# cavelandiah/BBMap

Hardware: AMD Instinct MI355X
Metric: aligned_reads_per_sec (higher is better)
Workload: dtype int32

## Files before the change

### bbmap_amd/csrc/mapper_ctx.h

```cpp
#pragma once
#include <hip/hip_runtime.h>

#include <cstdio>
#include <thread>
#include <vector>

#include "bbmap_amd.h"
#include "host_common.h"
#include "index_ctx.h"
#include "mapper_dev.h"
#include "msa_ctx.h"

enum { HIO_READS, HIO_BASES, HIO_SCORES, HIO_KEYINFO, HIO_COUNTS, HIO_OFFSETS, HIO_PACKED, BUF_PACK_TMP, BUF_SAM_TMP, BUF_SAM_TEXT, BUF_COUNT };

enum { ACC_STATS, ACC_COV, ACC_HIST, ACC_SPLIT, ACC_COUNT };
struct Accum { bool counted = false; hipStream_t stream = nullptr; };

struct bbmap_ctx {
    bbmap_config cfg;
    bbidx_ctx *index;
    hipStream_t hostStream = nullptr;
    bbidx_launch probeLs;
    bbmsa_ctx *msa, *msaGapped;
    bbmapper::Settings S;
    std::vector<void *> allocs;
    bbidx_site *d_psites; int *d_pnsites;
    bbmap_msite *d_ms; int *d_mcount, *d_near;
    bbmapper::SlowState *d_slow;
    int *d_active[2];
    int *d_classList;
    unsigned *d_counters;
    bbmsa_job *d_jobs; bbmap_jobinfo *d_jinfo; bbmsa_result *d_results; uint8_t *d_match;
    bbmsa_job *d_gjobs; bbmsa_gaps *d_ggaps; bbmap_jobinfo *d_ginfo; bbmsa_result *d_gresults; uint8_t *d_gmatch;
    bbresc_job *d_rjobs; bbmapper::RescInfo *d_rinfo; bbresc_result *d_rres; bbmapper::PairResc *d_pres; bbmap_msite *d_rsite;
    const uint8_t *const *d_chromArr; const int *d_chromArrLen; const uint8_t *refsBase;
    int *d_chromMin;
    long long *d_chromOff;
    long long jobCap, gjobCap, rescCap;
    bbmapper::FinalRead *d_fin; bbmap_final *d_final; uint8_t *d_pool; long long poolUnits, poolUsed, finalFills;
    int matchStride, gmatchStride, maxRows, plainColumns;
    unsigned *h_counters;
    hipEvent_t ev[bbmapper::EV_COUNT];
    bbmap_stats stats;
    long long nJobs, nGapped;
    bool ran;
    bbmap_ctx *tier;
    bool ownsMsa;
    long long narrowMinJobs;
    bool sortWide;
    bool sortPlain;
    bool classSwap;
    bool classOrder;
    bool kernargDev;
    int *d_tierUnits; bbidx_read *d_tierReads; int *d_tierReadIds;
    long long tierReads;
    hipStream_t tierStream;
    hipStream_t dpStream; hipEvent_t evFork, evJoin;
    std::thread tierThread;
    bool tierStarted;
    int tierRc; char tierErr[320];
    long long overAfterBegin;
    struct BatchArgs { int64_t n_reads; const bbidx_read *reads; uint8_t *bases; int64_t minus_delta; const int8_t *baseScores; const int32_t *keyinfo; } batch;
    DevBuf buf[BUF_COUNT];
    bbmap_scafrec *d_scafRec = nullptr;
    int *d_scafTier = nullptr;
    bbmap_samrec *d_samRec = nullptr;
    bbmap_samtags *d_samTags = nullptr;
    int *d_samCounts = nullptr;
    long long *d_samOffsets = nullptr;
    float *d_mapqMax = nullptr;
    long long samTextBytes = 0;
    unsigned long long *d_runStats = nullptr, *d_insertHist = nullptr;
    int adaptive = 0;
    long long numMatedSeen = 0;
    const bbmap_truth *truthNext = nullptr;
    struct CovState *cov = nullptr;
    unsigned long long *d_readHist = nullptr;
    int rhFlags = 0;
    uint8_t *d_pool2 = nullptr; long long pool2Units = 0;
    int *d_untrimCounts = nullptr;
    long long *d_untrimOffsets = nullptr;
    DevBuf untrimTmp;
    bool untrimmed = false;
    struct SplitState *split = nullptr;
    Accum accum[ACC_COUNT];
    void new_batch() { for (Accum &a : accum) a.counted = false; untrimmed = false; }
};

struct SplitState {
    bbmap_split_config cfg = {};
    int nscaf = 0;
    long long gen = 0, added = -1, total = 0;
    DevBuf sets, keys, state, recs, ws, setoff, units;
    SplitState() = default;
    SplitState(const SplitState &) = delete;
    ~SplitState() { for (DevBuf *b : {&sets, &keys, &state, &recs, &ws, &setoff, &units}) b->release(); }
};

struct CovState {
    int flags = 0, nscaf = 0, binsize = -1;
    long long slots = 0, nbins = 0, gen = 0;
    DevBuf covoff, len, diff[2], depth[2], recs, hist[2], totals, ws, refgc, binoff, bins[2];
// ... 19 lines not shown
```

### bbmap_amd/csrc/mapper_host.hip

```cpp
#include <hip/hip_runtime.h>

#include <algorithm>
#include <cstdlib>
#include <cstring>
#include <new>
#include <thread>
#include <vector>

#include "mapper_ctx.h"

using namespace bbmapper;

extern "C" int bbmap_default_config_profile(int32_t profile, bbmap_config *c) {
    if (!c || (profile != BBIDX_PROFILE_BBMAP && profile != BBIDX_PROFILE_PACBIO)) return bbfail(BBMAP_E_ARG, "bbmap_default_config: bad argument");
    memset(c, 0, sizeof *c);
    c->paired = 0; c->max_reads = 0; c->max_sites = 32;
    c->extraPadding = 10; c->maxPairDist = 32000; c->averagePairDist = 100; c->maxRescueDist = 1200; c->maxRescueMismatches = 32;
    c->maxTrimSitesToRetain = 800; c->trimList = 1; c->doRescue = 1; c->clearzone3 = 800; c->fastCols = 0; c->jobsPerRead = 0;
    c->finalStage = profile == BBIDX_PROFILE_BBMAP ? 1 : 0;
    if (profile == BBIDX_PROFILE_PACBIO) {
        c->max_read_len = 6016; c->minRatio = 0.46f; c->slowAlignPadding = 8; c->slowRescuePadding = 16; c->tipSearchDist = 15;
        c->alignColumns = 7600; c->msaMaxColumns = 7600;
    } else {
        c->max_read_len = 150; c->minRatio = 0.56f; c->slowAlignPadding = 4; c->slowRescuePadding = 8; c->tipSearchDist = 100;
// ... 62 lines not shown
    S.clearzone1e = 2 * S.ptsMatch2 - S.ptsMatch - S.ptsSub + 1;
    S.msaMaxColumns = cfg->msaMaxColumns;
    if (pacbio) { S.ptsSubR = -157; S.ptsIns = -205; S.ptsIns2 = -42; S.ptsIns3 = -23; S.ptsIns4 = -8; S.ptsDel = -292; S.ptsDel2 = -37; S.ptsDel3 = -17; S.ptsDel4 = -2; }
    else { S.ptsSubR = -147; S.ptsIns = -395; S.ptsIns2 = -39; S.ptsIns3 = -23; S.ptsIns4 = -8; S.ptsDel = -472; S.ptsDel2 = -33; S.ptsDel3 = -9; S.ptsDel4 = -1; }
    S.ptsDel5 = -1; S.ptsGap = -2;
    if (pacbio && (cfg->finalStage < 0 || cfg->finalStage > 2)) return bail(bbfail(BBMAP_E_ARG, "bbmap_create: finalStage must be 0, 1 or 2"));
    S.finalStage = cfg->finalStage ? 1 : 0;
    S.finalPolicy = (pacbio && cfg->finalStage == 1) ? 1 : 0;
    {
        const float rP = S.finalPolicy ? 1.5f : 1.6f, r1 = S.finalPolicy ? 2.2f : 2.0f, r1b = S.finalPolicy ? 2.8f : 2.6f, r1c = S.finalPolicy ? 4.8f : 4.6f;
        const float m2 = (float)S.ptsMatch2;
        S.czP = (int)(rP * m2); S.cz1 = (int)(r1 * m2); S.cz1b = (int)(r1b * m2); S.cz1c = (int)(r1c * m2);
        S.czLimit1e = 40;
    }
    index->dev.p.quitAfterTwoPerfects = cfg->paired ? 0 : 1;
    S.expLimit = (cfg->alignColumns * 17) / 20 - (2 * (cfg->slowAlignPadding + 10));
    const int maxRows = ((cfg->max_read_len + 31) / 32) * 32;
    c->maxRows = maxRows;
    bbmsa_config mc; memset(&mc, 0, sizeof mc);
    mc.device = cfg->device; mc.maxRows = maxRows;
    bbmsa_config gc;
    if (pacbio) {
        mc.maxRows = cfg->max_read_len + 4 > 6100 ? 6100 : cfg->max_read_len + 4;
        c->maxRows = mc.maxRows;
        mc.maxColumns = cfg->msaMaxColumns;
        mc.reserved[2] = BBMSA_SCHEME_9PACBIO;
        gc = mc;
        c->plainColumns = mc.maxColumns;
        if (parent) { c->msa = parent->msa; c->msaGapped = parent->msaGapped; c->ownsMsa = false; }
        else {
            c->ownsMsa = true;
            if ((rc = bbmsa_create(&mc, &c->msa)) != BBMAP_OK) return bail(rc);
            c->msaGapped = c->msa;
        }
    } else {
        mc.maxColumns = cfg->fastCols > 0 ? cfg->fastCols : 256;
        if (mc.maxColumns > cfg->msaMaxColumns) mc.maxColumns = cfg->msaMaxColumns;
        c->plainColumns = mc.maxColumns;
        gc = mc;
        gc.maxColumns = cfg->msaMaxColumns;
        gc.reserved[0] = 32; gc.reserved[1] = 640 < gc.maxColumns ? 640 : gc.maxColumns;
        if (const char *e = getenv("BBMAP_G2_LANES")) { if (*e) gc.reserved[0] = atoi(e); }
        if (const char *e = getenv("BBMAP_G2_COLS")) { if (*e) gc.reserved[1] = atoi(e) < gc.maxColumns ? atoi(e) : gc.maxColumns; }
        (void)parent;
        c->ownsMsa = true;
        if ((rc = bbmsa_create(&mc, &c->msa)) != BBMAP_OK) return bail(rc);
        if ((rc = bbmsa_create(&gc, &c->msaGapped)) != BBMAP_OK) return bail(rc);
    }
    const long long n = cfg->max_reads;
    const int cap = cfg->max_sites;
    c->narrowMinJobs = getenv("BBMAP_NARROW_MIN_JOBS") ? atoll(getenv("BBMAP_NARROW_MIN_JOBS")) : 32768;
    c->sortWide = !(getenv("BBMAP_SORT_WIDE") && atoi(getenv("BBMAP_SORT_WIDE")) == 0);
    c->sortPlain = !(getenv("BBMAP_SORT_PLAIN") && atoi(getenv("BBMAP_SORT_PLAIN")) == 0);
    c->classOrder = !(getenv("BBMAP_CLASS_ORDER") && atoi(getenv("BBMAP_CLASS_ORDER")) == 0);
    c->classSwap = getenv("BBMAP_CLASS_ORDER") && atoi(getenv("BBMAP_CLASS_ORDER")) == 2;
    c->kernargDev = !(getenv("BBMAP_KERNARG_DEV") && atoi(getenv("BBMAP_KERNARG_DEV")) == 0);
    S.chunkLoads = !(getenv("BBMAP_CHUNK_LOADS") && atoi(getenv("BBMAP_CHUNK_LOADS")) == 0);
    if (!pacbio) {
        const bool wideUnl = !(getenv("BBMAP_WIDE_UNLIMITED") && atoi(getenv("BBMAP_WIDE_UNLIMITED")) == 0);
        bbmsa_set_wide_unlimited(c->msa, wideUnl);
        if (c->msaGapped != c->msa) bbmsa_set_wide_unlimited(c->msaGapped, wideUnl);
    }
    if (!pacbio) {
        const long long lat = getenv("BBMAP_LATENCY_JOBS") ? atoll(getenv("BBMAP_LATENCY_JOBS")) : 4096;
        if ((rc = bbmsa_set_latency_jobs(c->msa, lat)) != BBMAP_OK) return bail(rc);
        if (c->msaGapped != c->msa && (rc = bbmsa_set_latency_jobs(c->msaGapped, lat)) != BBMAP_OK) return bail(rc);
    }
    const int jpr = cfg->jobsPerRead > 0 ? cfg->jobsPerRead : 3;
    c->jobCap = n * jpr + 1024;
    c->gjobCap = parent ? n * 16 + 4096 : (n * jpr) / 24 + 4096;
    if (cfg->jobsPerRead < 0) c->jobCap = c->gjobCap = -(long long)cfg->jobsPerRead;
    c->rescCap = parent ? n * 64 + 1024 : n * 2 + 1024;
    c->matchStride = ((maxRows + c->plainColumns + 15) / 16) * 16;
    c->gmatchStride = ((maxRows + gc.maxColumns + 2 + 128 * 8 + 15) / 16) * 16;
#define DA(ptr, count) if ((rc = dalloc(c, &(ptr), (size_t)(count))) != BBMAP_OK) return bail(rc)
    DA(c->d_psites, n * cap); DA(c->d_pnsites, n);
    DA(c->d_ms, n * cap); DA(c->d_mcount, n); DA(c->d_near, n);
    DA(c->d_slow, n);
    DA(c->d_active[0], n); DA(c->d_active[1], n);
    c->d_classList = nullptr;
    if (c->classOrder) DA(c->d_classList, 2 * n);
    DA(c->d_counters, CNT_WORDS);
    DA(c->d_jobs, c->jobCap); DA(c->d_jinfo, c->jobCap); DA(c->d_results, c->jobCap); DA(c->d_match, c->jobCap * c->matchStride);
    DA(c->d_gjobs, c->gjobCap); DA(c->d_ggaps, c->gjobCap); DA(c->d_ginfo, c->gjobCap); DA(c->d_gresults, c->gjobCap); DA(c->d_gmatch, c->gjobCap * c->gmatchStride);
    DA(c->d_rjobs, c->rescCap); DA(c->d_rinfo, c->rescCap); DA(c->d_rres, c->rescCap); DA(c->d_rsite, c->rescCap);
    DA(c->d_pres, n / 2 + 1);
    if (S.finalStage) {
        c->poolUnits = (n * (long long)(3 * (cfg->max_read_len + 16)) + 65536) / 4;
        if (const char *e = getenv("BBMAP_FINAL_POOL_UNITS")) { if (*e && atoll(e) >= 64) c->poolUnits = atoll(e); }
        DA(c->d_fin, n); DA(c->d_final, n); DA(c->d_pool, c->poolUnits * 4);
    }
    const int nch = index->dev.nchroms;
    DA(c->d_chromMin, nch + 1); DA(c->d_chromOff, nch + 1);
#undef DA
    c->d_chromArr = index->dev.chromArr; c->d_chromArrLen = index->dev.chromArrLen;
    {
        std::vector<const uint8_t *> hc((size_t)nch + 1);
        if (hipMemcpy(hc.data(), index->dev.chromArr, sizeof(void *) * hc.size(), hipMemcpyDeviceToHost) != hipSuccess) return bail(bbfail(BBMAP_E_HIP, "bbmap_create: reading the chromosome table failed"));
        c->refsBase = hc[1];
        std::vector<long long> off((size_t)nch + 1, 0);
        for (int i = 1; i <= nch; i++) off[(size_t)i] = (long long)(hc[(size_t)i] - hc[1]);
        if (hipMemcpy(c->d_chromOff, off.data(), 8 * off.size(), hipMemcpyHostToDevice) != hipSuccess) return bail(bbfail(BBMAP_E_HIP, "bbmap_create: upload failed"));
        if (hipMemset(c->d_chromMin, 0, 4 * ((size_t)nch + 1)) != hipSuccess) return bail(bbfail(BBMAP_E_HIP, "bbmap_create: memset failed"));
    }
    if (hipHostMalloc((void **)&c->h_counters, CNT_WORDS * 4) != hipSuccess) return bail(bbfail(BBMAP_E_NOMEM, "bbmap_create: pinned allocation failed"));
    for (hipEvent_t &e : c->ev) if (hipEventCreate(&e) != hipSuccess) return bail(bbfail(BBMAP_E_HIP, "bbmap_create: hipEventCreate failed"));
// ... 30 lines not shown
    return BBMAP_OK;
}

static int read_counters(bbmap_ctx *c, hipStream_t stream) {
    BBHIP(hipMemcpyAsync(c->h_counters, c->d_counters, CNT_WORDS * 4, hipMemcpyDeviceToHost, stream));
    BBHIP(hipStreamSynchronize(stream));
    return BBMAP_OK;
}

template <class T> static int regrow(bbmap_ctx *c, hipStream_t stream, T **p, size_t oldCount, size_t newCount, std::vector<void *> &dead) {
    void *d = nullptr;
    if (hipMalloc(&d, (newCount ? newCount : 1) * sizeof(T)) != hipSuccess) return bbfail(BBMAP_E_NOMEM, "bbmap_map_batch_device: growing a fill log failed (device memory)");
    if (oldCount) BBHIP(hipMemcpyAsync(d, *p, oldCount * sizeof(T), hipMemcpyDeviceToDevice, stream));
    for (void *&q : c->allocs) if (q == (void *)*p) q = d;
    dead.push_back((void *)*p);
    *p = (T *)d;
    return BBMAP_OK;
}
struct DeadArrays {
    hipStream_t stream; std::vector<void *> v;
    explicit DeadArrays(hipStream_t s) : stream(s) {}
    ~DeadArrays() { if (!v.empty()) { (void)hipStreamSynchronize(stream); for (void *q : v) (void)hipFree(q); } }
};
static int grow_logs(bbmap_ctx *c, hipStream_t stream, Dev &D, long long needJobs, long long needGapped, long long usedJobs, long long usedGapped) {
    DeadArrays guard(stream);
    std::vector<void *> &dead = guard.v;
    if (needJobs > c->jobCap) {
        long long nc = c->jobCap * 2; if (nc < needJobs) nc = needJobs + needJobs / 4 + 1024;
        BBTRY(regrow(c, stream, &c->d_jobs, (size_t)usedJobs, (size_t)nc, dead));
        BBTRY(regrow(c, stream, &c->d_jinfo, (size_t)usedJobs, (size_t)nc, dead));
        BBTRY(regrow(c, stream, &c->d_results, (size_t)usedJobs, (size_t)nc, dead));
        BBTRY(regrow(c, stream, &c->d_match, (size_t)usedJobs * c->matchStride, (size_t)nc * c->matchStride, dead));
        c->jobCap = nc;
    }
    if (needGapped > c->gjobCap) {
        long long nc = c->gjobCap * 2; if (nc < needGapped) nc = needGapped + needGapped / 4 + 1024;
        BBTRY(regrow(c, stream, &c->d_gjobs, (size_t)usedGapped, (size_t)nc, dead));
        BBTRY(regrow(c, stream, &c->d_ggaps, (size_t)usedGapped, (size_t)nc, dead));
        BBTRY(regrow(c, stream, &c->d_ginfo, (size_t)usedGapped, (size_t)nc, dead));
        BBTRY(regrow(c, stream, &c->d_gresults, (size_t)usedGapped, (size_t)nc, dead));
        BBTRY(regrow(c, stream, &c->d_gmatch, (size_t)usedGapped * c->gmatchStride, (size_t)nc * c->gmatchStride, dead));
        c->gjobCap = nc;
    }
    c->h_counters[CNT_STAGE_FILLS] = (unsigned)usedJobs; c->h_counters[CNT_STAGE_GAPPED] = (unsigned)usedGapped;
    BBHIP(hipMemcpyAsync(c->d_counters + CNT_FILLS, c->h_counters + CNT_STAGE_FILLS, 8, hipMemcpyHostToDevice, stream));
    BBHIP(hipStreamSynchronize(stream));
    D.jobs = c->d_jobs; D.jinfo = c->d_jinfo; D.results = c->d_results; D.match = c->d_match; D.jobCap = c->jobCap;
    D.gjobs = c->d_gjobs; D.ggaps = c->d_ggaps; D.ginfo = c->d_ginfo; D.gresults = c->d_gresults; D.gmatch = c->d_gmatch; D.gjobCap = c->gjobCap;
    c->stats.log_growths += 1.0f;
    return BBMAP_OK;
}

static int run_fills(bbmap_ctx *c, hipStream_t stream, const uint8_t *bases, long long jobBase, long long nNew, long long gBase, long long gNew,
                     bool finalStage = false) {
    bbmsa_use_narrow(c->msa, nNew >= c->narrowMinJobs);
    bbmsa_sort_by_width(c->msa, c->sortPlain && nNew >= c->narrowMinJobs);
    bbmsa_sort_with_band(c->msa, c->sortPlain);
    if (c->msaGapped != c->msa) { bbmsa_use_narrow(c->msaGapped, false); bbmsa_sort_by_width(c->msaGapped, c->sortWide); }
    hipStream_t gs = (c->dpStream && nNew > 0) ? c->dpStream : stream;
    if (gNew > 0) {
        if (gs != stream) { BBHIP(hipEventRecord(c->evFork, stream)); BBHIP(hipStreamWaitEvent(gs, c->evFork, 0)); }
        BBTRY(bbmsa_align_gapped_batch_device(c->msaGapped, gs, gNew, c->d_gjobs + gBase, c->d_ggaps + gBase, bases, c->refsBase,
                                             c->d_gresults + gBase, c->d_gmatch + gBase * c->gmatchStride, c->gmatchStride));
        if (gs != stream) { BBHIP(hipEventRecord(c->evJoin, gs)); if (nNew > 0) BBTRY(bbmsa_wait_first_pass(c->msaGapped, stream)); }
    }
    if (nNew > 0)
        BBTRY(bbmsa_align_batch_device(c->msa, stream, nNew, c->d_jobs + jobBase, bases, c->refsBase, c->d_results + jobBase,
                                      c->d_match + jobBase * c->matchStride, c->matchStride));
    const int r1 = nNew > 0 ? bbmsa_last_route_flags(c->msa) : 0;
    const int r2 = gNew > 0 ? bbmsa_last_route_flags(c->msaGapped) : 0;
    c->stats.dp_narrow_launches += (r1 & 1) + (r2 & 1);
    c->stats.dp_sorted_launches += ((r1 >> 1) & 1) + ((r2 >> 1) & 1);
    if (gNew > 0 && gs != stream) BBHIP(hipStreamWaitEvent(stream, c->evJoin, 0));
    return BBMAP_OK;
}

static void add_dp_ms(bbmap_ctx *c, bool plain, bool gapped) {
    float k3[3];
    if (plain && bbmsa_last_kernel_ms3(c->msa, k3) == BBMAP_OK) { c->stats.ms_dp_narrow += k3[0]; c->stats.ms_dp_wave += k3[1]; c->stats.ms_dp_generic += k3[2];
                                                                 if (k3[1] > c->stats.ms_dp_wave_max) c->stats.ms_dp_wave_max = k3[1]; }
    if (gapped && c->msaGapped != c->msa && bbmsa_last_kernel_ms3(c->msaGapped, k3) == BBMAP_OK) c->stats.ms_dp_gapped += k3[0] + k3[1] + k3[2];
    static const bool show = getenv("BBMAP_DP_COUNTS") != nullptr;
    if (show) {
        int64_t n4[4], u4[4];
        if (plain && bbmsa_last_counts(c->msa, n4) == BBMAP_OK && bbmsa_last_unlimited(c->msa, u4) == BBMAP_OK)
            fprintf(stderr, "dp counts plain : narrow finished %lld, narrow handed on %lld, wavefront list %lld, to the wide/generic pass %lld, "
                    "unlimited in their own build %lld, in the general build %lld, wavefront steps unlimited %lld of %lld\n",
                    (long long)n4[0], (long long)n4[1], (long long)n4[2], (long long)n4[3], (long long)u4[0], (long long)u4[1], (long long)u4[2], (long long)u4[3]);
        if (gapped && bbmsa_last_counts(c->msaGapped, n4) == BBMAP_OK && bbmsa_last_unlimited(c->msaGapped, u4) == BBMAP_OK)
            fprintf(stderr, "dp counts second: narrow finished %lld, narrow handed on %lld, wavefront list %lld, to the wide/generic pass %lld, "
                    "unlimited in their own build %lld, in the general build %lld, wavefront steps unlimited %lld of %lld\n",
                    (long long)n4[0], (long long)n4[1], (long long)n4[2], (long long)n4[3], (long long)u4[0], (long long)u4[1], (long long)u4[2], (long long)u4[3]);
    }
}

static void tier_start_async(bbmap_ctx *c, long long found);

struct Rounds {
    bool finalStage;
    long long jobBase, gBase;
    long long nActive;
    int cur = 0;
    bool first = true, ranPlain = false, ranGapped = false;
};
template <class K> static int round_begin(bbmap_ctx *c, hipStream_t stream, Dev &D, Rounds &R, K kernel) {
    BBHIP(hipMemsetAsync(c->d_counters + CNT_NEXT_ACTIVE, 0, 4, stream));
    if (R.finalStage) {
        BBHIP(hipMemsetAsync(c->d_counters + CNT_POOL_AT_FAILURE, 0xff, 4, stream));
        BBHIP(hipMemsetAsync(c->d_counters + CNT_POOL_FAILED, 0, 4, stream));
    }
    D.activeIn = R.first ? nullptr : c->d_active[R.cur]; D.nActiveIn = (int)R.nActive; D.activeOut = c->d_active[1 - R.cur];
    BBTRY(launch<128>(kernel, R.nActive, stream, D));
    return read_counters(c, stream);
}
static int round_end(bbmap_ctx *c, hipStream_t stream, Dev &D, Rounds &R, const uint8_t *bases) {
    add_dp_ms(c, R.ranPlain, R.ranGapped);
    const long long asked = c->h_counters[CNT_FILLS], gasked = c->h_counters[CNT_GAPPED_FILLS];
    const long long total = asked < c->jobCap ? asked : c->jobCap, gtotal = gasked < c->gjobCap ? gasked : c->gjobCap;
    BBTRY(run_fills(c, stream, bases, R.jobBase, total - R.jobBase, R.gBase, gtotal - R.gBase, R.finalStage));
    R.ranPlain = total > R.jobBase; R.ranGapped = gtotal > R.gBase;
    R.jobBase = total; R.gBase = gtotal;
    if (asked > c->jobCap || gasked > c->gjobCap) BBTRY(grow_logs(c, stream, D, asked, gasked, total, gtotal));
    R.nActive = c->h_counters[CNT_NEXT_ACTIVE];
    R.cur = 1 - R.cur; R.first = false;
    return BBMAP_OK;
}

static int grow_pool(bbmap_ctx *c, hipStream_t stream, Dev &D, long long used, long long units, bool setCounter) {
    if (units > 0x7ffffff0LL) return bbfail(BBMAP_E_NOMEM, "bbmap_map_batch_device: the final stage's match strings exceed 8 GB; map smaller batches");
    DeadArrays guard(stream);
    BBTRY(regrow(c, stream, &c->d_pool, (size_t)used * 4, (size_t)units * 4, guard.v));
    if (setCounter) {
        c->h_counters[CNT_STAGE_POOL] = (unsigned)used;
        BBHIP(hipMemcpyAsync(c->d_counters + CNT_POOL_UNITS, c->h_counters + CNT_STAGE_POOL, 4, hipMemcpyHostToDevice, stream));
    }
    BBHIP(hipStreamSynchronize(stream));
    c->poolUnits = units; D.pool = c->d_pool; D.poolUnits = units;
    return BBMAP_OK;
}

static int run_final_stage(bbmap_ctx *c, hipStream_t stream, Dev &D, int64_t n_reads, const uint8_t *bases, long long jobBase, long long gBase,
                           long long &finalRounds, long long &finalLocal) {
    const long long units = c->cfg.paired ? n_reads / 2 : n_reads;
    const unsigned *h = c->h_counters;
    D.fin = c->d_fin; D.finalOut = c->d_final; D.pool = c->d_pool; D.poolUnits = c->poolUnits;
    D.match = c->d_match; D.gmatch = c->d_gmatch; D.matchStride = c->matchStride; D.gmatchStride = c->gmatchStride;
    if (D.classList) BBHIP(hipMemsetAsync(c->d_counters + CNT_CLASS_LONG, 0, 8, stream));
    BBTRY(launch<128>(final_begin_kernel, units, stream, D));
    Rounds R; R.finalStage = true; R.jobBase = jobBase; R.gBase = gBase; R.nActive = n_reads;
    for (int round = 0; R.nActive > 0; round++) {
        if (round > 64 * c->cfg.max_sites + 64) return bbfail(BBMAP_E_HIP, "bbmap_map_batch_device: the final stage does not come to an end (internal error)");
        BBTRY(round_begin(c, stream, D, R, DEV_KERNEL(c, final_round_kernel)));
        BBTRY(round_end(c, stream, D, R, bases));
        if (h[CNT_POOL_FAILED] > 0) {
            const long long used = h[CNT_POOL_AT_FAILURE];
            long long nu = c->poolUnits * 2, need = used + ((long long)h[CNT_POOL_UNITS] - used) * 2 + 65536;
            if (nu < need) nu = need;
            BBTRY(grow_pool(c, stream, D, used, nu, true));
        }
        finalRounds++;
    }
    BBHIP(hipStreamSynchronize(stream));
    add_dp_ms(c, R.ranPlain, R.ranGapped);
    BBHIP(hipMemsetAsync(c->d_counters + CNT_LOCAL_READS, 0, 8, stream));
    BBTRY(launch<128>(final_end_kernel, units, stream, D));
    BBTRY(read_counters(c, stream));
    finalLocal = h[CNT_LOCAL_READS];
    const long long used = h[CNT_POOL_UNITS], local = h[CNT_LOCAL_UNITS];
    if (used + local + 64 > c->poolUnits) BBTRY(grow_pool(c, stream, D, used, used + local + 65536, false));
    BBTRY(launch<128>(final_local_kernel, units, stream, D));
    return BBMAP_OK;
}
// ... 51 lines not shown
    if (writeRc) BBTRY(launch<128>(revcomp_unprobed_kernel, n_reads, stream, reads, (long long)n_reads, (int)c->index->dev.p.k, (const uint8_t *)bases, bases + minus_delta));
    BBHIP(hipEventRecord(c->ev[EV_PROBE_END], stream));
    Dev D;
    fill_dev(c, D, n_reads, reads, bases, minus_delta);
    const long long units = c->cfg.paired ? n_reads / 2 : n_reads;
    BBTRY(launch<128>(begin_kernel, units, stream, D));
    if (c->tier) {
        BBTRY(launch<128>(collect_overflow_kernel, units, stream, c->d_mcount, units, c->cfg.paired, c->d_tierUnits, c->d_counters + CNT_TIER_FOUND));
    }
    BBHIP(hipEventRecord(c->ev[EV_BEGIN_END], stream));
    BBTRY(launch<128>(DEV_KERNEL(c, score_kernel), n_reads, stream, D));
    BBHIP(hipEventRecord(c->ev[EV_SCORE_END], stream));
    Rounds R; R.finalStage = false; R.jobBase = R.gBase = 0; R.nActive = n_reads;
    for (int round = 0; R.nActive > 0 && round < 4 * c->cfg.max_sites + 4; round++) {
        BBTRY(round_begin(c, stream, D, R, slow_round_kernel));
        if (round == 0) {
            float pms = 0; long long ps[5];
            if (writeRc && bbidx_last_stats_with(c->index, &c->probeLs, (int64_t *)ps, &pms) == BBMAP_OK) for (int i = 0; i < 5; i++) c->stats.probe_stats[i] = ps[i];
            c->overAfterBegin = c->h_counters[CNT_OVERFLOWED];
            if (c->tier && c->h_counters[CNT_TIER_FOUND] > 0 && c->tier->msa != c->msa) tier_start_async(c, c->h_counters[CNT_TIER_FOUND]);
        }
        BBTRY(round_end(c, stream, D, R, bases));
        c->stats.rounds++;
    }
    long long jobBase = R.jobBase, gBase = R.gBase;
    BBHIP(hipEventRecord(c->ev[EV_SLOW_END], stream));
    BBTRY(launch<128>(finish_kernel, n_reads, stream, D));
    BBHIP(hipEventRecord(c->ev[EV_FINISH_END], stream));
    if (c->cfg.paired && c->cfg.doRescue) {
        const long long pairs = n_reads / 2;
        for (int pass = 0; pass < 2; pass++) {
            D.pass = pass;
            BBHIP(hipMemsetAsync(c->d_counters + CNT_RESCUE_SEARCHES, 0, 4, stream));
            BBTRY(launch<128>(rescue_plan_kernel, pairs, stream, D));
            BBTRY(read_counters(c, stream));
            const long long nsearch = c->h_counters[CNT_RESCUE_SEARCHES];
            if (nsearch > c->rescCap) return bbfail(BBMAP_E_NOMEM, "bbmap_map_batch_device: rescue list full");
            c->stats.rescue_scans += nsearch;
            if (nsearch == 0) {
                BBTRY(launch<128>(rescue_finish_kernel, pairs, stream, D));
                continue;
            }
            hipEvent_t q0 = c->ev[EV_QUICK_BEGIN], q1 = c->ev[EV_QUICK_END];
            BBHIP(hipEventRecord(q0, stream));
            BBTRY(bbpipe_quick_rescue_device(stream, nsearch, c->d_rjobs, bases, (const int64_t *)c->d_chromOff, c->d_chromArrLen, c->d_chromMin, c->refsBase,
                                            c->d_rres, c->S.ptsMatch, c->S.ptsMatch2, 1, 100));
            BBHIP(hipEventRecord(q1, stream));
            if (jobBase + nsearch > c->jobCap || gBase + nsearch > c->gjobCap) BBTRY(grow_logs(c, stream, D, jobBase + nsearch, gBase + nsearch, jobBase, gBase));
            BBTRY(launch<128>(DEV_KERNEL(c, rescue_prep_kernel), pairs, stream, D));
            BBTRY(read_counters(c, stream));
            { float ms = 0; if (hipEventElapsedTime(&ms, q0, q1) == hipSuccess) c->stats.ms_quick_rescue += ms; }
            const long long total = c->h_counters[CNT_FILLS], gtotal = c->h_counters[CNT_GAPPED_FILLS];
            if (total > c->jobCap || gtotal > c->gjobCap) return bbfail(BBMAP_E_HIP, "bbmap_map_batch_device: rescue fills beyond the reserved log entries (internal error)");
            BBTRY(run_fills(c, stream, bases, jobBase, total - jobBase, gBase, gtotal - gBase));
            const bool ranPlain = total > jobBase, ranGapped = gtotal > gBase;
            jobBase = total; gBase = gtotal;
            BBTRY(launch<128>(rescue_finish_kernel, pairs, stream, D));
            BBHIP(hipStreamSynchronize(stream));
            add_dp_ms(c, ranPlain, ranGapped);
        }
    }
    BBHIP(hipEventRecord(c->ev[EV_RESCUE_END], stream));
    c->finalFills = 0; c->poolUsed = 0;
    long long finalRounds = 0, finalLocal = 0;
    if (c->S.finalStage) BBTRY(run_final_stage(c, stream, D, n_reads, bases, jobBase, gBase, finalRounds, finalLocal));
    BBTRY(finish_stats(c, stream, true, jobBase + gBase, finalRounds, finalLocal));
    c->ran = true;
    return BBMAP_OK;
}

static int tier_pass(bbmap_ctx *c, hipStream_t s, long long found) {
    bbmap_ctx *t = c->tier;
    const bbmap_ctx::BatchArgs &B = c->batch;
    const int paired = c->cfg.paired;
    c->tierReads = 0; t->ran = false;
    std::vector<int> ids((size_t)found);
    BBHIP(hipMemcpyAsync(ids.data(), c->d_tierUnits, 4 * (size_t)found, hipMemcpyDeviceToHost, s));
    BBHIP(hipStreamSynchronize(s));
    std::sort(ids.begin(), ids.end());
    const long long room = paired ? t->cfg.max_reads / 2 : t->cfg.max_reads;
    const long long take = found < room ? found : room;
    BBHIP(hipMemcpyAsync(c->d_tierUnits, ids.data(), 4 * (size_t)take, hipMemcpyHostToDevice, s));
    BBTRY(launch<128>(gather_reads_kernel, take, s, B.reads, c->d_tierUnits, (int)take, paired, c->d_tierReads, c->d_tierReadIds));
    BBHIP(hipStreamSynchronize(s));
    const long long tn = paired ? 2 * take : take;
    BBTRY(map_records(t, s, tn, c->d_tierReads, B.bases, B.minus_delta, B.baseScores, B.keyinfo, false));
    c->tierReads = tn;
    return BBMAP_OK;
}

static void tier_start_async(bbmap_ctx *c, long long found) {
    c->tierStarted = true; c->tierRc = BBMAP_OK; c->tierErr[0] = 0;
    c->tierThread = std::thread([c, found]() {
        int rc = hipSetDevice(c->cfg.device) == hipSuccess ? BBMAP_OK : BBMAP_E_HIP;
        if (rc == BBMAP_OK) rc = tier_pass(c, c->tierStream, found);
        if (rc != BBMAP_OK) { snprintf(c->tierErr, sizeof c->tierErr, "overflow tier: %s", bbmap_last_error()); }
        c->tierRc = rc;
    });
}

static int tier_finish(bbmap_ctx *c, hipStream_t stream) {
    bbmap_ctx *t = c->tier;
    const long long tn = c->tierReads;
    if (tn == 0) return BBMAP_OK;
    BBHIP(hipMemsetAsync(c->d_counters + CNT_TIER_RESOLVED, 0, 4, stream));
    BBTRY(launch<128>(mark_tier_kernel, tn, stream, c->d_mcount, t->d_mcount, c->d_tierReadIds, (int)tn, c->d_counters + CNT_TIER_RESOLVED));
    BBTRY(read_counters(c, stream));
    bbmap_stats &st = c->stats; const bbmap_stats &ts = t->stats;
    st.reads_reprobed = tn;
    st.reads_overflowed -= (long long)c->h_counters[CNT_TIER_RESOLVED];
    st.reads_without_site += ts.reads_without_site;
    st.fills += ts.fills; st.gapped_fills += ts.gapped_fills; st.refills += ts.refills; st.rescue_scans += ts.rescue_scans;
    st.rescue_fills += ts.rescue_fills; st.fills_dropped += ts.fills_dropped;
    st.final_fills += ts.final_fills; st.final_local += ts.final_local;
    st.dp_narrow_launches += ts.dp_narrow_launches; st.dp_sorted_launches += ts.dp_sorted_launches;
    st.sites_cross_scaffold += ts.sites_cross_scaffold;
    if (getenv("BBMAP_TIER_DEBUG"))
        fprintf(stderr, "[bbmap tier] reads %lld: probe %.2f begin %.2f score %.2f slow %.2f (rounds %lld) finish %.2f rescue %.2f total %.2f\n",
                tn, ts.ms_probe, ts.ms_begin, ts.ms_score, ts.ms_slow, (long long)ts.rounds, ts.ms_finish, ts.ms_rescue, ts.ms_total);
    return BBMAP_OK;
}

static int rescue_skip_rule(bbmap_ctx *c, bool *skip) {
    *skip = false;
    if (!c->d_runStats) return BBMAP_OK;
    bbmap_runstats rs;
    BBHIP(hipStreamSynchronize(c->accum[ACC_STATS].stream));
    BBHIP(hipMemcpy(&rs, c->d_runStats, sizeof rs, hipMemcpyDeviceToHost));
    *skip = rs.mappedRetained2 > 1000 && rs.numMated * 20LL < rs.mappedRetained2;
    return BBMAP_OK;
}

static int adapt_after_batch(bbmap_ctx *c, hipStream_t stream) {
    if (!(c->adaptive & BBMAP_ADAPT_INSERT_LENGTH)) return BBMAP_OK;
    bbmap_runstats rs;
    BBHIP(hipMemcpyAsync(&rs, c->d_runStats, sizeof rs, hipMemcpyDeviceToHost, stream));
    BBHIP(hipStreamSynchronize(stream));
    const bool heldPaired = rs.numMated > c->numMatedSeen;
    c->numMatedSeen = rs.numMated;
    if (rs.numMated > 1000 && heldPaired) {
        volatile float sum = (float)rs.innerLengthSum, cnt = (float)rs.numMated;
        const float q = sum * 1.0f / cnt;
        const int v = (int)q;
        if (v >= 0) BBTRY(bbmap_set_average_pair_dist(c, v));
    }
    return BBMAP_OK;
}

extern "C" int bbmap_get_adaptive_state(bbmap_ctx *c, int32_t *averagePairDist, int32_t *rescueSkipped) {
    if (!c) return bbfail(BBMAP_E_ARG, "bbmap_get_adaptive_state: null context");
    if (averagePairDist) *averagePairDist = c->cfg.averagePairDist;
    if (rescueSkipped) {
        bool skip = false;
        if (c->adaptive & BBMAP_ADAPT_RESCUE_SKIP) { BBHIP(hipSetDevice(c->cfg.device)); BBTRY(rescue_skip_rule(c, &skip)); }
        *rescueSkipped = skip ? 1 : 0;
    }
    return BBMAP_OK;
}

static int map_batch_device(bbmap_ctx *c, hipStream_t stream, int64_t n_reads, const bbidx_read *reads, uint8_t *bases,
                            int64_t minus_delta, const int8_t *baseScores, const int32_t *keyinfo) {
    c->batch = {n_reads, reads, bases, minus_delta, baseScores, keyinfo};
    c->tierStarted = false; c->tierReads = 0;
    if (c->tier) c->tier->ran = false;
    const int rc = map_records(c, stream, n_reads, reads, bases, minus_delta, baseScores, keyinfo, true);
    hipEvent_t e0 = c->ev[EV_TIER_BEGIN], e1 = c->ev[EV_TIER_END];
    if (c->tierStarted) {
        c->tierThread.join();
        if (rc == BBMAP_OK && c->tierRc != BBMAP_OK) return bbfail(c->tierRc, "%s", c->tierErr);
// ... 71 lines not shown
```

### bbmap_amd/csrc/msa_common.h

```cpp
#pragma once
#include <hip/hip_runtime.h>
#include <stdint.h>
#include "bbmap_amd.h"

namespace bbmsa {

constexpr int kScoreOffset = 11;
constexpr int kTimeMask = 0x7FF;
constexpr int kScoreMask = (int)0xFFFFF800;
constexpr int kMaxTime = 2047;

#define BBMSA_PT(x) ((x) * 2048)
constexpr int P_MATCH = BBMSA_PT(70), P_MATCH2 = BBMSA_PT(100);
constexpr int P_SUB = BBMSA_PT(-127), P_SUBR = BBMSA_PT(-147), P_SUB2 = BBMSA_PT(-51), P_SUB3 = BBMSA_PT(-25);
constexpr int P_INS = BBMSA_PT(-395), P_INS2 = BBMSA_PT(-39), P_INS3 = BBMSA_PT(-23), P_INS4 = BBMSA_PT(-8);
constexpr int P_DEL = BBMSA_PT(-472), P_DEL2 = BBMSA_PT(-33), P_DEL3 = BBMSA_PT(-9), P_DEL4 = BBMSA_PT(-1),
              P_DEL5 = BBMSA_PT(-1);
constexpr int P_DEL_REF_N = BBMSA_PT(-10), P_GAP = BBMSA_PT(-2);
constexpr int kBadOff = (-(((1 << 20) - 1) - 2000) - 1) * 2048;
constexpr int kMinOffScore = (-(((1 << 20) - 1) - 2000)) * 2048;
constexpr int kNegInf = -(1 << 30);
constexpr int kGapLen = 128;

constexpr int kTableLen = 3072;
// ... 48 lines not shown
    static constexpr int BAR_I1 = 1, BAR_D1 = 1;
    static constexpr int BADOFF = (-(((1 << 22) - 1) - 2000) - 1) * 512;
#undef BBMSA_PB
    __host__ __device__ static inline int del_off(int len) {
        if (len <= 0) return 0;
        int s = DEL;
        if (len > 80) { s += ((len - 80 + 3) / 4) * DEL5; len = 80; }
        if (len > 20) { s += (len - 20) * DEL4; len = 20; }
        if (len > 5) { s += (len - 5) * DEL3; len = 5; }
        if (len > 1) s += (len - 1) * DEL2;
        return s;
    }
    __host__ __device__ static inline int ins_cum_off(int len) {
        if (len <= 0) return 0;
        int s = INS;
        if (len > 20) { s += (len - 20) * INS4; len = 20; }
        if (len > 5) { s += (len - 5) * INS3; len = 5; }
        if (len > 1) s += (len - 1) * INS2;
        return s;
    }
    __host__ __device__ static inline int col0(int row) {
        if (row <= 0) return 0;
        int s = INS;
        if (row >= 20) { s += (row - 19) * INS4; row = 19; }
        if (row >= 5) { s += (row - 4) * INS3; row = 4; }
        if (row >= 2) s += (row - 1) * INS2;
        return s;
    }
};

__host__ __device__ inline int fill_halfband(int rows, int columns, int bandwidth, float bandwidthRatio) {
    if (bandwidth < 1 && bandwidthRatio <= 0.0f) return 0;
    const int bwA = bandwidth < 1 ? 9999999 : bandwidth;
    const int bwB = bandwidthRatio <= 0.0f ? 9999999 : 8 + (int)((float)rows * bandwidthRatio);
    return max(min(bwA, bwB), columns - rows + 8) / 2;
}
__host__ __device__ inline bool fill_is_limited(int flags, int minScore, int rows, int columns, int halfband) {
    const int mode = flags & BBMSA_MODE_MASK;
    if (mode == BBMSA_FILL_UNLIMITED_RAW) return false;
    if (mode == BBMSA_FILL_LIMITED_RAW) return true;
    return !(minScore < 1 || (columns + rows < 90) ||
             ((halfband < 1 || halfband * 3 > columns) && (columns > rows + min(170, rows + 20))));
}

__host__ __device__ inline bool band_is_candidate(int flags, int minScore, int rows, int columns, int maxRows, int maxColumns, int bandRows, int maxSlack) {
    const int mode = flags & BBMSA_MODE_MASK;
    if (!(rows >= 16 && columns >= rows && rows <= maxRows && rows <= bandRows && columns <= maxColumns && mode != BBMSA_FILL_UNLIMITED_RAW)) return false;
    int tmin = minScore;
    if (mode == BBMSA_FILL_LIMITED) {
        if (tmin < 1 || (columns + rows < 90) || (columns > rows + min(170, rows + 20))) return false;
        tmin -= 120;
    }
    return (70 + 100 * (rows - 1)) - tmin <= maxSlack;
}

__device__ inline long long job_count(long long njobs, const unsigned int *njobs_dev) {
    if (!njobs_dev) return njobs;
    const long long n = (long long)__hip_atomic_load(njobs_dev, __ATOMIC_RELAXED, __HIP_MEMORY_SCOPE_AGENT);
    return n < njobs ? n : njobs;
}

constexpr int kCounterWords = 32, kCounterBytes = kCounterWords * 4;
enum CounterSlot {
    CNT_FAST_QUEUE = 0,
    CNT_SLOW_COUNT = 1,
    CNT_GENERIC_QUEUE = 2,
    CNT_BAND_QUEUE = 3,
    CNT_LIST_COUNT = 4,
    CNT_BAND_DONE = 5,
    CNT_BAND_HANDED = 6,
    CNT_WIDE_SLOW_COUNT = 7,
    CNT_WIDE_QUEUE = 8,
    CNT_UNL_RAN_UNL = 9,
    CNT_UNL_RAN_GENERAL = 10,
    CNT_UNL_LIST_COUNT = 11,
    CNT_UNL_QUEUE = 12,
    CNT_UNL_STEPS = 13,
    CNT_ALL_STEPS = 14,
    CNT_CAND_COUNT = 15,
    CNT_SORTED_COUNT = 16,
    CNT_WAVE_STEPS = 17,
};
constexpr int CNT_BAND_STATS = 5, CNT_UNL_STATS = 9;
enum BandStat { BAND_STAT_DONE = 0, BAND_STAT_HANDED = 1 };
enum UnlStat { UNL_STAT_RAN_UNL = 0, UNL_STAT_RAN_GENERAL = 1, UNL_STAT_STEPS = 4, UNL_STAT_ALL_STEPS = 5, UNL_STAT_WAVE_STEPS = 8 };
static_assert(CNT_BAND_DONE == CNT_BAND_STATS + BAND_STAT_DONE && CNT_BAND_HANDED == CNT_BAND_STATS + BAND_STAT_HANDED, "band kernel's counters");
static_assert(CNT_UNL_RAN_UNL == CNT_UNL_STATS + UNL_STAT_RAN_UNL && CNT_UNL_RAN_GENERAL == CNT_UNL_STATS + UNL_STAT_RAN_GENERAL &&
              CNT_UNL_STEPS == CNT_UNL_STATS + UNL_STAT_STEPS && CNT_ALL_STEPS == CNT_UNL_STATS + UNL_STAT_ALL_STEPS &&
              CNT_WAVE_STEPS == CNT_UNL_STATS + UNL_STAT_WAVE_STEPS, "wavefront kernel's counters");
constexpr bool counter_slots_distinct() {
    constexpr int all[] = {CNT_FAST_QUEUE, CNT_SLOW_COUNT, CNT_GENERIC_QUEUE, CNT_BAND_QUEUE, CNT_LIST_COUNT, CNT_BAND_DONE, CNT_BAND_HANDED,
                           CNT_WIDE_SLOW_COUNT, CNT_WIDE_QUEUE, CNT_UNL_RAN_UNL, CNT_UNL_RAN_GENERAL, CNT_UNL_LIST_COUNT, CNT_UNL_QUEUE,
                           CNT_UNL_STEPS, CNT_ALL_STEPS, CNT_CAND_COUNT, CNT_SORTED_COUNT, CNT_WAVE_STEPS};
    unsigned seen = 0;
    for (int s : all) { if (s < 0 || s >= kCounterWords || ((seen >> s) & 1u)) return false; seen |= 1u << s; }
    return true;
}
static_assert(counter_slots_distinct(), "two counter names share a word, or one lies outside d_counters");

struct FillParams {
    const bbmsa_job *jobs;
    const uint8_t *reads;
    const uint8_t *refs;
    bbmsa_result *results;
    uint8_t *match;
    long long njobs;
    const unsigned int *njobs_dev;
    unsigned int *queue;
    unsigned int *dirbuf;
    long long dir_slot_dwords;
    const int *list;
    const unsigned int *list_count;
    int priority;
    int *slow_list;
    unsigned int *slow_count;
    int match_stride;
    int lanesPerJob;
    int fastCols;
    int tmpBytes;
    int tableLen;
    int maxRows, maxColumns;
    int bandwidth;
    float bandwidthRatio;
    unsigned int *unl_stats;
    int *planes;
    const long long *plane_off;
    int *limits;
    const long long *limits_off;
};

struct NarrowParams {
    const bbmsa_job *jobs;
    const uint8_t *reads;
    const uint8_t *refs;
    bbmsa_result *results;
    uint8_t *match;
    long long njobs;
    const unsigned int *njobs_dev;
    unsigned int *queue;
    int *fast_list;
    unsigned int *fast_count;
    unsigned int *stats;
    int match_stride;
    int maxRows, maxColumns;
    int bandwidth;
    float bandwidthRatio;
    int maxSlack;
    unsigned int *dirbuf32;
    int tableLen;
    int bandRows;
    const int *list;
    const unsigned int *list_count;
};

struct GenericParams {
    const bbmsa_job *jobs;
    const uint8_t *reads;
    const uint8_t *refs;
    bbmsa_result *results;
    uint8_t *match;
    const int *list;
    const unsigned int *list_count;
    long long njobs;
    const unsigned int *njobs_dev;
    int *matrix;
    int *limits;
    unsigned int *queue;
    int match_stride;
    int maxRows, maxColumns;
    int bandwidth;
    float bandwidthRatio;
};

}
```

### bbmap_amd/csrc/msa_ctx.h

```cpp
#pragma once
#include <hip/hip_runtime.h>

#include "bbmap_amd.h"
#include "host_common.h"
#include "msa_route.h"

struct bbmsa_ctx {
    bbmsa_config cfg = {};
    int device = 0;
    int numCUs = 0;
    RouteSwitches sw;
    Route last;
    int G = 0, R = 0, fastCols = 0, tmpBytes = 0, blocks = 0, ldsBytes = 0, tableLen = 0, wideTableLen = 0;
    long long dirSlotDwords = 0;
    unsigned int *d_dir = nullptr;
    unsigned int *d_counters = nullptr;
    DevBuf slowList;
    int genThreads = 0;
    int *d_matrix = nullptr;
    int *d_limits = nullptr;
    int wideR = 0, wideCols = 0, wideTmpBytes = 0, wideBlocks = 0, wideLdsBytes = 0;
    long long wideDirSlotDwords = 0;
    unsigned int *d_wideDir = nullptr;
    DevBuf slowList2;
    int narrowBlocks = 0, narrowSlack = 0;
    bool unlimitedStats = false;
    unsigned int *d_widthHist = nullptr;
    int bandRows = 0, bandLds = 0;
    unsigned int *d_bandDir = nullptr;
    DevBuf fastList;
    DevBuf gref, gaux, gjobs;
    hipEvent_t ev[4] = {};
    bool timed = false;
    bool legacyOnly = false;
    struct bbmsa_legacy *legacy = nullptr;
    int stripBlocks = 0, stripLds = 0;
    long long stripDwords = 0, stripSlotDwords = 0;
    int *d_stripBoundary = nullptr;
    uint8_t *d_stripTmp = nullptr;
    int pipeK = 0, pipeSlots = 0;
    int *d_pipeBoundary = nullptr, *d_pipeSync = nullptr;
};

struct JobBatch {
    int64_t n_jobs; const uint32_t *n_jobs_dev; const bbmsa_job *jobs; const uint8_t *reads, *refs; bbmsa_result *results; uint8_t *match;
    int32_t match_stride;
};
template <class P> void set_batch(P &p, const bbmsa_ctx *c, const JobBatch &B) {
    p.jobs = B.jobs; p.reads = B.reads; p.refs = B.refs; p.results = B.results; p.match = B.match;
    p.njobs = B.n_jobs; p.njobs_dev = B.n_jobs_dev; p.match_stride = B.match_stride;
    p.maxRows = c->cfg.maxRows; p.maxColumns = c->cfg.maxColumns; p.bandwidth = c->cfg.bandwidth; p.bandwidthRatio = c->cfg.bandwidthRatio;
}

int bbmsa_width_sort(bbmsa_ctx *c, hipStream_t stream, const bbmsa_job *jobs, int64_t n_jobs, bool band);

int bbmsa_align_impl(bbmsa_ctx *c, void *stream_, int64_t n_jobs, const uint32_t *n_jobs_dev, const bbmsa_job *jobs,
                     const uint8_t *reads, const uint8_t *refs, bbmsa_result *results, uint8_t *match, int32_t match_stride);

void bbmsa_use_narrow(bbmsa_ctx *c, bool on);
int bbmsa_wait_first_pass(bbmsa_ctx *c, void *waiter);
void bbmsa_sort_by_width(bbmsa_ctx *c, bool on);
void bbmsa_sort_with_band(bbmsa_ctx *c, bool on);
void bbmsa_set_wide_unlimited(bbmsa_ctx *c, bool on);
int bbmsa_set_latency_jobs(bbmsa_ctx *c, int64_t n);
enum { BBMSA_ROUTE_NARROW = 1, BBMSA_ROUTE_SORTED = 2, BBMSA_ROUTE_LATENCY = 4 };
int bbmsa_last_route_flags(const bbmsa_ctx *c);

int bbmsa_legacy_create(bbmsa_ctx *c);
void bbmsa_legacy_destroy(bbmsa_ctx *c);
void bbmsa_legacy_rows_per_lane(bbmsa_ctx *c, int *last, int *mask);
```

### bbmap_amd/csrc/msa_fill_band.hip

```cpp
#include "msa_common.h"
#include "msa_cell.h"

namespace bbmsa {

namespace {

__device__ __forceinline__ int from_left(int x, int fill) { return __builtin_amdgcn_update_dpp(fill, x, 0x138, 0xf, 0xf, false); }
__device__ __forceinline__ int from_right(int x, int fill) { return __builtin_amdgcn_update_dpp(fill, x, 0x130, 0xf, 0xf, false); }

__device__ __forceinline__ unsigned ld_coherent(const unsigned *p) { return __hip_atomic_load(p, __ATOMIC_RELAXED, __HIP_MEMORY_SCOPE_AGENT); }
__device__ __forceinline__ unsigned ld_coherent(const uint8_t *p) { return __hip_atomic_load(p, __ATOMIC_RELAXED, __HIP_MEMORY_SCOPE_AGENT); }

struct BandSet {
    int M[4], D[4], I[4];
    int rows, columns;
    int c0off;
    int minScoreOff, vs;
    unsigned w;
    int gprev;
    int gmask, mprev;
    int gpass;
    int bail;
    int rdOff, rfOff;
    int slot;
};

}

#ifndef BBMSA_BAND_OCC
#define BBMSA_BAND_OCC 4
#endif

template <int Q>
__global__ __launch_bounds__(256, BBMSA_BAND_OCC) void msa_fill_band_kernel(const NarrowParams p) {
    constexpr int B = 4 * Q;
    constexpr int GROUPS = 64 / Q;
    constexpr int JOBS = 2 * GROUPS;
    static_assert(Q == 4 || Q == 8 || Q == 16, "a group is a power of two of lanes, its good bits fit 64");
    extern __shared__ int lds[];
    const int TL = p.tableLen;
    int *delC = lds, *insC = lds + TL, *delExt = lds + 2 * TL, *insExt = delExt + 128;
    int4 *mTab = reinterpret_cast<int4 *>(delExt + 192);
    LdsPen pen; pen.delC = delC; pen.insC = insC; pen.delExt = delExt; pen.insExt = insExt; pen.mTab = mTab;
    for (int i = threadIdx.x; i < TL; i += blockDim.x) { delC[i] = calc_del_off(i); insC[i] = calc_ins_cum_off(i); }
    for (int i = threadIdx.x; i < 128; i += blockDim.x) delExt[i] = SpelledPen<Scheme11ts>().del_ext(i);
    if (threadIdx.x < 32) insExt[threadIdx.x] = SpelledPen<Scheme11ts>().ins_ext(threadIdx.x);
    if (threadIdx.x < 32) {
        const int st = threadIdx.x & 7, mt = (threadIdx.x >> 3) & 1, pv = threadIdx.x >> 4;
        const MEntry e = SpelledPen<Scheme11ts>().m_entry(min(st, 5), 0, 0, pv != 0, mt != 0);
        int4 v; v.x = e.addA; v.y = e.bonus; v.z = e.t3sub; v.w = 0;
        mTab[threadIdx.x] = v;
    }
    __syncthreads();

    const int lane = threadIdx.x & 63, wave = threadIdx.x >> 6;
    const int q = lane & (Q - 1), grp = lane / Q, groupBase = grp * Q;
    const int RB = (p.bandRows + 4 + 3) & ~3, FB = (p.bandRows + B + 4 + 3) & ~3;
    uint8_t *jobLds = reinterpret_cast<uint8_t *>(lds + lds_table_ints(TL)) + (long long)wave * JOBS * (RB + FB);
    unsigned *dir = p.dirbuf32 + ((long long)blockIdx.x * 4 + wave) * (long long)(p.bandRows + 1) * 128;
    const long long NJ = p.list ? (long long)ld_coherent(p.list_count) : job_count(p.njobs, p.njobs_dev);
    unsigned nDone = 0, nLeft = 0;

    for (;;) {
        long long myJ = -1;
        if (lane < JOBS) {
            for (;;) {
                const long long e_ = (long long)atomicAdd(p.queue, 1u);
                if (e_ >= NJ || e_ >= p.njobs) break;
                const long long t_ = p.list ? (long long)p.list[e_] : e_;
                const bbmsa_job t = p.jobs[t_];
                int ta = t.refStartLoc, tb = t.refEndLoc;
                if (t.flags & BBMSA_CLAMP_WINDOW) {
                    ta = max(0, ta); tb = min(t.ref_len - 1, tb);
                    if (tb - ta >= p.maxColumns) tb = min(t.ref_len - 1, ta + p.maxColumns - 1);
                }
                if (band_is_candidate(t.flags, t.minScore, t.read_len, tb - ta + 1, p.maxRows, p.maxColumns, p.bandRows, p.maxSlack)) { myJ = t_; break; }
                const unsigned k = atomicAdd(p.fast_count, 1u);
                p.fast_list[k] = (int)t_;
            }
        }
        if (!__any(myJ >= 0)) break;

        BandSet S[2];
        long long jobJ[2]; bool jobOk[2];
#pragma unroll
        for (int s = 0; s < 2; s++) {
            const long long j = __shfl(myJ, grp * 2 + s, 64);
            jobJ[s] = j;
            bbmsa_job jb;
            jb.read_off = 0; jb.ref_off = 0; jb.read_len = 0; jb.ref_len = 0; jb.refStartLoc = 0; jb.refEndLoc = -1; jb.minScore = 0; jb.flags = 0;
            if (j >= 0) jb = p.jobs[j];
            int a = jb.refStartLoc, b = jb.refEndLoc;
            if (jb.flags & BBMSA_CLAMP_WINDOW) {
                a = max(0, a); b = min(jb.ref_len - 1, b);
                if (b - a >= p.maxColumns) b = min(jb.ref_len - 1, a + p.maxColumns - 1);
            }
            const int rows = jb.read_len, columns = b - a + 1;
            int minScore = jb.minScore;
            if ((jb.flags & BBMSA_MODE_MASK) == BBMSA_FILL_LIMITED) minScore -= 120;
            const int D0 = (columns - rows) / 2 - B / 2;
            const uint8_t *rd = p.reads + jb.read_off, *rf = p.refs + jb.ref_off + a;
            const int rdOff = (grp * 2 + s) * (RB + FB), rfOff = rdOff + RB;
            int cost = 0; bool allDef = true;
#pragma unroll 4
            for (int i = q; i < rows; i += Q) {
                const int cb = rd[i];
                jobLds[rdOff + i] = (uint8_t)cb;
                if (fully_defined(cb)) cost += (i + 1 < rows && fully_defined(rd[i + 1])) ? P_MATCH2 : P_MATCH;
            }
            if (j >= 0)
#pragma unroll 4
            for (int k = q; k < rows + B + 1; k += Q) {
                const int col = k + D0;
                int v = 0;
                if (col == 0) v = '!';
                else if (col >= 1 && col <= columns) { v = rf[col - 1]; allDef = allDef && fully_defined(v); }
                jobLds[rfOff + k] = (uint8_t)v;
            }
            for (int c = 1 + q; c <= columns; c += Q) if (c < 1 + D0 || c > D0 + B) allDef = allDef && fully_defined(rf[c - 1]);
            int nd = allDef ? 0 : 1;
            for (int d = 1; d < Q; d <<= 1) { cost += __shfl_xor(cost, d, 64); nd |= __shfl_xor(nd, d, 64); }
            bool ok = j >= 0 && nd == 0;

            const int minScoreOff = minScore * 2048;
            const int floorv = minScoreOff - ((rows - 1) * P_MATCH2 + P_MATCH);
            const int subfloor = floorv - 5 * P_MATCH2;
            if (ok) {
                const int cl1 = rd[0];
                const int c0cost = fully_defined(cl1) ? ((rows > 1 && fully_defined(rd[1])) ? P_MATCH2 : P_MATCH) : 0;
                const int vlimP = max(minScoreOff - (cost - c0cost), floorv) + 2048;
                int outGood = 0;
                for (int c = 1 + q; c <= columns; c += Q) {
                    if (c >= 1 + D0 && c <= D0 + B) continue;
                    const int ref1 = rf[c - 1];
                    const int hs = c <= columns - 1 ? P_MATCH + (columns - 1 - c) * P_MATCH2 : 0;
                    CellIn ci;
                    ci.row = 1; ci.c = c; ci.rows = rows; ci.insNeededBase = (columns - c) + 1;
                    ci.cl1 = cl1; ci.ref1 = ref1; ci.refN = false; ci.gap = false; ci.match = cl1 == ref1; ci.act = true;
                    ci.refPen = 0; ci.limitP = max(vlimP, max(minScoreOff - hs, floorv) + 2048); ci.floorP = floorv + 2048; ci.subfloor = subfloor;
                    ci.dgM = 0; ci.dgD = 0; ci.dgI = 0;
                    ci.lM = c == 1 ? insC[1] : subfloor; ci.lD = ci.lM; ci.upM = 0; ci.upI = 0;
                    ci.delForce = INT_MAX;
                    ci.insForce = (c > 1 || (1 > rows - 2 && c < columns - 1)) ? INT_MAX : INT_MIN;
                    ci.pm8 = 0;
                    const CellOut co = cell_update<Scheme11ts, false>(pen, ci);
                    outGood |= (co.goodM | co.goodD | co.goodI) ? 1 : 0;
                }
                for (int d = 1; d < Q; d <<= 1) outGood |= __shfl_xor(outGood, d, 64);
                if (outGood) ok = false;
            }
            if (j >= 0 && !ok && q == 0) { const unsigned k = atomicAdd(p.fast_count, 1u); p.fast_list[k] = (int)j; nLeft++; }
            jobOk[s] = ok;

            const int set = (q & 1) ^ s;
#pragma unroll
            for (int x = 0; x < 2; x++) if (x == set) {
                BandSet &T = S[x];
                for (int i = 0; i < 4; i++) { T.M[i] = 0; T.D[i] = 0; T.I[i] = 0; }
                T.rows = ok ? rows : 0; T.columns = columns; T.c0off = D0 + 4 * q;
                T.minScoreOff = minScoreOff; T.vs = cost;
                T.w = 0; T.gprev = 1; T.gmask = 0; T.mprev = 0; T.gpass = 0; T.bail = 0;
                T.rdOff = rdOff; T.rfOff = rfOff; T.slot = s;
            }
        }
        __builtin_amdgcn_fence(__ATOMIC_ACQ_REL, "wavefront");
        __builtin_amdgcn_wave_barrier();
#pragma unroll
        for (int x = 0; x < 2; x++) {
            BandSet &T = S[x];
            if (T.rows > 0) for (int i = 0; i < 3; i++) T.w |= (unsigned)jobLds[T.rfOff + 1 + 4 * q + i] << (8 * (i + 1));
        }
        int maxRowsWave = max(S[0].rows, S[1].rows);
        for (int d = 32; d >= 1; d >>= 1) maxRowsWave = max(maxRowsWave, __shfl_xor(maxRowsWave, d, 64));

        const int rowLagX = (q + 1) >> 1, rowLagY = q >> 1;
        for (int k = 1; k <= maxRowsWave + Q / 2; k++) {
#pragma unroll
            for (int x = 0; x < 2; x++) {
                BandSet &T = S[x];
                const BandSet &O = S[1 - x];
                const int row = k - (x == 0 ? rowLagX : rowLagY);
                int lM = from_left(O.M[3], 0), lD = from_left(O.D[3], 0), gIn = from_left(O.gpass, 0);
                int uM = from_right(O.M[0], 0), uI = from_right(O.I[0], 0), uG = from_right(O.gmask, 0);
                const bool rowAct = row >= 1 && row <= T.rows;
                if (rowAct) {
                    const int rows = T.rows, columns = T.columns;
                    const int floorv = T.minScoreOff - ((rows - 1) * P_MATCH2 + P_MATCH);
                    const int subfloor = floorv - 5 * P_MATCH2, floorP = floorv + 2048;
                    if (q == 0) { lM = subfloor; lD = subfloor; gIn = 0; }
                    if (q == Q - 1) { uM = row == 1 ? 0 : subfloor; uI = uM; uG = 0; }
                    const int cl1 = jobLds[T.rdOff + row - 1];
                    const int clN = row < rows ? jobLds[T.rdOff + row] : 0;
                    T.vs -= fully_defined(cl1) ? (fully_defined(clN) ? P_MATCH2 : P_MATCH) : 0;
                    const int vlimP = max(T.minScoreOff - T.vs, floorv) + 2048;
                    T.w = (T.w >> 8) | ((unsigned)jobLds[T.rfOff + row + 4 * q + 3] << 24);
                    const int c0 = row + T.c0off;
                    const int insRow = insC[row], insPrev = insC[row - 1];
                    const int delForce = (row < 3 || row > rows - 3) ? INT_MAX : INT_MIN;
                    const unsigned g5 = (unsigned)T.gmask | (((unsigned)uG & 1u) << 4);
                    const bool rowOne = row == 1;
                    unsigned goods = 0, mbits = 0, word = 0;
                    int leftM = lM, leftD = lD;
#pragma unroll
                    for (int i = 0; i < 4; i++) {
                        const int c = c0 + i;
                        const int ref1 = (int)((T.w >> (8 * i)) & 255u);
                        const bool inRange = (c >= 1) & (c <= columns);
                        const bool started = (T.gprev != 0) | ((g5 & ((4u << i) - 1u)) != 0u);
                        const bool first = c == 1;
                        const int hs = c <= columns - 1 ? P_MATCH + (columns - 1 - c) * P_MATCH2 : 0;
                        CellIn ci;
                        ci.row = row; ci.c = c; ci.rows = rows; ci.insNeededBase = (columns - c) + 1;
                        ci.cl1 = cl1; ci.ref1 = ref1; ci.refN = false; ci.gap = false; ci.match = cl1 == ref1; ci.act = inRange & started;
                        ci.refPen = 0; ci.limitP = max(vlimP, max(T.minScoreOff - hs, floorv) + 2048); ci.floorP = floorP; ci.subfloor = subfloor;
                        ci.dgM = first ? insPrev : T.M[i]; ci.dgD = first ? insPrev : T.D[i]; ci.dgI = first ? insPrev : T.I[i];
                        ci.lM = first ? insRow : leftM; ci.lD = first ? insRow : leftD;
                        ci.upM = i < 3 ? T.M[i + 1] : uM; ci.upI = i < 3 ? T.I[i + 1] : uI;
                        ci.delForce = delForce;
                        ci.insForce = ((rowOne & (c > 1)) | ((row > rows - 2) & (c < columns - 1))) ? INT_MAX : INT_MIN;
                        ci.pm8 = ((T.mprev >> i) & 1) ? 8 : 0;
                        const CellOut co = cell_update<Scheme11ts, false>(pen, ci);
                        const bool good = co.goodM | co.goodD | co.goodI;
                        goods |= good ? (1u << i) : 0u;
                        mbits |= ci.match ? (1u << i) : 0u;
                        word |= co.nib << (4 * i);
                        T.M[i] = co.nM; T.D[i] = co.nD; T.I[i] = co.nI;
                        leftM = co.nM; leftD = co.nD;
                    }
                    if (q == 0 && (goods & 1u) && c0 >= 1) T.bail = 1;
                    if (q == Q - 1 && (goods & 8u) && c0 + 3 < columns) T.bail = 1;
                    T.gprev = gIn; T.gmask = (int)goods; T.mprev = (int)mbits; T.gpass = (gIn | (goods ? 1 : 0));
                    dir[((long long)row * 2 + T.slot) * 64 + lane] = word | (goods << 16);
                }
            }
        }
        asm volatile("s_waitcnt vmcnt(0)" ::: "memory");
        __builtin_amdgcn_wave_barrier();

#pragma unroll
        for (int s = 0; s < 2; s++) {
            const long long j = jobJ[s];
            const int set = (q & 1) ^ s;
            int lastM[4], lastD[4], lastI[4];
#pragma unroll
            for (int i = 0; i < 4; i++) { lastM[i] = set ? S[1].M[i] : S[0].M[i]; lastD[i] = set ? S[1].D[i] : S[0].D[i]; lastI[i] = set ? S[1].I[i] : S[0].I[i]; }
            int bail = set ? S[1].bail : S[0].bail;
            for (int d = 1; d < Q; d <<= 1) bail |= __shfl_xor(bail, d, 64);
            const bool live = jobOk[s];
            if (live && bail) { if (q == 0) { const unsigned k = atomicAdd(p.fast_count, 1u); p.fast_list[k] = (int)j; nLeft++; } }
            if (!(live && !bail)) continue;

            const bbmsa_job jb = p.jobs[j];
            int a = jb.refStartLoc, b = jb.refEndLoc;
            if (jb.flags & BBMSA_CLAMP_WINDOW) {
                a = max(0, a); b = min(jb.ref_len - 1, b);
                if (b - a >= p.maxColumns) b = min(jb.ref_len - 1, a + p.maxColumns - 1);
            }
            const int rows = jb.read_len, columns = b - a + 1, mode = jb.flags & BBMSA_MODE_MASK;
            const int minScoreOff = (mode == BBMSA_FILL_LIMITED ? jb.minScore - 120 : jb.minScore) * 2048;
            const int subfloor = minScoreOff - ((rows - 1) * P_MATCH2 + P_MATCH) - 5 * P_MATCH2;
            const int D0 = (columns - rows) / 2 - B / 2;
            const uint8_t *rdL = jobLds + (grp * 2 + s) * (RB + FB), *rfL = rdL + RB;
            const unsigned *jdir = dir + s * 64 + groupBase;

            const int per = (rows + Q - 1) / Q;
            const int rFirst = q * per + 1, rLast = min(rows, (q + 1) * per);
            int iters = 0, lastColStart = 1, lastHasGood = 0, lastEntered = 0;
            {
                unsigned long long pg = 0;
                if (rFirst > 1 && rFirst <= rLast) for (int l = 0; l < Q; l++) pg |= (unsigned long long)((ld_coherent(jdir + (long long)(rFirst - 1) * 128 + l) >> 16) & 15u) << (4 * l);
                for (int r = rFirst; r <= rLast; r++) {
                    unsigned long long g = 0;
                    for (int l = 0; l < Q; l++) g |= (unsigned long long)((ld_coherent(jdir + (long long)r * 128 + l) >> 16) & 15u) << (4 * l);
                    const bool entered = r == 1 || pg != 0;
                    const int colStart = r == 1 ? 1 : (r - 1) + D0 + __builtin_ctzll(pg | (1ull << 63));
                    const int colStop = r == 1 ? columns : (r - 1) + D0 + (63 - __builtin_clzll(pg | 1ull));
                    const int maxG = g ? r + D0 + (63 - __builtin_clzll(g)) : -2;
                    const int endc = min(columns, max(colStop, maxG) + 1);
                    if (entered) iters += endc - colStart + 1;
                    if (r == rows) { lastColStart = colStart; lastHasGood = g != 0; lastEntered = entered; }
                    pg = g;
                }
            }
            for (int d = 1; d < Q; d <<= 1) iters += __shfl_xor(iters, d, 64);
            {
                const int owner = groupBase + (rows - 1) / per;
                lastColStart = __shfl(lastColStart, owner, 64); lastHasGood = __shfl(lastHasGood, owner, 64); lastEntered = __shfl(lastEntered, owner, 64);
            }
            int bScore = INT_MIN, bKey = INT_MAX, bPacked = 0;
#pragma unroll
            for (int i = 0; i < 4; i++) {
                const int c = rows + D0 + 4 * q + i;
                if (c >= 1 && c <= columns) {
                    const int v[3] = {lastM[i], lastD[i], lastI[i]};
#pragma unroll
                    for (int st = 0; st < 3; st++) {
                        const int sc = v[st] & kScoreMask, key = st * 65536 + c;
                        if (sc > bScore || (sc == bScore && key < bKey)) { bScore = sc; bKey = key; bPacked = v[st]; }
                    }
                }
            }
            for (int d = 1; d < Q; d <<= 1) {
                const int os = __shfl_xor(bScore, d, 64), ok_ = __shfl_xor(bKey, d, 64), op = __shfl_xor(bPacked, d, 64);
                if (os > bScore || (os == bScore && ok_ < bKey)) { bScore = os; bKey = ok_; bPacked = op; }
            }
            const int bCol = bKey & 65535, bState = bKey >> 16;

            int res1, res2, res3, res4 = 0;
            bool fillNull = false;
            if (!lastEntered) { res1 = 1; res2 = 0; res3 = kBadOff; res4 = 1; fillNull = true; }
            else if (!lastHasGood) { res1 = max(1, lastColStart - 1); res2 = 0; res3 = subfloor; res4 = 1; fillNull = true; }
            else if (bScore < minScoreOff) { res1 = bCol; res2 = bState; res3 = bScore; res4 = 1; fillNull = true; }
            else { res1 = bCol; res2 = bState; res3 = bScore >> kScoreOffset; }

            const bool wantScore = !fillNull && (jb.flags & BBMSA_DO_SCORE);
            const bool wantTrace = !fillNull && (jb.flags & BBMSA_DO_TRACEBACK) && p.match != nullptr;
            int sc[8] = {0, 0, 0, 0, 0, 0, 0, 0};
            int scoreLen = 0, matchLen = 0;
            if (wantScore || wantTrace) {
                uint8_t *out = p.match ? p.match + j * (long long)p.match_stride : nullptr;
                auto nib_at = [&](int r, int c) -> unsigned {
                    const int pos = c - r - D0;
                    if (pos < 0 || pos >= B) return 0u;
                    return (ld_coherent(jdir + (long long)r * 128 + (pos >> 2)) >> (4 * (pos & 3))) & 15u;
                };
                int row = rows, col = res1, state = res2, n = 0, stateTime = 0;
                while (row > 0 && col > 0) {
                    if (state == 0) {
                        const int rr = row - q, cq = col - q;
                        const bool inside = rr >= 1 && cq >= 1;
                        const unsigned nibv = inside ? nib_at(rr, cq) : 0u;
                        const bool brk = !inside || (nibv & 3u) != 0u;
                        const unsigned long long mine = (__ballot(brk) >> groupBase) & ((1ull << Q) - 1ull);
                        const int fb = mine ? __builtin_ctzll(mine) : Q;
                        const int fbInside = __shfl((int)inside, groupBase + min(fb, Q - 1), 64);
                        const int fbPrev = __shfl((int)(nibv & 3u), groupBase + min(fb, Q - 1), 64);
                        const int consumed = (fb < Q && fbInside) ? fb + 1 : fb;
                        if (wantTrace && q < consumed && n + q < p.match_stride) {
                            const int cb = rdL[rr - 1], rb = rfL[min(max(cq - D0, 0), rows + B)];
                            out[n + q] = (cb == rb) ? 'm' : ((!fully_defined(cb) || !fully_defined(rb)) ? 'N' : 'S');
                        }
                        stateTime += fb;
                        if (fb < Q && fbInside) { stateTime = 0; state = fbPrev; }
                        row -= consumed; col -= consumed; n += consumed;
                    } else {
                        const unsigned nibv = nib_at(row, col);
                        int prev;
                        uint8_t sym;
                        if (state == 1) { prev = (nibv & 4u) ? 1 : 0; sym = 'D'; col--; }
                        else { prev = (nibv & 8u) ? 2 : 0; sym = (col >= columns) ? 'Y' : 'I'; row--; }
                        if (wantTrace && q == 0 && n < p.match_stride) out[n] = sym;
                        n++;
                        if (prev == state) stateTime++; else stateTime = 0;
                        state = prev;
                    }
                }
                int colS = col;
                if (row > colS) colS -= row;
                const int bestRefStart = a + colS, bestRefStop = a + res1 - 1;
                int padLeft = 0, padRight = 0;
                if (bestRefStart < a) padLeft = max(0, a - bestRefStart);
                else if (bestRefStart == a && state == 2) padLeft = stateTime;
                const int bW = (jb.flags & BBMSA_INTERNAL_GAPPED) ? jb.ref_len : b;
                if (bestRefStop > bW) padRight = max(0, bestRefStop - bW);
                else if (bestRefStop == bW && res2 == 2) padRight = bPacked & kTimeMask;
                if (wantScore) {
                    sc[0] = bScore >> kScoreOffset; sc[1] = bestRefStart; sc[2] = bestRefStop; sc[3] = rows; sc[4] = res1; sc[5] = res2;
                    scoreLen = (padLeft > 0 || padRight > 0) ? 8 : 6;
                    if (scoreLen == 8) { sc[6] = padLeft; sc[7] = padRight; }
                }
                if (wantTrace) {
                    const int xs = (col != row) ? row : 0;
                    for (int i = q; i < xs; i += Q) if (n + i < p.match_stride) out[n + i] = 'X';
                    n += xs;
                    if (n > p.match_stride) matchLen = -1;
                    else {
                        asm volatile("s_waitcnt vmcnt(0)" ::: "memory");
                        __builtin_amdgcn_wave_barrier();
                        for (int i = q; i < n / 2; i += Q) {
                            const uint8_t lo = (uint8_t)ld_coherent(out + i), hi = (uint8_t)ld_coherent(out + n - 1 - i);
                            out[i] = hi; out[n - 1 - i] = lo;
                        }
                        matchLen = n;
                    }
                }
            }
            if (q == 0) {
                bbmsa_result r;
                r.result[0] = rows; r.result[1] = res1; r.result[2] = res2; r.result[3] = res3; r.result[4] = res4;
                r.status = (fillNull && mode == BBMSA_FILL_LIMITED) ? BBMSA_ST_NULL : BBMSA_ST_OK;
                r.iterations = iters;
#pragma unroll
                for (int i = 0; i < 8; i++) r.score[i] = sc[i];
                r.score_len = scoreLen; r.match_len = matchLen; r.fill_kind = 0; r.columns = columns;
                p.results[j] = r;
                nDone++;
            }
        }
        __builtin_amdgcn_fence(__ATOMIC_ACQ_REL, "wavefront");
        __builtin_amdgcn_wave_barrier();
    }
    if (p.stats) {
        for (int d = 32; d >= 1; d >>= 1) { nDone += __shfl_xor(nDone, d, 64); nLeft += __shfl_xor(nLeft, d, 64); }
        if (lane == 0) { if (nDone) atomicAdd(&p.stats[BAND_STAT_DONE], nDone); if (nLeft) atomicAdd(&p.stats[BAND_STAT_HANDED], nLeft); }
    }
}

template __global__ void msa_fill_band_kernel<8>(const NarrowParams);

const void *band_kernel() { return (const void *)msa_fill_band_kernel<8>; }
int band_lds_bytes(int tableLen, int bandRows) {
    constexpr int Q = 8, B = 4 * Q, JOBS = 2 * (64 / Q);
    const int RB = (bandRows + 4 + 3) & ~3, FB = (bandRows + B + 4 + 3) & ~3;
    return lds_table_ints(tableLen) * 4 + 4 * JOBS * (RB + FB);
}

}
```

### bbmap_amd/csrc/msa_host.hip

```cpp
#include <hip/hip_runtime.h>

#include <cstdio>
#include <cstdlib>
#include <new>

#include "host_common.h"
#include "msa_common.h"
#include "msa_ctx.h"

namespace bbmsa {
struct StripParams {
    const bbmsa_job *jobs; const uint8_t *reads; const uint8_t *refs; bbmsa_result *results; uint8_t *match;
    long long njobs; const unsigned int *njobs_dev; unsigned int *queue; unsigned int *dirbuf;
    long long dir_slot_dwords, dir_strip_dwords; int *boundary; uint8_t *tmpbuf; int *slow_list; unsigned int *slow_count;
    int match_stride; int maxRows, maxColumns; int bandwidth; float bandwidthRatio;
    int pipeK, pipeSlots; int *pipeBoundary; int *pipeSync; int pipeSpinLimit;
};
int strip_rows_per_lane();
const void *strip_kernel_pacbio();
const void *strip_kernel_pacbio_pipelined();
int strip_pipe_sync_ints(int K);
const void *fast_kernel_for(int R, bool banded);
const void *fast_kernel_unl_for(int R);
const void *fast_kernel_both_for(int R);
template <class S> __global__ void msa_fill_generic_kernel(const GenericParams p);
const void *band_kernel();
int band_lds_bytes(int tableLen, int bandRows);
}

static int clamp_occupancy(int per, int most) { return per < 1 ? 1 : (per > most ? most : per); }

static int setup_wide_pass(bbmsa_ctx *c) {
    if (c->wideBlocks > 0) return BBMAP_OK;
    c->wideR = (c->cfg.maxRows + 63) / 64;
    c->wideCols = c->cfg.maxColumns;
    c->wideTmpBytes = ((64 * c->wideR + c->wideCols + 8) + 3) & ~3;
    const int perJob = bbmsa::lds_job_ints(c->wideCols, c->wideTmpBytes);
    c->wideLdsBytes = (bbmsa::lds_table_ints(c->wideTableLen) + perJob) * 4;
    const void *wfn = bbmsa::fast_kernel_for(c->wideR, c->sw.banded);
    if (wfn && c->wideLdsBytes <= 160 * 1024) {
        if (c->wideLdsBytes > 64 * 1024) BBHIP(hipFuncSetAttribute(wfn, hipFuncAttributeMaxDynamicSharedMemorySize, c->wideLdsBytes));
        const void *bfn = c->sw.banded ? nullptr : bbmsa::fast_kernel_both_for(c->wideR);
        if (bfn && c->wideLdsBytes > 64 * 1024) BBHIP(hipFuncSetAttribute(bfn, hipFuncAttributeMaxDynamicSharedMemorySize, c->wideLdsBytes));
        int per = 0;
        BBHIP(hipOccupancyMaxActiveBlocksPerMultiprocessor(&per, wfn, 64, c->wideLdsBytes));
        per = clamp_occupancy(per, 8);
        const long long slotDwords = (long long)(((c->wideCols + 64 - 1) >> 3) + 1) * c->wideR * 64;
        BBHIP(hipMalloc(&c->d_wideDir, (size_t)((long long)c->numCUs * per * slotDwords * 4)));
        c->wideDirSlotDwords = slotDwords;
        c->wideBlocks = c->numCUs * per;
        c->sw.widePresent = true;
    }
    return BBMAP_OK;
}

static int generic_threads(const bbmsa_config &cfg, int defaultMB, long long mostThreads, int *out) {
    const long long perThread = 3LL * (cfg.maxRows + 1) * (cfg.maxColumns + 2) * 4;
    long long threads = ((long long)env_int("BBMSA_GENERIC_SCRATCH_MB", defaultMB) << 20) / perThread;
    if (threads > mostThreads) threads = mostThreads;
    threads = (threads / 64) * 64;
    if (threads < 64) return bbfail(BBMAP_E_NOMEM, "bbmsa_create: BBMSA_GENERIC_SCRATCH_MB cannot hold one wavefront of scratch matrices for this maxRows x maxColumns");
    *out = (int)threads;
    return BBMAP_OK;
}
static int alloc_generic_scratch(bbmsa_ctx *c, int threads) {
    c->genThreads = threads;
    BBHIP(hipMalloc(&c->d_matrix, (size_t)threads * 3 * (size_t)(c->cfg.maxRows + 1) * (size_t)(c->cfg.maxColumns + 2) * 4));
    BBHIP(hipMalloc(&c->d_limits, (size_t)threads * (size_t)(c->cfg.maxRows + c->cfg.maxColumns + 4) * 4));
    return BBMAP_OK;
}

static int create_legacy_only(bbmsa_ctx *c) {
    BBTRY(alloc_generic_scratch(c, 1));
    return bbmsa_legacy_create(c);
}

static int create_pacbio(bbmsa_ctx *c) {
    const bbmsa_config *cfg = &c->cfg;
    int threads = 0;
    BBTRY(generic_threads(*cfg, 40960, 4096, &threads));
// ... 36 lines not shown
    if (G != 16 && G != 32 && G != 64) {
        G = env_int("BBMSA_LANES_PER_JOB", 0);
        if (G != 16 && G != 32 && G != 64) G = (cfg->maxRows <= 320) ? 32 : 64;
    }
    while (G < 64 && (cfg->maxRows + G - 1) / G > 10) G *= 2;
    c->G = G;
    c->R = (cfg->maxRows + G - 1) / G;
    int fastCols = cfg->reserved[1] > 0 ? cfg->reserved[1] : env_int("BBMSA_FAST_COLS", 0);
    if (fastCols <= 0) fastCols = cfg->maxColumns < 640 ? cfg->maxColumns : 640;
    if (fastCols > cfg->maxColumns) fastCols = cfg->maxColumns;
    c->fastCols = fastCols;
    c->tmpBytes = ((G * c->R + fastCols + 8) + 3) & ~3;
    const int jobsPerWave = 64 / G;
    const int perJobInts = bbmsa::lds_job_ints(fastCols, c->tmpBytes);
    {
        const int side = (cfg->maxColumns > cfg->maxRows ? cfg->maxColumns : cfg->maxRows) + 2;
        c->wideTableLen = (side < 2048 ? side : 2048) + cfg->maxRows + 8;
        const int sideF = (fastCols > cfg->maxRows ? fastCols : cfg->maxRows) + 2;
        c->tableLen = (sideF < 2048 ? sideF : 2048) + cfg->maxRows + 8;
    }
    if (c->tableLen > bbmsa::kTableLen) c->tableLen = bbmsa::kTableLen;
    if (c->wideTableLen > bbmsa::kTableLen) c->wideTableLen = bbmsa::kTableLen;
    c->tableLen = (c->tableLen + 3) & ~3; c->wideTableLen = (c->wideTableLen + 3) & ~3;
    c->ldsBytes = (bbmsa::lds_table_ints(c->tableLen) + 4 * jobsPerWave * perJobInts) * 4;
    if (c->ldsBytes > 160 * 1024) return bbfail(BBMAP_E_ARG, "bbmsa_create: fast-path LDS budget exceeded; lower reserved[1] (fastCols)");

    c->sw.banded = !(cfg->bandwidth < 1 && cfg->bandwidthRatio <= 0.0f);
    const void *kfn = bbmsa::fast_kernel_for(c->R, c->sw.banded);
    if (!kfn) return bbfail(BBMAP_E_ARG, "bbmsa_create: no kernel for this rows-per-lane");
    if (c->ldsBytes > 64 * 1024) {
        BBHIP(hipFuncSetAttribute(kfn, hipFuncAttributeMaxDynamicSharedMemorySize, c->ldsBytes));
        BBHIP(hipFuncSetAttribute(bbmsa::fast_kernel_unl_for(c->R), hipFuncAttributeMaxDynamicSharedMemorySize, c->ldsBytes));
    }
    int blocksPerCU = 0;
    BBHIP(hipOccupancyMaxActiveBlocksPerMultiprocessor(&blocksPerCU, kfn, 256, c->ldsBytes));
    if (blocksPerCU < 1) blocksPerCU = 1;
    const int capBlocks = env_int("BBMSA_BLOCKS_PER_CU", 0);
    if (capBlocks > 0 && capBlocks < blocksPerCU) blocksPerCU = capBlocks;
    c->blocks = c->numCUs * blocksPerCU;

    const int maxSteps = fastCols + G - 1;
    c->dirSlotDwords = (long long)((maxSteps >> 3) + 1) * c->R * G;
    const long long slots = (long long)c->blocks * 4 * jobsPerWave;
    BBHIP(hipMalloc(&c->d_dir, (size_t)(slots * c->dirSlotDwords * 4)));

    int threads = 0;
    BBTRY(generic_threads(*cfg, 2048, 16384, &threads));
    BBTRY(alloc_generic_scratch(c, threads));
    if (cfg->maxColumns > fastCols) BBTRY(setup_wide_pass(c));
    c->narrowSlack = env_int("BBMSA_NARROW_SLACK", 2000);
    if (!c->sw.banded && env_int("BBMSA_NARROW", 1) != 0) {
        int perCU = 0;
        c->bandRows = cfg->maxRows < 256 ? cfg->maxRows : 256;
        c->bandLds = bbmsa::band_lds_bytes(c->tableLen, c->bandRows);
        if (c->bandLds > 64 * 1024) BBHIP(hipFuncSetAttribute(bbmsa::band_kernel(), hipFuncAttributeMaxDynamicSharedMemorySize, c->bandLds));
        BBHIP(hipOccupancyMaxActiveBlocksPerMultiprocessor(&perCU, bbmsa::band_kernel(), 256, c->bandLds));
        c->narrowBlocks = c->numCUs * clamp_occupancy(perCU, 4);
        c->sw.bandPresent = true;
        BBHIP(hipMalloc(&c->d_bandDir, (size_t)c->narrowBlocks * 4 * (size_t)(c->bandRows + 1) * 128 * 4));
    }
    c->sw.sortByWidth = env_int("BBMSA_SORT_BY_WIDTH", 0) != 0;
    c->sw.sortWithBand = env_int("BBMSA_SORT_WITH_BAND", 0) != 0;
    c->sw.wideUnlimited = env_int("BBMSA_WIDE_UNLIMITED", 0) != 0;
    c->sw.unlimitedLoop = env_int("BBMSA_UNLIMITED_LOOP", 1) != 0;
    c->unlimitedStats = env_int("BBMSA_UNLIMITED_STATS", 0) != 0 || getenv("BBMAP_DP_COUNTS") != nullptr;
    { const int lat = env_int("BBMSA_LATENCY_JOBS", 0); if (lat > 0) BBTRY(bbmsa_set_latency_jobs(c, lat)); }
    return BBMAP_OK;
}

extern "C" int bbmsa_create(const bbmsa_config *cfg, bbmsa_ctx **out) {
    if (!cfg || !out) return bbfail(BBMAP_E_ARG, "bbmsa_create: null argument");
    *out = nullptr;
    const int scheme = cfg->reserved[2] & 0xFF;
    const bool legacyOnly = (cfg->reserved[2] & BBMSA_LEGACY_ONLY) != 0;
    if (scheme != BBMSA_SCHEME_11TS && scheme != BBMSA_SCHEME_9PACBIO) return bbfail(BBMAP_E_ARG, "bbmsa_create: unknown scoring scheme");
    if (scheme == BBMSA_SCHEME_11TS && (cfg->maxRows < 1 || cfg->maxRows > 640 || cfg->maxColumns < 1 || cfg->maxColumns > 4096))
        return bbfail(BBMAP_E_ARG, "bbmsa_create: maxRows must be 1..640 and maxColumns 1..4096");
    if (scheme == BBMSA_SCHEME_9PACBIO && (cfg->maxRows < 1 || cfg->maxRows > 6100 || cfg->maxColumns < 1 || cfg->maxColumns > 8192))
        return bbfail(BBMAP_E_ARG, "bbmsa_create: the PacBio scheme takes maxRows 1..6100 and maxColumns 1..8192");
    hipDeviceProp_t prop;
    BBTRY(bb_use_gfx950("bbmsa_create", cfg->device, &prop));

    bbmsa_ctx *c = new (std::nothrow) bbmsa_ctx();
    if (!c) return bbfail(BBMAP_E_NOMEM, "bbmsa_create: out of host memory");
    c->cfg = *cfg;
    c->device = cfg->device;
    c->numCUs = prop.multiProcessorCount;
    c->sw.scheme = scheme;
    c->legacyOnly = legacyOnly;
    struct Guard { bbmsa_ctx *c; ~Guard() { if (c) bbmsa_destroy(c); } } guard{c};
    BBTRY(legacyOnly ? create_legacy_only(c) : scheme != BBMSA_SCHEME_11TS ? create_pacbio(c) : create_11ts(c));
    BBHIP(hipMalloc(&c->d_counters, bbmsa::kCounterBytes));
    BBHIP(hipMemset(c->d_counters, 0, bbmsa::kCounterBytes));
    for (int i = 0; i < 4; i++) BBHIP(hipEventCreate(&c->ev[i]));
    guard.c = nullptr;
    *out = c;
    return BBMAP_OK;
}

extern "C" void bbmsa_destroy(bbmsa_ctx *c) {
    if (!c) return;
    (void)hipSetDevice(c->device);
    bbmsa_legacy_destroy(c);
    if (c->d_dir) (void)hipFree(c->d_dir);
    if (c->d_counters) (void)hipFree(c->d_counters);
    if (c->d_widthHist) (void)hipFree(c->d_widthHist);
    for (DevBuf *b : {&c->slowList, &c->slowList2, &c->fastList, &c->gref, &c->gaux, &c->gjobs}) b->release();
    if (c->d_matrix) (void)hipFree(c->d_matrix);
    if (c->d_limits) (void)hipFree(c->d_limits);
    if (c->d_wideDir) (void)hipFree(c->d_wideDir);
    if (c->d_bandDir) (void)hipFree(c->d_bandDir);
    if (c->d_stripBoundary) (void)hipFree(c->d_stripBoundary);
    if (c->d_stripTmp) (void)hipFree(c->d_stripTmp);
    if (c->d_pipeBoundary) (void)hipFree(c->d_pipeBoundary);
    if (c->d_pipeSync) (void)hipFree(c->d_pipeSync);
    for (int i = 0; i < 4; i++) if (c->ev[i]) (void)hipEventDestroy(c->ev[i]);
    delete c;
}

extern "C" int bbmsa_align_batch_device(bbmsa_ctx *c, void *stream_, int64_t n_jobs,
                                        const bbmsa_job *jobs, const uint8_t *reads, const uint8_t *refs,
                                        bbmsa_result *results, uint8_t *match, int32_t match_stride) {
    return bbmsa_align_impl(c, stream_, n_jobs, nullptr, jobs, reads, refs, results, match, match_stride);
}

extern "C" int bbmsa_align_batch_device_indirect(bbmsa_ctx *c, void *stream_, const uint32_t *n_jobs_dev, int64_t max_jobs,
                                                 const bbmsa_job *jobs, const uint8_t *reads, const uint8_t *refs,
                                                 bbmsa_result *results, uint8_t *match, int32_t match_stride) {
    if (!n_jobs_dev) return bbfail(BBMAP_E_ARG, "bbmsa_align_batch_device_indirect: null counter");
    return bbmsa_align_impl(c, stream_, max_jobs, n_jobs_dev, jobs, reads, refs, results, match, match_stride);
}

namespace {
using namespace bbmsa;

template <class S> int launch_generic(bbmsa_ctx *c, const JobBatch &B, hipStream_t stream, const int *list, const unsigned int *count) {
    bbmsa::GenericParams gp;
    set_batch(gp, c, B);
    gp.list = list; gp.list_count = count;
    gp.matrix = c->d_matrix; gp.limits = c->d_limits; gp.queue = c->d_counters + CNT_GENERIC_QUEUE;
    hipLaunchKernelGGL(bbmsa::msa_fill_generic_kernel<S>, dim3(c->genThreads / 64), dim3(64), 0, stream, gp);
    BBHIP(hipGetLastError());
    BBHIP(hipEventRecord(c->ev[2], stream));
    c->timed = true;
    return BBMAP_OK;
}

int launch_strip(bbmsa_ctx *c, const JobBatch &B, const Route &r, hipStream_t stream) {
    bbmsa::StripParams sp;
    set_batch(sp, c, B);
    sp.queue = c->d_counters + CNT_FAST_QUEUE; sp.dirbuf = c->d_dir; sp.dir_slot_dwords = c->stripSlotDwords; sp.dir_strip_dwords = c->stripDwords;
    sp.boundary = c->d_stripBoundary; sp.tmpbuf = c->d_stripTmp; sp.slow_list = c->slowList.as<int>(); sp.slow_count = c->d_counters + CNT_SLOW_COUNT;
    sp.pipeK = 0; sp.pipeSlots = 0; sp.pipeBoundary = nullptr; sp.pipeSync = nullptr;
    sp.pipeSpinLimit = env_int("BBMSA_PIPE_SPIN_LIMIT", 1 << 21);
    if (sp.pipeSpinLimit < 1) sp.pipeSpinLimit = 1;
    void *sargs[] = {&sp};
    if (r.pipelined) {
        const long long slots = r.jobs < c->pipeSlots ? r.jobs : c->pipeSlots;
        sp.pipeK = c->pipeK; sp.pipeSlots = (int)slots; sp.pipeBoundary = c->d_pipeBoundary; sp.pipeSync = c->d_pipeSync;
        BBHIP(hipMemsetAsync(c->d_pipeSync, 0, (size_t)(slots * bbmsa::strip_pipe_sync_ints(c->pipeK) * 4), stream));
        BBHIP(hipLaunchKernel(bbmsa::strip_kernel_pacbio_pipelined(), dim3((unsigned)(slots * c->pipeK)), dim3(64), sargs, (size_t)c->stripLds, stream));
        return BBMAP_OK;
    }
    const long long sblocks = r.jobs < c->stripBlocks ? r.jobs : c->stripBlocks;
    BBHIP(hipLaunchKernel(bbmsa::strip_kernel_pacbio(), dim3((unsigned)sblocks), dim3(64), sargs, (size_t)c->stripLds, stream));
    return BBMAP_OK;
}

int launch_band(bbmsa_ctx *c, const JobBatch &B, const Route &r, hipStream_t stream) {
    int *const fastList = c->fastList.as<int>();
    bbmsa::NarrowParams np;
    set_batch(np, c, B);
    np.queue = c->d_counters + CNT_BAND_QUEUE; np.fast_list = fastList; np.fast_count = c->d_counters + CNT_LIST_COUNT;
    np.stats = c->d_counters + CNT_BAND_STATS; np.maxSlack = c->narrowSlack;
    np.dirbuf32 = c->d_bandDir; np.tableLen = c->tableLen; np.bandRows = c->bandRows;
    np.list = r.sorted ? fastList + 2 * r.jobs : nullptr; np.list_count = r.sorted ? c->d_counters + CNT_CAND_COUNT : nullptr;
    long long nb = (r.jobs + 63) / 64;
    if (nb > c->narrowBlocks) nb = c->narrowBlocks;
    void *nargs[] = {&np};
    BBHIP(hipLaunchKernel(bbmsa::band_kernel(), dim3((unsigned)nb), dim3(256), nargs, (size_t)c->bandLds, stream));
    return BBMAP_OK;
}

bbmsa::FillParams first_pass_params(const bbmsa_ctx *c, const JobBatch &B, const Route &r) {
    bbmsa::FillParams fp = {};
    set_batch(fp, c, B);
    fp.queue = c->d_counters + CNT_FAST_QUEUE; fp.dirbuf = c->d_dir; fp.dir_slot_dwords = c->dirSlotDwords;
    fp.list = (r.band || r.sorted) ? c->fastList.as<int>() : nullptr; fp.list_count = c->d_counters + CNT_LIST_COUNT; fp.priority = 0;
    fp.slow_list = c->slowList.as<int>(); fp.slow_count = c->d_counters + CNT_SLOW_COUNT;
    fp.lanesPerJob = c->G; fp.fastCols = c->fastCols; fp.tmpBytes = c->tmpBytes; fp.tableLen = c->tableLen;
    fp.unl_stats = c->unlimitedStats ? c->d_counters + CNT_UNL_STATS : nullptr;
    return fp;
}

int launch_unlimited(bbmsa_ctx *c, const bbmsa::FillParams &fp, const Route &r, long long blocks, hipStream_t stream) {
    bbmsa::FillParams up = fp;
    up.queue = c->d_counters + CNT_UNL_QUEUE; up.list = c->fastList.as<int>() + r.jobs; up.list_count = c->d_counters + CNT_UNL_LIST_COUNT;
    void *uargs[] = {&up};
    BBHIP(hipLaunchKernel(bbmsa::fast_kernel_unl_for(c->R), dim3((unsigned)blocks), dim3(256), uargs, (size_t)c->ldsBytes, stream));
    return BBMAP_OK;
}

int launch_wide(bbmsa_ctx *c, const bbmsa::FillParams &fp, const Route &r, hipStream_t stream) {
    bbmsa::FillParams wp = fp;
    wp.queue = c->d_counters + CNT_WIDE_QUEUE; wp.dirbuf = c->d_wideDir; wp.dir_slot_dwords = c->wideDirSlotDwords;
    wp.list = r.latency ? nullptr : fp.slow_list; wp.list_count = r.latency ? nullptr : fp.slow_count;
    wp.slow_list = c->slowList2.as<int>(); wp.slow_count = c->d_counters + CNT_WIDE_SLOW_COUNT;
    wp.lanesPerJob = 64; wp.fastCols = c->wideCols; wp.tmpBytes = c->wideTmpBytes; wp.tableLen = c->wideTableLen;
    static const int widePrio = env_int("BBMSA_WIDE_PRIORITY", 2);
    wp.priority = widePrio;
    void *wargs[] = {&wp};
    const long long wblocks = r.latency && r.jobs < c->wideBlocks ? r.jobs : c->wideBlocks;
    const void *bothFn = r.wideBoth ? bbmsa::fast_kernel_both_for(c->wideR) : nullptr;
    BBHIP(hipLaunchKernel(bothFn ? bothFn : bbmsa::fast_kernel_for(c->wideR, c->sw.banded), dim3((unsigned)wblocks), dim3(64), wargs, (size_t)c->wideLdsBytes, stream));
    return BBMAP_OK;
}
}

int bbmsa_align_impl(bbmsa_ctx *c, void *stream_, int64_t n_jobs, const uint32_t *n_jobs_dev,
                     const bbmsa_job *jobs, const uint8_t *reads, const uint8_t *refs,
                     bbmsa_result *results, uint8_t *match, int32_t match_stride) {
    if (!c) return bbfail(BBMAP_E_ARG, "bbmsa_align_batch_device: null context");
    if (n_jobs < 0 || n_jobs > 0x7fffffffLL) return bbfail(BBMAP_E_ARG, "bbmsa_align_batch_device: n_jobs out of range");
    if (n_jobs == 0) return BBMAP_OK;
    if (!jobs || !reads || !refs || !results) return bbfail(BBMAP_E_ARG, "bbmsa_align_batch_device: null buffer");
    if (match && match_stride < 1) return bbfail(BBMAP_E_ARG, "bbmsa_align_batch_device: match_stride must be positive");
    hipStream_t stream = (hipStream_t)stream_;
    BBHIP(hipSetDevice(c->device));
    if (c->legacyOnly) return bbfail(BBMAP_E_ARG, "bbmsa_align_batch_device: this context was created for bbmsa_fill_packed only (BBMSA_LEGACY_ONLY)");
    const JobBatch B = {n_jobs, n_jobs_dev, jobs, reads, refs, results, match, match_stride};
    const Route r = plan_route(c->sw, n_jobs, n_jobs_dev != nullptr);
    const size_t listBytes = (size_t)n_jobs * 4;
    BBHIP(c->slowList.grow(listBytes, 0, &stream));
    if (r.wide) BBHIP(c->slowList2.grow(listBytes, 0, &stream));
    if (c->sw.bandPresent || r.sorted) BBHIP(c->fastList.grow(r.sorted ? 3 * listBytes : listBytes, 0, &stream));
    BBHIP(hipMemsetAsync(c->d_counters, 0, bbmsa::kCounterBytes, stream));
    c->last = r;
    BBHIP(hipEventRecord(c->ev[0], stream));
    if (c->sw.scheme != BBMSA_SCHEME_11TS) {
        BBHIP(hipEventRecord(c->ev[3], stream));
        BBTRY(launch_strip(c, B, r, stream));
        BBHIP(hipEventRecord(c->ev[1], stream));
        return launch_generic<bbmsa::Scheme9PacBio>(c, B, stream, c->slowList.as<int>(), c->d_counters + CNT_SLOW_COUNT);
    }
    if (r.sorted) BBTRY(bbmsa_width_sort(c, stream, jobs, n_jobs, r.band));
    if (r.band) BBTRY(launch_band(c, B, r, stream));
    BBHIP(hipEventRecord(c->ev[3], stream));
    bbmsa::FillParams fp = first_pass_params(c, B, r);
    const int jobsPerBlock = 4 * (64 / c->G);
    long long blocks = (n_jobs + jobsPerBlock - 1) / jobsPerBlock;
    if (blocks > c->blocks) blocks = c->blocks;
    if (r.unlList) BBTRY(launch_unlimited(c, fp, r, blocks, stream));
    void *args[] = {&fp};
    if (!r.latency)
        BBHIP(hipLaunchKernel(bbmsa::fast_kernel_for(c->R, c->sw.banded), dim3((unsigned)blocks), dim3(256), args, (size_t)c->ldsBytes, stream));
    if (r.wide) BBTRY(launch_wide(c, fp, r, stream));
    BBHIP(hipEventRecord(c->ev[1], stream));
    return launch_generic<bbmsa::Scheme11ts>(c, B, stream, r.wide ? c->slowList2.as<int>() : fp.slow_list,
                                             c->d_counters + (r.wide ? CNT_WIDE_SLOW_COUNT : CNT_SLOW_COUNT));
}

void bbmsa_use_narrow(bbmsa_ctx *c, bool on) { if (c) c->sw.bandOff = !on; }
void bbmsa_sort_by_width(bbmsa_ctx *c, bool on) { if (c) c->sw.sortByWidth = on; }
void bbmsa_sort_with_band(bbmsa_ctx *c, bool on) { if (c) c->sw.sortWithBand = on; }
void bbmsa_set_wide_unlimited(bbmsa_ctx *c, bool on) { if (c) c->sw.wideUnlimited = on; }
int bbmsa_set_latency_jobs(bbmsa_ctx *c, int64_t n) {
    if (!c || c->sw.scheme != BBMSA_SCHEME_11TS || c->legacyOnly) return BBMAP_OK;
    BBHIP(hipSetDevice(c->device));
    if (n > 0) BBTRY(setup_wide_pass(c));
    if (n > 0 && !c->slowList2.p) BBHIP(c->slowList2.grow(c->slowList.cap));
    c->sw.latencyJobs = c->sw.widePresent ? n : 0;
    return BBMAP_OK;
}
int bbmsa_wait_first_pass(bbmsa_ctx *c, void *waiter) {
    if (!c || !c->timed) return BBMAP_OK;
    BBHIP(hipStreamWaitEvent((hipStream_t)waiter, c->ev[3], 0));
    return BBMAP_OK;
}

extern "C" int bbmsa_last_kernel_ms(bbmsa_ctx *c, float *ms_fast, float *ms_slow) {
    if (!c || !c->timed) return bbfail(BBMAP_E_ARG, "bbmsa_last_kernel_ms: nothing launched yet");
    BBHIP(hipSetDevice(c->device));
    BBHIP(hipEventSynchronize(c->ev[2]));
    float a = 0, b = 0;
    BBHIP(hipEventElapsedTime(&a, c->ev[0], c->ev[1]));
    BBHIP(hipEventElapsedTime(&b, c->ev[1], c->ev[2]));
    if (ms_fast) *ms_fast = a;
    if (ms_slow) *ms_slow = b;
    return BBMAP_OK;
}

extern "C" int bbmsa_last_kernel_ms3(bbmsa_ctx *c, float *ms3) {
    if (!c || !c->timed || !ms3) return bbfail(BBMAP_E_ARG, "bbmsa_last_kernel_ms3: nothing launched yet");
    BBHIP(hipSetDevice(c->device));
    BBHIP(hipEventSynchronize(c->ev[2]));
    BBHIP(hipEventElapsedTime(&ms3[0], c->ev[0], c->ev[3]));
    BBHIP(hipEventElapsedTime(&ms3[1], c->ev[3], c->ev[1]));
    BBHIP(hipEventElapsedTime(&ms3[2], c->ev[1], c->ev[2]));
    return BBMAP_OK;
}

static int read_counters(bbmsa_ctx *c, unsigned (&h)[bbmsa::kCounterWords]) {
    BBHIP(hipSetDevice(c->device));
    BBHIP(hipEventSynchronize(c->ev[2]));
    BBHIP(hipMemcpy(h, c->d_counters, sizeof h, hipMemcpyDeviceToHost));
    return BBMAP_OK;
}

extern "C" int bbmsa_last_counts(bbmsa_ctx *c, int64_t *counts4) {
    if (!c || !c->timed || !counts4) return bbfail(BBMAP_E_ARG, "bbmsa_last_counts: nothing launched yet");
    unsigned h[bbmsa::kCounterWords];
    BBTRY(read_counters(c, h));
    const Route &r = c->last;
    counts4[0] = h[CNT_BAND_DONE]; counts4[1] = h[CNT_BAND_HANDED];
    counts4[2] = r.band ? (r.sorted ? h[CNT_SORTED_COUNT] + h[CNT_UNL_LIST_COUNT] : h[CNT_LIST_COUNT]) : 0;
    counts4[3] = r.wide ? h[CNT_WIDE_SLOW_COUNT] : h[CNT_SLOW_COUNT];
    if (getenv("BBMAP_DP_COUNTS")) {
        if (r.wide) fprintf(stderr, "   (first pass handed %u jobs to the wide pass)\n", h[CNT_SLOW_COUNT]);
        if (r.sorted) fprintf(stderr, "   (sorted: %u general, %u unlimited, %u band candidates)\n", h[CNT_SORTED_COUNT], h[CNT_UNL_LIST_COUNT], h[CNT_CAND_COUNT]);
        fprintf(stderr, "   (the wavefronts ran %u steps)\n", h[CNT_WAVE_STEPS]);
    }
    return BBMAP_OK;
}

extern "C" int bbmsa_debug_sorted_lists(bbmsa_ctx *c, int64_t n_jobs, int32_t *lists3, int64_t *lens3) {
    if (!c || !c->timed || !lists3 || !lens3) return bbfail(BBMAP_E_ARG, "bbmsa_debug_sorted_lists: nothing launched yet");
    if (!c->last.sorted || n_jobs != c->last.jobs) return bbfail(BBMAP_E_ARG, "bbmsa_debug_sorted_lists: the last launch was not a sorted launch of n_jobs jobs");
    unsigned h[bbmsa::kCounterWords];
    BBTRY(read_counters(c, h));
    const unsigned len[3] = {h[CNT_SORTED_COUNT], h[CNT_UNL_LIST_COUNT], h[CNT_CAND_COUNT]};
    for (int k = 0; k < 3; k++) {
        if ((int64_t)len[k] > n_jobs) return bbfail(BBMAP_E_HIP, "bbmsa_debug_sorted_lists: a list is longer than the launch");
        lens3[k] = len[k];
        if (len[k]) BBHIP(hipMemcpy(lists3 + (size_t)k * (size_t)n_jobs, c->fastList.as<int>() + (size_t)k * (size_t)n_jobs, (size_t)len[k] * 4, hipMemcpyDeviceToHost));
    }
    return BBMAP_OK;
}

extern "C" int bbmsa_last_unlimited(bbmsa_ctx *c, int64_t *counts4) {
    if (!c || !c->timed || !counts4) return bbfail(BBMAP_E_ARG, "bbmsa_last_unlimited: nothing launched yet");
    const bool wave = c->sw.scheme == BBMSA_SCHEME_11TS && !c->legacyOnly;
    if (wave && !c->unlimitedStats) return bbfail(BBMAP_E_ARG, "bbmsa_last_unlimited: the context does not count (create it with BBMSA_UNLIMITED_STATS=1 in the environment)");
    unsigned h[bbmsa::kCounterWords];
    BBTRY(read_counters(c, h));
    counts4[0] = wave ? h[CNT_UNL_RAN_UNL] : 0; counts4[1] = wave ? h[CNT_UNL_RAN_GENERAL] : 0;
    counts4[2] = wave ? h[CNT_UNL_STEPS] : 0; counts4[3] = wave ? h[CNT_ALL_STEPS] : 0;
    return BBMAP_OK;
}

int bbmsa_last_route_flags(const bbmsa_ctx *c) {
    if (!c || !c->timed) return 0;
    return (c->last.band ? BBMSA_ROUTE_NARROW : 0) | (c->last.sorted ? BBMSA_ROUTE_SORTED : 0) | (c->last.latency ? BBMSA_ROUTE_LATENCY : 0);
}

extern "C" int bbmsa_last_route(bbmsa_ctx *c, int64_t *route8) {
    if (!c || !c->timed || !route8) return bbfail(BBMAP_E_ARG, "bbmsa_last_route: nothing launched yet");
    unsigned h[bbmsa::kCounterWords];
    BBTRY(read_counters(c, h));
    const Route &r = c->last;
    route8[0] = r.band; route8[1] = r.sorted; route8[2] = r.latency; route8[3] = r.wide; route8[4] = r.indirect;
    route8[5] = h[CNT_SLOW_COUNT]; route8[6] = r.wide ? h[CNT_WIDE_SLOW_COUNT] : 0; route8[7] = r.band ? h[CNT_BAND_DONE] : 0;
    return BBMAP_OK;
}

extern "C" int bbmsa_geometry(bbmsa_ctx *c, int32_t *geo4) {
    if (!c || !geo4) return bbfail(BBMAP_E_ARG, "bbmsa_geometry: null argument");
    geo4[0] = geo4[1] = geo4[2] = geo4[3] = 0;
    if (c->legacy) {
        int last = 0, mask = 0;
        bbmsa_legacy_rows_per_lane(c, &last, &mask);
        geo4[0] = 64; geo4[1] = last; geo4[2] = c->cfg.maxColumns; geo4[3] = mask;
    } else if (c->sw.scheme == BBMSA_SCHEME_11TS) {
        geo4[0] = c->G; geo4[1] = c->R; geo4[2] = c->fastCols; geo4[3] = c->wideBlocks > 0 ? c->wideR : 0;
    }
    return BBMAP_OK;
}

extern "C" int bbmsa_align_batch(bbmsa_ctx *c, int64_t n_jobs, const bbmsa_job *jobs,
                                 const uint8_t *reads, int64_t reads_bytes,
                                 const uint8_t *refs, int64_t refs_bytes,
                                 bbmsa_result *results, uint8_t *match, int32_t match_stride) {
    if (!c) return bbfail(BBMAP_E_ARG, "bbmsa_align_batch: null context");
    if (n_jobs == 0) return BBMAP_OK;
    if (n_jobs < 0 || !jobs || !reads || !refs || !results || reads_bytes < 0 || refs_bytes < 0)
        return bbfail(BBMAP_E_ARG, "bbmsa_align_batch: bad argument");
    BBHIP(hipSetDevice(c->device));
    for (int64_t i = 0; i < n_jobs; i++) {
        const bbmsa_job &j = jobs[i];
        if (j.read_len < 0 || j.read_off < 0 || j.read_off + j.read_len > reads_bytes)
            return bbfail(BBMAP_E_ARG, "bbmsa_align_batch: a read lies outside the reads buffer");
        if (j.ref_len < 0 || j.ref_off < 0 || j.ref_off + j.ref_len > refs_bytes)
            return bbfail(BBMAP_E_ARG, "bbmsa_align_batch: a reference array lies outside the refs buffer");
        if (!(j.flags & BBMSA_CLAMP_WINDOW) && (j.refStartLoc < 0 || j.refEndLoc >= j.ref_len))
            return bbfail(BBMAP_E_ARG, "bbmsa_align_batch: window outside its reference array (set BBMSA_CLAMP_WINDOW to clamp)");
    }
    DevTmp<bbmsa_job> d_jobs; DevTmp<uint8_t> d_reads, d_refs, d_match; DevTmp<bbmsa_result> d_res;
    BBTRY(d_jobs.upload(jobs, (size_t)n_jobs));
    BBTRY(d_reads.upload(reads, (size_t)reads_bytes));
    BBTRY(d_refs.upload(refs, (size_t)refs_bytes));
    BBTRY(d_res.alloc((size_t)n_jobs));
    if (match) BBTRY(d_match.alloc((size_t)n_jobs * (size_t)match_stride));
    BBHIP(hipMemset(d_res, 0xff, (size_t)n_jobs * sizeof(bbmsa_result)));
    BBTRY(bbmsa_align_batch_device(c, nullptr, n_jobs, d_jobs, d_reads, d_refs, d_res, d_match, match_stride));
    BBHIP(hipStreamSynchronize(nullptr));
    BBHIP(hipMemcpy(results, d_res, (size_t)n_jobs * sizeof(bbmsa_result), hipMemcpyDeviceToHost));
// ... 4 lines not shown
```

### bbmap_amd/csrc/msa_route.h

```cpp
#pragma once
#include "bbmap_amd.h"

struct RouteSwitches {
    int scheme = 0;
    bool banded = false;
    bool bandPresent = false;
    bool bandOff = false;
    bool sortByWidth = false;
    bool sortWithBand = false;
    bool unlimitedLoop = true;
    bool wideUnlimited = false;
    bool widePresent = false;
    long long latencyJobs = 0;
    int pipeJobsMax = 0;
};

struct Route {
    bool band = false;
    bool sorted = false;
    bool latency = false;
    bool indirect = false;
    bool wide = false;
    bool unlList = false;
    bool wideBoth = false;
    bool pipelined = false;
    long long jobs = 0;
};

inline Route plan_route(const RouteSwitches &s, long long n_jobs, bool indirect) {
    Route r;
    r.indirect = indirect; r.jobs = n_jobs;
    if (s.scheme != BBMSA_SCHEME_11TS) {
        r.pipelined = !indirect && s.pipeJobsMax > 0 && n_jobs <= s.pipeJobsMax;
        return r;
    }
    r.band = s.bandPresent && !s.bandOff;
    r.wide = s.widePresent;
    r.sorted = s.sortByWidth && !indirect && n_jobs >= 256 && n_jobs > s.latencyJobs && (!r.band || s.sortWithBand);
    r.latency = r.wide && !indirect && !r.band && n_jobs <= s.latencyJobs;
    r.unlList = r.sorted && s.unlimitedLoop;
    r.wideBoth = s.wideUnlimited && !s.banded;
    return r;
}
```

### bbmap_amd/csrc/msa_sort.hip

```cpp
#include <hip/hip_runtime.h>

#include "host_common.h"
#include "msa_common.h"
#include "msa_ctx.h"

namespace bbmsa {
constexpr int WIDTH_PER_CLASS = 512;
constexpr int WIDTH_CLASSES = 3;
constexpr int WIDTH_BUCKETS = WIDTH_CLASSES * WIDTH_PER_CLASS;
enum { CLASS_UNLIMITED = 0, CLASS_CANDIDATE = 1, CLASS_GENERAL = 2 };
constexpr int SORT_THREADS = 256, SORT_JOBS_PER_THREAD = 4;
struct SortKey { int maxRows, maxColumns, bandwidth; float bandwidthRatio; int byKind, band, bandRows, maxSlack; };
__device__ inline int job_width_bucket(const bbmsa_job &t, const SortKey k) {
    int a = t.refStartLoc, b = t.refEndLoc;
    if (t.flags & BBMSA_CLAMP_WINDOW) { a = max(0, a); b = min(t.ref_len - 1, b); if (b - a >= k.maxColumns) b = min(t.ref_len - 1, a + k.maxColumns - 1); }
    const int cols = max(0, b - a + 1);
    int cls = CLASS_GENERAL;
    if (k.band && band_is_candidate(t.flags, t.minScore, t.read_len, b - a + 1, k.maxRows, k.maxColumns, k.bandRows, k.maxSlack)) cls = CLASS_CANDIDATE;
    else if (k.byKind && !fill_is_limited(t.flags, t.minScore, t.read_len, b - a + 1, fill_halfband(t.read_len, b - a + 1, k.bandwidth, k.bandwidthRatio))) cls = CLASS_UNLIMITED;
    constexpr int W = WIDTH_PER_CLASS;
    return cls * W + W - 1 - min(W - 1, cols >> 3);
}
__global__ __launch_bounds__(SORT_THREADS) void width_hist_kernel(const bbmsa_job *jobs, long long n, SortKey key, unsigned *hist) {
    __shared__ unsigned s[WIDTH_BUCKETS];
    for (int i = threadIdx.x; i < WIDTH_BUCKETS; i += SORT_THREADS) s[i] = 0;
    __syncthreads();
    const long long base = (long long)blockIdx.x * (SORT_THREADS * SORT_JOBS_PER_THREAD) + threadIdx.x;
#pragma unroll
    for (int k = 0; k < SORT_JOBS_PER_THREAD; k++) {
        const long long i = base + (long long)k * SORT_THREADS;
        if (i < n) atomicAdd(&s[job_width_bucket(jobs[i], key)], 1u);
    }
    __syncthreads();
    for (int i = threadIdx.x; i < WIDTH_BUCKETS; i += SORT_THREADS) { const unsigned v = s[i]; if (v) atomicAdd(&hist[i], v); }
}
__global__ void width_scan_kernel(unsigned *hist, unsigned *listCount, unsigned *sortedCount, unsigned *unlCount, unsigned *candCount) {
    __shared__ unsigned s[WIDTH_PER_CLASS];
    const int t = threadIdx.x;
    for (int cls = 0; cls < WIDTH_CLASSES; cls++) {
        const unsigned own = hist[cls * WIDTH_PER_CLASS + t];
        s[t] = own;
        __syncthreads();
        for (int d = 1; d < WIDTH_PER_CLASS; d <<= 1) { const unsigned v = t >= d ? s[t - d] : 0u; __syncthreads(); s[t] += v; __syncthreads(); }
        hist[cls * WIDTH_PER_CLASS + t] = s[t] - own;
        if (t == WIDTH_PER_CLASS - 1) {
            if (cls == CLASS_UNLIMITED) *unlCount = s[t];
            else if (cls == CLASS_CANDIDATE) *candCount = s[t];
            else { *listCount = s[t]; *sortedCount = s[t]; }
        }
        __syncthreads();
    }
}
__global__ __launch_bounds__(SORT_THREADS) void width_scatter_kernel(const bbmsa_job *jobs, long long n, SortKey key, unsigned *cursor, int *list, int *unlList, int *candList) {
    __shared__ unsigned s[WIDTH_BUCKETS];
    for (int i = threadIdx.x; i < WIDTH_BUCKETS; i += SORT_THREADS) s[i] = 0;
    __syncthreads();
    const long long base = (long long)blockIdx.x * (SORT_THREADS * SORT_JOBS_PER_THREAD) + threadIdx.x;
    int bucket[SORT_JOBS_PER_THREAD]; unsigned rank[SORT_JOBS_PER_THREAD];
#pragma unroll
    for (int k = 0; k < SORT_JOBS_PER_THREAD; k++) {
        const long long i = base + (long long)k * SORT_THREADS;
        bucket[k] = -1; rank[k] = 0;
        if (i < n) { bucket[k] = job_width_bucket(jobs[i], key); rank[k] = atomicAdd(&s[bucket[k]], 1u); }
    }
    __syncthreads();
    for (int i = threadIdx.x; i < WIDTH_BUCKETS; i += SORT_THREADS) { const unsigned v = s[i]; if (v) s[i] = atomicAdd(&cursor[i], v); }
    __syncthreads();
#pragma unroll
    for (int k = 0; k < SORT_JOBS_PER_THREAD; k++) {
        if (bucket[k] < 0) continue;
        const long long i = base + (long long)k * SORT_THREADS;
        const unsigned pos = s[bucket[k]] + rank[k];
        if ((long long)pos >= n) continue;
        const int cls = bucket[k] / WIDTH_PER_CLASS;
        (cls == CLASS_UNLIMITED ? unlList : (cls == CLASS_CANDIDATE ? candList : list))[pos] = (int)i;
    }
}
}

int bbmsa_width_sort(bbmsa_ctx *c, hipStream_t stream, const bbmsa_job *jobs, int64_t n_jobs, bool band) {
    using namespace bbmsa;
    if (!c->d_widthHist) BBHIP(hipMalloc(&c->d_widthHist, WIDTH_BUCKETS * 4));
    BBHIP(hipMemsetAsync(c->d_widthHist, 0, WIDTH_BUCKETS * 4, stream));
    const int perBlock = SORT_THREADS * SORT_JOBS_PER_THREAD;
    const unsigned sb = (unsigned)((n_jobs + perBlock - 1) / perBlock);
    const SortKey key = {c->cfg.maxRows, c->cfg.maxColumns, c->cfg.bandwidth, c->cfg.bandwidthRatio, c->sw.unlimitedLoop ? 1 : 0,
                         band ? 1 : 0, c->bandRows, c->narrowSlack};
    int *const list = c->fastList.as<int>();
    unsigned *const cnt = c->d_counters;
    hipLaunchKernelGGL(width_hist_kernel, dim3(sb), dim3(SORT_THREADS), 0, stream, jobs, (long long)n_jobs, key, c->d_widthHist);
    hipLaunchKernelGGL(width_scan_kernel, dim3(1), dim3(WIDTH_PER_CLASS), 0, stream, c->d_widthHist, cnt + CNT_LIST_COUNT, cnt + CNT_SORTED_COUNT,
                       cnt + CNT_UNL_LIST_COUNT, cnt + CNT_CAND_COUNT);
    hipLaunchKernelGGL(width_scatter_kernel, dim3(sb), dim3(SORT_THREADS), 0, stream, jobs, (long long)n_jobs, key, c->d_widthHist,
                       list, list + n_jobs, list + 2 * n_jobs);
    BBHIP(hipGetLastError());
    return BBMAP_OK;
}
```

### bbmap_amd/mapper.py

```python
import ctypes as C

import numpy as np
import torch

from . import _lib
from . import msa as M
from .index import READ_DTYPE, read_lens

MSITE_DTYPE = np.dtype([("chrom", "<i4"), ("strand", "<i4"), ("start", "<i4"), ("stop", "<i4"), ("hits", "<i4"),
                        ("quickScore", "<i4"), ("score", "<i4"), ("slowScore", "<i4"), ("pairedScore", "<i4"),
                        ("perfect", "<i4"), ("semiperfect", "<i4"), ("rescued", "<i4"), ("ngaps", "<i4"),
                        ("gaps", "<i4", (16,)), ("match_job", "<i4"), ("reserved", "<i4", (2,))])
JOBINFO_DTYPE = np.dtype([("read", "<i4"), ("seq", "<i4"), ("kind", "<i4"), ("site", "<i4")])
FINAL_DTYPE = np.dtype([("mapped", "<i4"), ("chrom", "<i4"), ("strand", "<i4"), ("start", "<i4"), ("stop", "<i4"), ("mapScore", "<i4"),
                        ("paired", "<i4"), ("ambiguous", "<i4"), ("perfect", "<i4"), ("rescued", "<i4"), ("match_len", "<i4"),
                        ("nsites", "<i4"), ("match_off", "<i8"), ("reserved", "<i4", (2,))])
SCAFREC_DTYPE = np.dtype([("scaffold", "<i4"), ("start", "<i4"), ("stop", "<i4"), ("pos", "<i4"), ("end", "<i4"), ("scaflen", "<i4"),
                          ("flags", "<i4"), ("reserved", "<i4")])
SCAF_MAPPED, SCAF_PAIRED, SCAF_INBOUNDS, SCAF_SAME_SCAFFOLD = 1, 2, 4, 8
SAMREC_DTYPE = np.dtype([("flag", "<i4"), ("mapq", "<i4"), ("rname", "<i4"), ("rnext", "<i4"), ("pos", "<i4"), ("pnext", "<i4"),
                         ("tlen", "<i4"), ("nm", "<i4"), ("am", "<i4"), ("tags", "<i4"), ("cigar_off", "<i8"), ("cigar_len", "<i4"),
                         ("md_len", "<i4"), ("md_off", "<i8")])
SAM_CIGAR13, SAM_MD = 1, 2
SAM_TAG_XT = 1
SAMTAGS_DTYPE = np.dtype([(n, "<i4") for n in ("present", "xs", "nh", "sm", "xm", "ys", "yl_query", "yl_ref", "yi_good", "yi_bad",
                                               "yi_perfect", "yr", "x8", "xb", "introns", "splices")])
from .sam import (MAKE_AM as SAM_MAKE_AM, MAKE_BOUNDS as SAM_MAKE_BOUNDS, MAKE_IDENTITY as SAM_MAKE_IDENTITY,
                  MAKE_INSERT as SAM_MAKE_INSERT, MAKE_LENGTH as SAM_MAKE_LENGTH, MAKE_NH as SAM_MAKE_NH, MAKE_NM as SAM_MAKE_NM,
                  MAKE_SCORE as SAM_MAKE_SCORE, MAKE_SM as SAM_MAKE_SM, MAKE_STOP as SAM_MAKE_STOP, MAKE_XM as SAM_MAKE_XM,
                  MAKE_XS as SAM_MAKE_XS, NO_TAGS as SAM_NO_TAGS, XS_SECONDSTRAND as SAM_XS_SECONDSTRAND)
SAM_DEFAULT_TAGS = SAM_MAKE_NM | SAM_MAKE_AM
SAM_ALL_TAGS = (SAM_DEFAULT_TAGS | SAM_MAKE_SM | SAM_MAKE_XM | SAM_MAKE_XS | SAM_MAKE_NH | SAM_MAKE_STOP | SAM_MAKE_LENGTH |
                SAM_MAKE_IDENTITY | SAM_MAKE_SCORE | SAM_MAKE_INSERT | SAM_MAKE_BOUNDS)
SAM_NO_INTRON_LIMIT = 2 ** 31 - 1
GAPPED_BIT = 1 << 30


class bbmap_config(C.Structure):
    _fields_ = [("device", C.c_int32), ("paired", C.c_int32), ("max_reads", C.c_int32), ("max_read_len", C.c_int32),
                ("max_sites", C.c_int32), ("minRatio", C.c_float)] + [(n, C.c_int32) for n in (
                    "slowAlignPadding", "slowRescuePadding", "extraPadding", "tipSearchDist", "maxPairDist", "averagePairDist",
                    "maxRescueDist", "maxRescueMismatches", "maxTrimSitesToRetain", "trimList", "doRescue", "alignColumns",
                    "clearzone3", "msaMaxColumns", "fastCols", "jobsPerRead", "finalStage")] + [("reserved", C.c_int32 * 4)]


class bbmap_sam_config(C.Structure):
    _fields_ = [("flags", C.c_int32), ("intronLimit", C.c_int32), ("tags", C.c_int32), ("reserved", C.c_int32 * 5)]


def sam_config(flags=0, intron_limit=None, tags=None):
    return bbmap_sam_config(int(flags), SAM_NO_INTRON_LIMIT if intron_limit is None else int(intron_limit),
                            SAM_DEFAULT_TAGS if tags is None else int(tags))


class bbmap_output(C.Structure):
    _fields_ = [("sites", C.c_void_p), ("nsites", C.c_void_p), ("cap", C.c_int32), ("match_stride", C.c_int32),
                ("gmatch_stride", C.c_int32), ("reserved", C.c_int32), ("n_jobs", C.c_int64), ("n_gapped_jobs", C.c_int64),
                ("jobs", C.c_void_p), ("results", C.c_void_p), ("jobinfo", C.c_void_p), ("match", C.c_void_p),
                ("gjobs", C.c_void_p), ("gresults", C.c_void_p), ("gjobinfo", C.c_void_p), ("gmatch", C.c_void_p),
                ("ggaps", C.c_void_p), ("final", C.c_void_p), ("final_match", C.c_void_p), ("final_match_bytes", C.c_int64),
                ("n_final_fills", C.c_int64)]


class bbmap_stats(C.Structure):
    _fields_ = [(n, C.c_int64) for n in ("reads", "reads_overflowed", "reads_without_site", "fills", "gapped_fills", "refills",
                                         "rescue_scans", "rescue_fills", "rounds", "fills_dropped")] + \
               [(n, C.c_float) for n in ("ms_probe", "ms_begin", "ms_score", "ms_slow", "ms_finish", "ms_rescue", "ms_total",
                                         "ms_dp_narrow", "ms_dp_wave", "ms_dp_generic", "ms_dp_gapped", "ms_quick_rescue")] + \
               [("probe_stats", C.c_int64 * 5), ("reads_reprobed", C.c_int64), ("ms_overflow", C.c_float), ("log_growths", C.c_float),
                ("ms_dp_wave_max", C.c_float), ("ms_final", C.c_float), ("final_fills", C.c_int64), ("final_rounds", C.c_int64),
                ("final_local", C.c_int64), ("dp_narrow_launches", C.c_int64), ("dp_sorted_launches", C.c_int64),
                ("sites_cross_scaffold", C.c_int64)]


class bbmap_overflow_output(C.Structure):
    _fields_ = [("n_reads", C.c_int64), ("read_ids", C.c_void_p), ("out", bbmap_output)]


NSITES_OVERFLOW, NSITES_MATE_OVERFLOW, NSITES_IN_TIER = -1, -2, -3


def sam_workspace_bytes(n_reads, max_read_len):
    L = _lib.load()
    b = L.bbpipe_sam_records_workspace_bytes(int(n_reads), int(max_read_len))
    if b < 0:
        _lib.check(int(b), "bbpipe_sam_records_workspace_bytes")
    return int(b)


def sam_records_device(reads, bases, finals, pool, scaf, recs, text, text_bytes, workspace, paired=False, flags=0, intron_limit=None,
                       tags=None, tagrecs=None, sites=None, nsites=None, cap=0, chrom_arr=None, chrom_arr_len=None, max_read_len=600):
    L = _lib.load()
    n = reads.numel() // READ_DTYPE.itemsize
    cfg = sam_config(flags, intron_limit, tags)
    ptr = lambda t: None if t is None else C.c_void_p(t.data_ptr())
    stream = torch.cuda.current_stream().cuda_stream
    _lib.check(L.bbpipe_sam_records_device(C.c_void_p(stream), n, int(bool(paired)), C.byref(cfg), int(max_read_len), ptr(reads), ptr(bases),
                                           ptr(finals), ptr(pool), ptr(scaf), ptr(sites), ptr(nsites), int(cap), ptr(chrom_arr),
                                           ptr(chrom_arr_len), ptr(recs), ptr(tagrecs), ptr(text), int(text.numel()), ptr(text_bytes),
                                           ptr(workspace), int(workspace.numel())), "bbpipe_sam_records_device")


def _copy(ptr, nbytes, dev=None):
    out = np.empty(max(nbytes, 0), np.uint8)
    if nbytes > 0:
        L = _lib.load()
        _lib.check(L.bbmap_copy_to_host(out.ctypes.data, C.c_void_p(ptr), nbytes), "bbmap_copy_to_host")
    return out


class Mapper:

    def _open(self, di, n, read_len, paired, device, max_sites, cfg_kw, profile=None):
        self.L = _lib.load()
        self.di, self.n, self.read_len, self.paired = di, n, read_len, paired
        self.dev = torch.device("cuda", device)
        cfg = bbmap_config()
        if profile is None:
            max_len = read_len
            _lib.check(self.L.bbmap_default_config(C.byref(cfg)), "bbmap_default_config")
        else:
            max_len = max(1, read_len)
            _lib.check(self.L.bbmap_default_config_profile(profile, C.byref(cfg)), "bbmap_default_config_profile")
        if not profile:
            di.set_max_read_len(max_len)
# ... 383 lines not shown
```

### bbmap_amd/msa.py

```python
import ctypes as C

import numpy as np

from . import _lib
from ._lib import bbmsa_config, bbmsa_job, bbmsa_result

FILL_LIMITED_RAW = 0
FILL_UNLIMITED_RAW = 1
FILL_LIMITED = 2
CLAMP_WINDOW = 1 << 3
DO_SCORE = 1 << 4
DO_TRACEBACK = 1 << 5
NO_ITERATIONS = 1 << 6
TRACE_KEEP_GAPS = 1 << 7
FILL_AND_SCORE_LIMITED = FILL_LIMITED | CLAMP_WINDOW | DO_SCORE

ST_OK, ST_NULL, ST_BAD_SHAPE = 0, 1, 2

JOB_DTYPE, RESULT_DTYPE = np.dtype(bbmsa_job), np.dtype(bbmsa_result)
GAPS_DTYPE = np.dtype([("ngaps", "<i4"), ("gaps", "<i4", (16,))])


class bbmsa_ticket(C.Structure):
    _fields_ = [("batch", C.c_int32), ("slot", C.c_int32), ("gen", C.c_int64), ("rows", C.c_int32), ("columns", C.c_int32)]
# ... 80 lines not shown
    def align_batch_device(self, n_jobs, jobs_ptr, reads_ptr, refs_ptr, results_ptr, match_ptr=0,
                           match_stride=0, stream=0):
        rc = self.L.bbmsa_align_batch_device(self.h, C.c_void_p(stream), n_jobs, C.c_void_p(jobs_ptr),
                                             C.c_void_p(reads_ptr), C.c_void_p(refs_ptr),
                                             C.c_void_p(results_ptr),
                                             C.c_void_p(match_ptr) if match_ptr else None, match_stride)
        _lib.check(rc, "bbmsa_align_batch_device")

    def align_batch_device_indirect(self, n_jobs_ptr, max_jobs, jobs_ptr, reads_ptr, refs_ptr, results_ptr, match_ptr=0,
                                    match_stride=0, stream=0):
        rc = self.L.bbmsa_align_batch_device_indirect(self.h, C.c_void_p(stream), C.c_void_p(n_jobs_ptr), max_jobs,
                                                      C.c_void_p(jobs_ptr), C.c_void_p(reads_ptr), C.c_void_p(refs_ptr),
                                                      C.c_void_p(results_ptr),
                                                      C.c_void_p(match_ptr) if match_ptr else None, match_stride)
        _lib.check(rc, "bbmsa_align_batch_device_indirect")

    def align_gapped_batch_device(self, n_jobs, jobs_ptr, gaps_ptr, reads_ptr, refs_ptr, results_ptr, match_ptr=0,
                                  match_stride=0, stream=0):
        rc = self.L.bbmsa_align_gapped_batch_device(self.h, C.c_void_p(stream), n_jobs, C.c_void_p(jobs_ptr), C.c_void_p(gaps_ptr),
                                                    C.c_void_p(reads_ptr), C.c_void_p(refs_ptr), C.c_void_p(results_ptr),
                                                    C.c_void_p(match_ptr) if match_ptr else None, match_stride)
        _lib.check(rc, "bbmsa_align_gapped_batch_device")

    def align_gapped_batch_device_indirect(self, n_jobs_ptr, max_jobs, jobs_ptr, gaps_ptr, reads_ptr, refs_ptr, results_ptr,
                                           match_ptr=0, match_stride=0, stream=0):
        rc = self.L.bbmsa_align_gapped_batch_device_indirect(self.h, C.c_void_p(stream), C.c_void_p(n_jobs_ptr), max_jobs,
                                                             C.c_void_p(jobs_ptr), C.c_void_p(gaps_ptr), C.c_void_p(reads_ptr),
                                                             C.c_void_p(refs_ptr), C.c_void_p(results_ptr),
                                                             C.c_void_p(match_ptr) if match_ptr else None, match_stride)
        _lib.check(rc, "bbmsa_align_gapped_batch_device_indirect")

    def last_route(self):
        r = (C.c_int64 * 8)()
        _lib.check(self.L.bbmsa_last_route(self.h, r), "bbmsa_last_route")
        return {"narrow": bool(r[0]), "sorted": bool(r[1]), "latency": bool(r[2]), "wide_pass": bool(r[3]), "indirect": bool(r[4]),
                "first_handed_on": r[5], "wide_handed_on": r[6], "narrow_finished": r[7]}

    def last_unlimited(self):
        c = (C.c_int64 * 4)()
        _lib.check(self.L.bbmsa_last_unlimited(self.h, c), "bbmsa_last_unlimited")
        return {"stripped": c[0], "general": c[1], "unlimited_steps": c[2], "steps": c[3]}

    def geometry(self):
        g = (C.c_int32 * 4)()
        _lib.check(self.L.bbmsa_geometry(self.h, g), "bbmsa_geometry")
        if self.legacy:
            return {"lanes": g[0], "rows_per_lane": g[1], "columns": g[2], "launched": {r for r in range(1, 32) if g[3] >> r & 1}}
        return {"lanes": g[0], "rows_per_lane": g[1], "fast_cols": g[2], "wide_rows_per_lane": g[3]}

    def last_counts(self):
        c = (C.c_int64 * 4)()
        _lib.check(self.L.bbmsa_last_counts(self.h, c), "bbmsa_last_counts")
        return {"narrow": c[0], "narrow_left": c[1], "wave": c[2], "generic": c[3]}

    def debug_sorted_lists(self, n_jobs):
        lists = np.full((3, n_jobs), -1, np.int32)
        lens = (C.c_int64 * 3)()
        _lib.check(self.L.bbmsa_debug_sorted_lists(self.h, n_jobs, lists.ctypes.data, lens), "bbmsa_debug_sorted_lists")
        return {"general": lists[0, :lens[0]].copy(), "unlimited": lists[1, :lens[1]].copy(), "candidates": lists[2, :lens[2]].copy()}

    def last_kernel_ms3(self):
        m = (C.c_float * 3)()
        _lib.check(self.L.bbmsa_last_kernel_ms3(self.h, m), "bbmsa_last_kernel_ms3")
        return m[0], m[1], m[2]

    def last_kernel_ms(self):
        a, b = C.c_float(), C.c_float()
        _lib.check(self.L.bbmsa_last_kernel_ms(self.h, C.byref(a), C.byref(b)), "bbmsa_last_kernel_ms")
        return a.value, b.value


def pack_problems(problems, flags):
    reads, refs, jobs = bytearray(), bytearray(), []
    ref_cache = {}
    for k, (read, ref, a, b, ms) in enumerate(problems):
        ro = len(reads)
        reads += bytes(read)
        key = id(ref)
        if key not in ref_cache:
            ref_cache[key] = len(refs)
            refs += bytes(ref)
        fo = ref_cache[key]
        fl = flags[k] if isinstance(flags, (list, tuple, np.ndarray)) else flags
        jobs.append((ro, fo, len(read), len(ref), a, b, ms, fl))
    jobs = np.array(jobs, dtype=JOB_DTYPE) if jobs else np.zeros(0, JOB_DTYPE)
    return jobs, np.frombuffer(bytes(reads) or b"\0", np.uint8), np.frombuffer(bytes(refs) or b"\0", np.uint8)


class MultiStateAligner11ts:

    def __init__(self, maxRows=601, maxColumns=3000, bandwidth=0, bandwidthRatio=0.0, device=0, **kw):
        self.ctx = MSAContext(maxRows, maxColumns, bandwidth, bandwidthRatio, device, **kw)
        self.maxRows, self.maxColumns = maxRows, maxColumns
        self.iterationsLimited = 0
        self.iterationsUnlimited = 0

    def _run(self, problems, flags, want_match=False):
        problems = list(problems)
        jobs, reads, refs = pack_problems(problems, flags)
        stride = 0
        if want_match and problems:
            stride = max(len(p[0]) + (p[3] - p[2] + 1) + 8 +
                         127 * bytes(p[1][max(0, p[2]):max(0, p[3] + 1)]).count(b"-") for p in problems)
            stride = (stride + 15) & ~15
        res, match = self.ctx.align_batch(jobs, reads, refs, stride)
        for r in res:
# ... 57 lines not shown
```

### include/bbmap_amd.h

```cpp
#ifndef BBMAP_AMD_H
#define BBMAP_AMD_H

#include <stdint.h>

#ifdef __cplusplus
extern "C" {
#endif

#define BBMAP_AMD_ABI_VERSION 6

enum {
    BBMAP_OK = 0,
    BBMAP_E_NODEVICE = -1,
    BBMAP_E_ARG = -2,
    BBMAP_E_NOMEM = -3,
    BBMAP_E_HIP = -4,
    BBMAP_E_SHAPE = -5
};

const char *bbmap_last_error(void);
int bbmap_abi_version(void);


enum {
// ... 48 lines not shown
    float   bandwidthRatio;
    int32_t reserved[3];
} bbmsa_config;

#define BBMSA_SCHEME_11TS 0
#define BBMSA_SCHEME_9PACBIO 1
#define BBMSA_LEGACY_ONLY 0x100

int bbmsa_create(const bbmsa_config *cfg, bbmsa_ctx **out);
void bbmsa_destroy(bbmsa_ctx *ctx);

int bbmsa_align_batch_device(bbmsa_ctx *ctx, void *stream, int64_t n_jobs,
                             const bbmsa_job *jobs, const uint8_t *reads, const uint8_t *refs,
                             bbmsa_result *results, uint8_t *match, int32_t match_stride);

int bbmsa_align_batch_device_indirect(bbmsa_ctx *ctx, void *stream, const uint32_t *n_jobs_dev, int64_t max_jobs,
                                      const bbmsa_job *jobs, const uint8_t *reads, const uint8_t *refs,
                                      bbmsa_result *results, uint8_t *match, int32_t match_stride);

int bbmsa_align_batch(bbmsa_ctx *ctx, int64_t n_jobs, const bbmsa_job *jobs,
                      const uint8_t *reads, int64_t reads_bytes,
                      const uint8_t *refs, int64_t refs_bytes,
                      bbmsa_result *results, uint8_t *match, int32_t match_stride);

typedef struct bbmsa_ticket {
    int32_t batch, slot;
    int64_t gen;
    int32_t rows, columns;
} bbmsa_ticket;
int bbmsa_fill_submit(bbmsa_ctx *ctx, const uint8_t *read, int32_t read_len, const uint8_t *ref, int32_t ref_len,
                      int32_t refStartLoc, int32_t refEndLoc, int32_t minScore, int32_t mode,
                      int32_t *result5, int64_t *iterations, bbmsa_ticket *ticket);
int bbmsa_fill_collect(bbmsa_ctx *ctx, bbmsa_ticket *ticket, int32_t *packed, int32_t *vertLimit, int32_t *horizLimit);
int bbmsa_fill_packed(bbmsa_ctx *ctx, const uint8_t *read, int32_t read_len, const uint8_t *ref, int32_t ref_len,
                      int32_t refStartLoc, int32_t refEndLoc, int32_t minScore, int32_t mode,
                      int32_t *result5, int64_t *iterations, int32_t *packed);
int bbmsa_legacy_stats(bbmsa_ctx *ctx, int64_t *stats6);

#define BBMSA_MAX_GAPS 16
typedef struct bbmsa_gaps { int32_t ngaps; int32_t gaps[BBMSA_MAX_GAPS]; } bbmsa_gaps;
int bbmsa_align_gapped_batch_device(bbmsa_ctx *ctx, void *stream, int64_t n_jobs, const bbmsa_job *jobs,
                                    const bbmsa_gaps *gaps, const uint8_t *reads, const uint8_t *refs,
                                    bbmsa_result *results, uint8_t *match, int32_t match_stride);
int bbmsa_align_gapped_batch_device_indirect(bbmsa_ctx *ctx, void *stream, const uint32_t *n_jobs_dev, int64_t max_jobs,
                                             const bbmsa_job *jobs, const bbmsa_gaps *gaps, const uint8_t *reads,
                                             const uint8_t *refs, bbmsa_result *results, uint8_t *match, int32_t match_stride);
int bbmsa_align_gapped_batch(bbmsa_ctx *ctx, int64_t n_jobs, const bbmsa_job *jobs, const bbmsa_gaps *gaps,
                             const uint8_t *reads, int64_t reads_bytes, const uint8_t *refs, int64_t refs_bytes,
                             bbmsa_result *results, uint8_t *match, int32_t match_stride);

int bbmsa_last_kernel_ms(bbmsa_ctx *ctx, float *ms_fast, float *ms_slow);
int bbmsa_last_kernel_ms3(bbmsa_ctx *ctx, float *ms3);
int bbmsa_last_counts(bbmsa_ctx *ctx, int64_t *counts4);
int bbmsa_debug_sorted_lists(bbmsa_ctx *ctx, int64_t n_jobs, int32_t *lists3, int64_t *lens3);
int bbmsa_last_route(bbmsa_ctx *ctx, int64_t *route8);
int bbmsa_last_unlimited(bbmsa_ctx *ctx, int64_t *counts4);
int bbmsa_geometry(bbmsa_ctx *ctx, int32_t *geo4);

enum {
    BBBAND_FORWARD = 0, BBBAND_FORWARD_RC = 1, BBBAND_REVERSE = 2, BBBAND_REVERSE_RC = 3,
    BBBAND_DIR_MASK = 3,
    BBBAND_EXACT = 1 << 2
};
enum {
    BBBAND_SEMANTICS_JNI_C = 0,
    BBBAND_SEMANTICS_JAVA = 1
};

typedef struct bbband_job {
    int64_t query_off;
    int64_t ref_off;
    int32_t query_len;
    int32_t ref_len;
    int32_t qstart;
    int32_t rstart;
    int32_t maxEdits;
    int32_t flags;
} bbband_job;

typedef struct bbband_result {
    int32_t edits;
    int32_t lastQueryLoc;
    int32_t lastRefLoc;
    int32_t lastRow;
    int32_t lastEdits;
    int32_t lastOffset;
    int32_t status;
    int32_t reserved;
} bbband_result;

typedef struct bbband_ctx bbband_ctx;
typedef struct bbband_config {
    int32_t device;
    int32_t width;
    int32_t semantics;
    int32_t reserved;
} bbband_config;

int bbband_create(const bbband_config *cfg, bbband_ctx **out);
void bbband_destroy(bbband_ctx *ctx);
int bbband_align_batch_device(bbband_ctx *ctx, void *stream, int64_t n_jobs, const bbband_job *jobs,
                              const uint8_t *seqs, bbband_result *results);
int bbband_align_batch(bbband_ctx *ctx, int64_t n_jobs, const bbband_job *jobs,
                       const uint8_t *seqs, int64_t seq_bytes, bbband_result *results);

typedef struct bbband_pair { int64_t query_off, ref_off; int32_t query_len, ref_len; } bbband_pair;
// ... 245 lines not shown
    int32_t trimList;
    int32_t doRescue;
    int32_t alignColumns;
    int32_t clearzone3;
    int32_t msaMaxColumns;
    int32_t fastCols;
    int32_t jobsPerRead;
    int32_t finalStage;
    int32_t reserved[4];
} bbmap_config;

typedef struct bbmap_final {
    int32_t mapped;
    int32_t chrom, strand, start, stop;
    int32_t mapScore;
    int32_t paired, ambiguous, perfect, rescued;
    int32_t match_len;
    int32_t nsites;
    int64_t match_off;
    int32_t reserved[2];
} bbmap_final;

typedef struct bbmap_output {
    const bbmap_msite *sites;
    const int32_t *nsites;
    int32_t cap;
    int32_t match_stride, gmatch_stride;
    int32_t reserved;
    int64_t n_jobs, n_gapped_jobs;
    const bbmsa_job *jobs;   const bbmsa_result *results;  const bbmap_jobinfo *jobinfo;  const uint8_t *match;
    const bbmsa_job *gjobs;  const bbmsa_result *gresults; const bbmap_jobinfo *gjobinfo; const uint8_t *gmatch;
    const bbmsa_gaps *ggaps;
    const bbmap_final *final;
    const uint8_t *final_match;
    int64_t final_match_bytes;
    int64_t n_final_fills;
} bbmap_output;

typedef struct bbmap_stats {
    int64_t reads, reads_overflowed, reads_without_site, fills, gapped_fills, refills, rescue_scans, rescue_fills, rounds;
    int64_t fills_dropped;
    float ms_probe, ms_begin, ms_score, ms_slow, ms_finish, ms_rescue, ms_total;
    float ms_dp_narrow, ms_dp_wave, ms_dp_generic, ms_dp_gapped, ms_quick_rescue;
    int64_t probe_stats[5];
    int64_t reads_reprobed;
    float ms_overflow;
    float log_growths;
    float ms_dp_wave_max;
    float ms_final;
    int64_t final_fills, final_rounds, final_local;
    int64_t dp_narrow_launches;
    int64_t dp_sorted_launches;
    int64_t sites_cross_scaffold;
} bbmap_stats;

typedef struct bbmap_ctx bbmap_ctx;
int bbmap_default_config(bbmap_config *cfg);
int bbmap_default_config_profile(int32_t profile, bbmap_config *cfg);
int bbmap_create(bbidx_ctx *index, const bbmap_config *cfg, bbmap_ctx **out);
void bbmap_destroy(bbmap_ctx *ctx);
int bbmap_set_average_pair_dist(bbmap_ctx *ctx, int32_t average_pair_dist);
int bbmap_map_batch_device(bbmap_ctx *ctx, void *stream, int64_t n_reads, const bbidx_read *reads, uint8_t *bases,
                           int64_t minus_delta, const int8_t *baseScores, const int32_t *keyinfo);
int bbmap_get_output(bbmap_ctx *ctx, bbmap_output *out);
int bbmap_final_batch_device(bbmap_ctx *ctx, void *stream, int64_t n_reads, const bbidx_read *reads, uint8_t *bases, int64_t minus_delta,
                             const bbmap_msite *sites, const int32_t *nsites);
int bbmap_map_batch(bbmap_ctx *ctx, int64_t n_reads, const bbidx_read *reads, const uint8_t *bases, int64_t bases_bytes,
                    const int8_t *baseScores, const int32_t *keyinfo, int64_t keyinfo_ints, int32_t *nsites_out,
                    int64_t *offsets_out, bbmap_msite *sites_out, int64_t sites_cap, int64_t *total_out);
typedef struct bbmap_overflow_output {
    int64_t n_reads;
    const int32_t *read_ids;
    bbmap_output out;
} bbmap_overflow_output;
int bbmap_get_overflow_output(bbmap_ctx *ctx, bbmap_overflow_output *out);
int bbmap_get_final(bbmap_ctx *ctx, int64_t n_reads, bbmap_final *out, uint8_t *match_out, int64_t match_cap, int64_t *match_bytes);
int bbmap_untrim_batch_device(bbmap_ctx *ctx, void *stream, const bbidx_read *reads_untrimmed, const bbtrim_rec *trims);
enum { BBMAP_SCAF_MAPPED = 1,
       BBMAP_SCAF_PAIRED = 2,
       BBMAP_SCAF_INBOUNDS = 4,
       BBMAP_SCAF_SAME_SCAFFOLD = 8 };
typedef struct bbmap_scafrec {
    int32_t scaffold;
    int32_t start, stop;
    int32_t pos, end;
    int32_t scaflen;
    int32_t flags;
    int32_t reserved;
} bbmap_scafrec;
int bbmap_get_scaffold_records(bbmap_ctx *ctx, void *stream, const bbmap_scafrec **out);
enum { BBMAP_SAM_CIGAR13 = 1,
       BBMAP_SAM_MD = 2 };
enum { BBMAP_SAM_TAG_XT = 1 };
typedef struct bbmap_samrec {
    int32_t flag, mapq;
    int32_t rname;
    int32_t rnext;
    int32_t pos, pnext, tlen;
    int32_t nm;
    int32_t am;
    int32_t tags;
    int64_t cigar_off;
    int32_t cigar_len;
    int32_t md_len;
    int64_t md_off;
} bbmap_samrec;
// ... 319 lines not shown
```

Baseline: 10.44 million.

## Add wider banded fill stage for rescue and final alignment jobs

```diff
diff --git a/bbmap_amd/csrc/mapper_ctx.h b/bbmap_amd/csrc/mapper_ctx.h
--- a/bbmap_amd/csrc/mapper_ctx.h
+++ b/bbmap_amd/csrc/mapper_ctx.h
@@ -15,6 +15,9 @@
 
 enum { ACC_STATS, ACC_COV, ACC_HIST, ACC_SPLIT, ACC_COUNT };
 struct Accum { bool counted = false; hipStream_t stream = nullptr; };
+
+enum FillStage { FILLS_SLOW = 0, FILLS_RESCUE = 1, FILLS_FINAL = 2 };
+enum { WIDE_BAND_MAY = (1 << FILLS_RESCUE) | (1 << FILLS_FINAL), WIDE_BAND_DEFAULT = WIDE_BAND_MAY };
 
 struct bbmap_ctx {
     bbmap_config cfg;
@@ -48,6 +51,7 @@
     bool ownsMsa;
     long long narrowMinJobs;
     bool sortWide;
+    int wideBandStages;
     bool sortPlain;
     bool classSwap;
     bool classOrder;
diff --git a/bbmap_amd/csrc/mapper_host.hip b/bbmap_amd/csrc/mapper_host.hip
--- a/bbmap_amd/csrc/mapper_host.hip
+++ b/bbmap_amd/csrc/mapper_host.hip
@@ -138,6 +138,7 @@
     c->narrowMinJobs = getenv("BBMAP_NARROW_MIN_JOBS") ? atoll(getenv("BBMAP_NARROW_MIN_JOBS")) : 32768;
     c->sortWide = !(getenv("BBMAP_SORT_WIDE") && atoi(getenv("BBMAP_SORT_WIDE")) == 0);
     c->sortPlain = !(getenv("BBMAP_SORT_PLAIN") && atoi(getenv("BBMAP_SORT_PLAIN")) == 0);
+    c->wideBandStages = getenv("BBMAP_WIDE_BAND") ? (atoi(getenv("BBMAP_WIDE_BAND")) & WIDE_BAND_MAY) : WIDE_BAND_DEFAULT;
     c->classOrder = !(getenv("BBMAP_CLASS_ORDER") && atoi(getenv("BBMAP_CLASS_ORDER")) == 0);
     c->classSwap = getenv("BBMAP_CLASS_ORDER") && atoi(getenv("BBMAP_CLASS_ORDER")) == 2;
     c->kernargDev = !(getenv("BBMAP_KERNARG_DEV") && atoi(getenv("BBMAP_KERNARG_DEV")) == 0);
@@ -274,10 +275,11 @@
 }
 
 static int run_fills(bbmap_ctx *c, hipStream_t stream, const uint8_t *bases, long long jobBase, long long nNew, long long gBase, long long gNew,
-                     bool finalStage = false) {
+                     FillStage stage) {
     bbmsa_use_narrow(c->msa, nNew >= c->narrowMinJobs);
     bbmsa_sort_by_width(c->msa, c->sortPlain && nNew >= c->narrowMinJobs);
     bbmsa_sort_with_band(c->msa, c->sortPlain);
+    bbmsa_set_wide_band(c->msa, (c->wideBandStages >> stage) & 1);
     if (c->msaGapped != c->msa) { bbmsa_use_narrow(c->msaGapped, false); bbmsa_sort_by_width(c->msaGapped, c->sortWide); }
     hipStream_t gs = (c->dpStream && nNew > 0) ? c->dpStream : stream;
     if (gNew > 0) {
@@ -293,6 +295,7 @@
     const int r2 = gNew > 0 ? bbmsa_last_route_flags(c->msaGapped) : 0;
     c->stats.dp_narrow_launches += (r1 & 1) + (r2 & 1);
     c->stats.dp_sorted_launches += ((r1 >> 1) & 1) + ((r2 >> 1) & 1);
+    c->stats.dp_wide_band_launches += (r1 >> 3) & 1;
     if (gNew > 0 && gs != stream) BBHIP(hipStreamWaitEvent(stream, c->evJoin, 0));
     return BBMAP_OK;
 }
@@ -302,6 +305,10 @@
     if (plain && bbmsa_last_kernel_ms3(c->msa, k3) == BBMAP_OK) { c->stats.ms_dp_narrow += k3[0]; c->stats.ms_dp_wave += k3[1]; c->stats.ms_dp_generic += k3[2];
                                                                  if (k3[1] > c->stats.ms_dp_wave_max) c->stats.ms_dp_wave_max = k3[1]; }
     if (gapped && c->msaGapped != c->msa && bbmsa_last_kernel_ms3(c->msaGapped, k3) == BBMAP_OK) c->stats.ms_dp_gapped += k3[0] + k3[1] + k3[2];
+    int64_t w4[4];
+    if (plain && (bbmsa_last_route_flags(c->msa) & BBMSA_ROUTE_WIDE_BAND) && bbmsa_last_wide_band(c->msa, w4) == BBMAP_OK) {
+        c->stats.dp_wide_band_finished += w4[2]; c->stats.dp_wide_band_handed += w4[3];
+    }
     static const bool show = getenv("BBMAP_DP_COUNTS") != nullptr;
     if (show) {
         int64_t n4[4], u4[4];
@@ -339,7 +346,7 @@
     add_dp_ms(c, R.ranPlain, R.ranGapped);
     const long long asked = c->h_counters[CNT_FILLS], gasked = c->h_counters[CNT_GAPPED_FILLS];
     const long long total = asked < c->jobCap ? asked : c->jobCap, gtotal = gasked < c->gjobCap ? gasked : c->gjobCap;
-    BBTRY(run_fills(c, stream, bases, R.jobBase, total - R.jobBase, R.gBase, gtotal - R.gBase, R.finalStage));
+    BBTRY(run_fills(c, stream, bases, R.jobBase, total - R.jobBase, R.gBase, gtotal - R.gBase, R.finalStage ? FILLS_FINAL : FILLS_SLOW));
     R.ranPlain = total > R.jobBase; R.ranGapped = gtotal > R.gBase;
     R.jobBase = total; R.gBase = gtotal;
     if (asked > c->jobCap || gasked > c->gjobCap) BBTRY(grow_logs(c, stream, D, asked, gasked, total, gtotal));
@@ -497,7 +504,7 @@
             { float ms = 0; if (hipEventElapsedTime(&ms, q0, q1) == hipSuccess) c->stats.ms_quick_rescue += ms; }
             const long long total = c->h_counters[CNT_FILLS], gtotal = c->h_counters[CNT_GAPPED_FILLS];
             if (total > c->jobCap || gtotal > c->gjobCap) return bbfail(BBMAP_E_HIP, "bbmap_map_batch_device: rescue fills beyond the reserved log entries (internal error)");
-            BBTRY(run_fills(c, stream, bases, jobBase, total - jobBase, gBase, gtotal - gBase));
+            BBTRY(run_fills(c, stream, bases, jobBase, total - jobBase, gBase, gtotal - gBase, FILLS_RESCUE));
             const bool ranPlain = total > jobBase, ranGapped = gtotal > gBase;
             jobBase = total; gBase = gtotal;
             BBTRY(launch<128>(rescue_finish_kernel, pairs, stream, D));
@@ -560,6 +567,7 @@
     st.final_fills += ts.final_fills; st.final_local += ts.final_local;
     st.dp_narrow_launches += ts.dp_narrow_launches; st.dp_sorted_launches += ts.dp_sorted_launches;
     st.sites_cross_scaffold += ts.sites_cross_scaffold;
+    st.dp_wide_band_launches += ts.dp_wide_band_launches; st.dp_wide_band_finished += ts.dp_wide_band_finished; st.dp_wide_band_handed += ts.dp_wide_band_handed;
     if (getenv("BBMAP_TIER_DEBUG"))
         fprintf(stderr, "[bbmap tier] reads %lld: probe %.2f begin %.2f score %.2f slow %.2f (rounds %lld) finish %.2f rescue %.2f total %.2f\n",
                 tn, ts.ms_probe, ts.ms_begin, ts.ms_score, ts.ms_slow, (long long)ts.rounds, ts.ms_finish, ts.ms_rescue, ts.ms_total);
diff --git a/bbmap_amd/csrc/msa_common.h b/bbmap_amd/csrc/msa_common.h
--- a/bbmap_amd/csrc/msa_common.h
+++ b/bbmap_amd/csrc/msa_common.h
@@ -124,6 +124,18 @@
         tmin -= 120;
     }
     return (70 + 100 * (rows - 1)) - tmin <= maxSlack;
+}
+
+__host__ __device__ inline bool wide_band_is_candidate(int flags, int minScore, int rows, int columns, int maxRows, int maxColumns, int bandRows, int maxSlack, int wideSlack) {
+    const int mode = flags & BBMSA_MODE_MASK;
+    if (!(rows >= 16 && columns >= rows && rows <= maxRows && rows <= bandRows && columns <= maxColumns && mode != BBMSA_FILL_UNLIMITED_RAW)) return false;
+    int tmin = minScore;
+    if (mode == BBMSA_FILL_LIMITED) {
+        if (tmin < 1 || (columns + rows < 90) || (columns > rows + min(170, rows + 20))) return false;
+        tmin -= 120;
+    }
+    const long long slack = (long long)(70 + 100 * (rows - 1)) - tmin;
+    return slack > maxSlack && 100LL * ((columns - rows) / 2) + slack <= wideSlack;
 }
 
 __device__ inline long long job_count(long long njobs, const unsigned int *njobs_dev) {
@@ -152,18 +164,24 @@
     CNT_CAND_COUNT = 15,
     CNT_SORTED_COUNT = 16,
     CNT_WAVE_STEPS = 17,
-};
-constexpr int CNT_BAND_STATS = 5, CNT_UNL_STATS = 9;
+    CNT_WBAND_QUEUE = 18,
+    CNT_WCAND_COUNT = 19,
+    CNT_WBAND_DONE = 20,
+    CNT_WBAND_HANDED = 21,
+};
+constexpr int CNT_BAND_STATS = 5, CNT_WBAND_STATS = 20, CNT_UNL_STATS = 9;
 enum BandStat { BAND_STAT_DONE = 0, BAND_STAT_HANDED = 1 };
 enum UnlStat { UNL_STAT_RAN_UNL = 0, UNL_STAT_RAN_GENERAL = 1, UNL_STAT_STEPS = 4, UNL_STAT_ALL_STEPS = 5, UNL_STAT_WAVE_STEPS = 8 };
 static_assert(CNT_BAND_DONE == CNT_BAND_STATS + BAND_STAT_DONE && CNT_BAND_HANDED == CNT_BAND_STATS + BAND_STAT_HANDED, "band kernel's counters");
+static_assert(CNT_WBAND_DONE == CNT_WBAND_STATS + BAND_STAT_DONE && CNT_WBAND_HANDED == CNT_WBAND_STATS + BAND_STAT_HANDED, "160-diagonal band stage's counters");
 static_assert(CNT_UNL_RAN_UNL == CNT_UNL_STATS + UNL_STAT_RAN_UNL && CNT_UNL_RAN_GENERAL == CNT_UNL_STATS + UNL_STAT_RAN_GENERAL &&
               CNT_UNL_STEPS == CNT_UNL_STATS + UNL_STAT_STEPS && CNT_ALL_STEPS == CNT_UNL_STATS + UNL_STAT_ALL_STEPS &&
               CNT_WAVE_STEPS == CNT_UNL_STATS + UNL_STAT_WAVE_STEPS, "wavefront kernel's counters");
 constexpr bool counter_slots_distinct() {
     constexpr int all[] = {CNT_FAST_QUEUE, CNT_SLOW_COUNT, CNT_GENERIC_QUEUE, CNT_BAND_QUEUE, CNT_LIST_COUNT, CNT_BAND_DONE, CNT_BAND_HANDED,
                            CNT_WIDE_SLOW_COUNT, CNT_WIDE_QUEUE, CNT_UNL_RAN_UNL, CNT_UNL_RAN_GENERAL, CNT_UNL_LIST_COUNT, CNT_UNL_QUEUE,
-                           CNT_UNL_STEPS, CNT_ALL_STEPS, CNT_CAND_COUNT, CNT_SORTED_COUNT, CNT_WAVE_STEPS};
+                           CNT_UNL_STEPS, CNT_ALL_STEPS, CNT_CAND_COUNT, CNT_SORTED_COUNT, CNT_WAVE_STEPS,
+                           CNT_WBAND_QUEUE, CNT_WCAND_COUNT, CNT_WBAND_DONE, CNT_WBAND_HANDED};
     unsigned seen = 0;
     for (int s : all) { if (s < 0 || s >= kCounterWords || ((seen >> s) & 1u)) return false; seen |= 1u << s; }
     return true;
@@ -223,6 +241,7 @@
     int bandRows;
     const int *list;
     const unsigned int *list_count;
+    int wideSlack;
 };
 
 struct GenericParams {
diff --git a/bbmap_amd/csrc/msa_ctx.h b/bbmap_amd/csrc/msa_ctx.h
--- a/bbmap_amd/csrc/msa_ctx.h
+++ b/bbmap_amd/csrc/msa_ctx.h
@@ -28,6 +28,7 @@
     unsigned int *d_widthHist = nullptr;
     int bandRows = 0, bandLds = 0;
     unsigned int *d_bandDir = nullptr;
+    int wideBandBlocks = 0, wideBandLds = 0, wideBandSlack = 0;
     DevBuf fastList;
     DevBuf gref, gaux, gjobs;
     hipEvent_t ev[4] = {};
@@ -52,7 +53,7 @@
     p.maxRows = c->cfg.maxRows; p.maxColumns = c->cfg.maxColumns; p.bandwidth = c->cfg.bandwidth; p.bandwidthRatio = c->cfg.bandwidthRatio;
 }
 
-int bbmsa_width_sort(bbmsa_ctx *c, hipStream_t stream, const bbmsa_job *jobs, int64_t n_jobs, bool band);
+int bbmsa_width_sort(bbmsa_ctx *c, hipStream_t stream, const bbmsa_job *jobs, int64_t n_jobs, bool band, bool wideBand);
 
 int bbmsa_align_impl(bbmsa_ctx *c, void *stream_, int64_t n_jobs, const uint32_t *n_jobs_dev, const bbmsa_job *jobs,
                      const uint8_t *reads, const uint8_t *refs, bbmsa_result *results, uint8_t *match, int32_t match_stride);
@@ -61,9 +62,10 @@
 int bbmsa_wait_first_pass(bbmsa_ctx *c, void *waiter);
 void bbmsa_sort_by_width(bbmsa_ctx *c, bool on);
 void bbmsa_sort_with_band(bbmsa_ctx *c, bool on);
+void bbmsa_set_wide_band(bbmsa_ctx *c, bool on);
 void bbmsa_set_wide_unlimited(bbmsa_ctx *c, bool on);
 int bbmsa_set_latency_jobs(bbmsa_ctx *c, int64_t n);
-enum { BBMSA_ROUTE_NARROW = 1, BBMSA_ROUTE_SORTED = 2, BBMSA_ROUTE_LATENCY = 4 };
+enum { BBMSA_ROUTE_NARROW = 1, BBMSA_ROUTE_SORTED = 2, BBMSA_ROUTE_LATENCY = 4, BBMSA_ROUTE_WIDE_BAND = 8 };
 int bbmsa_last_route_flags(const bbmsa_ctx *c);
 
 int bbmsa_legacy_create(bbmsa_ctx *c);
diff --git a/bbmap_amd/csrc/msa_fill_band.hip b/bbmap_amd/csrc/msa_fill_band.hip
--- a/bbmap_amd/csrc/msa_fill_band.hip
+++ b/bbmap_amd/csrc/msa_fill_band.hip
@@ -11,12 +11,15 @@
 __device__ __forceinline__ unsigned ld_coherent(const unsigned *p) { return __hip_atomic_load(p, __ATOMIC_RELAXED, __HIP_MEMORY_SCOPE_AGENT); }
 __device__ __forceinline__ unsigned ld_coherent(const uint8_t *p) { return __hip_atomic_load(p, __ATOMIC_RELAXED, __HIP_MEMORY_SCOPE_AGENT); }
 
-struct BandSet {
-    int M[4], D[4], I[4];
+template <int P> struct RefBytes { typedef unsigned type; };
+template <> struct RefBytes<5> { typedef unsigned long long type; };
+
+template <int P> struct BandSet {
+    int M[P], D[P], I[P];
     int rows, columns;
     int c0off;
     int minScoreOff, vs;
-    unsigned w;
+    typename RefBytes<P>::type w;
     int gprev;
     int gmask, mprev;
     int gpass;
@@ -31,12 +34,19 @@
 #define BBMSA_BAND_OCC 4
 #endif
 
-template <int Q>
-__global__ __launch_bounds__(256, BBMSA_BAND_OCC) void msa_fill_band_kernel(const NarrowParams p) {
-    constexpr int B = 4 * Q;
+#ifndef BBMSA_BANDW_OCC
+#define BBMSA_BANDW_OCC 3
+#endif
+
+template <int Q, int P>
+__global__ __launch_bounds__(256, (P == 4 ? BBMSA_BAND_OCC : BBMSA_BANDW_OCC)) void msa_fill_band_kernel(const NarrowParams p) {
+    constexpr int B = P * Q;
+    typedef typename RefBytes<P>::type RefW;
     constexpr int GROUPS = 64 / Q;
     constexpr int JOBS = 2 * GROUPS;
-    static_assert(Q == 4 || Q == 8 || Q == 16, "a group is a power of two of lanes, its good bits fit 64");
+    static_assert(Q == 4 || Q == 8 || Q == 16 || Q == 32, "a group is a power of two of lanes, two jobs per group");
+    static_assert((P == 4 || P == 5) && 4 * P + P <= 32, "a lane's records and good bits of a row share one dword");
+    static_assert(P == 5 || B <= 64, "with four positions per lane a row's good bits are gathered in one 64-bit word");
     extern __shared__ int lds[];
     const int TL = p.tableLen;
     int *delC = lds, *insC = lds + TL, *delExt = lds + 2 * TL, *insExt = delExt + 128;
@@ -74,14 +84,15 @@
                     ta = max(0, ta); tb = min(t.ref_len - 1, tb);
                     if (tb - ta >= p.maxColumns) tb = min(t.ref_len - 1, ta + p.maxColumns - 1);
                 }
-                if (band_is_candidate(t.flags, t.minScore, t.read_len, tb - ta + 1, p.maxRows, p.maxColumns, p.bandRows, p.maxSlack)) { myJ = t_; break; }
+                if (P == 4 ? band_is_candidate(t.flags, t.minScore, t.read_len, tb - ta + 1, p.maxRows, p.maxColumns, p.bandRows, p.maxSlack)
+                           : wide_band_is_candidate(t.flags, t.minScore, t.read_len, tb - ta + 1, p.maxRows, p.maxColumns, p.bandRows, p.maxSlack, p.wideSlack)) { myJ = t_; break; }
                 const unsigned k = atomicAdd(p.fast_count, 1u);
                 p.fast_list[k] = (int)t_;
             }
         }
         if (!__any(myJ >= 0)) break;
 
-        BandSet S[2];
+        BandSet<P> S[2];
         long long jobJ[2]; bool jobOk[2];
 #pragma unroll
         for (int s = 0; s < 2; s++) {
@@ -155,9 +166,9 @@
             const int set = (q & 1) ^ s;
 #pragma unroll
             for (int x = 0; x < 2; x++) if (x == set) {
-                BandSet &T = S[x];
-                for (int i = 0; i < 4; i++) { T.M[i] = 0; T.D[i] = 0; T.I[i] = 0; }
-                T.rows = ok ? rows : 0; T.columns = columns; T.c0off = D0 + 4 * q;
+                BandSet<P> &T = S[x];
+                for (int i = 0; i < P; i++) { T.M[i] = 0; T.D[i] = 0; T.I[i] = 0; }
+                T.rows = ok ? rows : 0; T.columns = columns; T.c0off = D0 + P * q;
                 T.minScoreOff = minScoreOff; T.vs = cost;
                 T.w = 0; T.gprev = 1; T.gmask = 0; T.mprev = 0; T.gpass = 0; T.bail = 0;
                 T.rdOff = rdOff; T.rfOff = rfOff; T.slot = s;
@@ -167,8 +178,8 @@
         __builtin_amdgcn_wave_barrier();
 #pragma unroll
         for (int x = 0; x < 2; x++) {
-            BandSet &T = S[x];
-            if (T.rows > 0) for (int i = 0; i < 3; i++) T.w |= (unsigned)jobLds[T.rfOff + 1 + 4 * q + i] << (8 * (i + 1));
+            BandSet<P> &T = S[x];
+            if (T.rows > 0) for (int i = 0; i < P - 1; i++) T.w |= (RefW)jobLds[T.rfOff + 1 + P * q + i] << (8 * (i + 1));
         }
         int maxRowsWave = max(S[0].rows, S[1].rows);
         for (int d = 32; d >= 1; d >>= 1) maxRowsWave = max(maxRowsWave, __shfl_xor(maxRowsWave, d, 64));
@@ -177,10 +188,10 @@
         for (int k = 1; k <= maxRowsWave + Q / 2; k++) {
 #pragma unroll
             for (int x = 0; x < 2; x++) {
-                BandSet &T = S[x];
-                const BandSet &O = S[1 - x];
+                BandSet<P> &T = S[x];
+                const BandSet<P> &O = S[1 - x];
                 const int row = k - (x == 0 ? rowLagX : rowLagY);
-                int lM = from_left(O.M[3], 0), lD = from_left(O.D[3], 0), gIn = from_left(O.gpass, 0);
+                int lM = from_left(O.M[P - 1], 0), lD = from_left(O.D[P - 1], 0), gIn = from_left(O.gpass, 0);
                 int uM = from_right(O.M[0], 0), uI = from_right(O.I[0], 0), uG = from_right(O.gmask, 0);
                 const bool rowAct = row >= 1 && row <= T.rows;
                 if (rowAct) {
@@ -193,16 +204,16 @@
                     const int clN = row < rows ? jobLds[T.rdOff + row] : 0;
                     T.vs -= fully_defined(cl1) ? (fully_defined(clN) ? P_MATCH2 : P_MATCH) : 0;
                     const int vlimP = max(T.minScoreOff - T.vs, floorv) + 2048;
-                    T.w = (T.w >> 8) | ((unsigned)jobLds[T.rfOff + row + 4 * q + 3] << 24);
+                    T.w = (T.w >> 8) | ((RefW)jobLds[T.rfOff + row + P * q + P - 1] << (8 * (P - 1)));
                     const int c0 = row + T.c0off;
                     const int insRow = insC[row], insPrev = insC[row - 1];
                     const int delForce = (row < 3 || row > rows - 3) ? INT_MAX : INT_MIN;
-                    const unsigned g5 = (unsigned)T.gmask | (((unsigned)uG & 1u) << 4);
+                    const unsigned g5 = (unsigned)T.gmask | (((unsigned)uG & 1u) << P);
                     const bool rowOne = row == 1;
                     unsigned goods = 0, mbits = 0, word = 0;
                     int leftM = lM, leftD = lD;
 #pragma unroll
-                    for (int i = 0; i < 4; i++) {
+                    for (int i = 0; i < P; i++) {
                         const int c = c0 + i;
                         const int ref1 = (int)((T.w >> (8 * i)) & 255u);
                         const bool inRange = (c >= 1) & (c <= columns);
@@ -215,7 +226,7 @@
                         ci.refPen = 0; ci.limitP = max(vlimP, max(T.minScoreOff - hs, floorv) + 2048); ci.floorP = floorP; ci.subfloor = subfloor;
                         ci.dgM = first ? insPrev : T.M[i]; ci.dgD = first ? insPrev : T.D[i]; ci.dgI = first ? insPrev : T.I[i];
                         ci.lM = first ? insRow : leftM; ci.lD = first ? insRow : leftD;
-                        ci.upM = i < 3 ? T.M[i + 1] : uM; ci.upI = i < 3 ? T.I[i + 1] : uI;
+                        ci.upM = i < P - 1 ? T.M[i + 1] : uM; ci.upI = i < P - 1 ? T.I[i + 1] : uI;
                         ci.delForce = delForce;
                         ci.insForce = ((rowOne & (c > 1)) | ((row > rows - 2) & (c < columns - 1))) ? INT_MAX : INT_MIN;
                         ci.pm8 = ((T.mprev >> i) & 1) ? 8 : 0;
@@ -228,9 +239,9 @@
                         leftM = co.nM; leftD = co.nD;
                     }
                     if (q == 0 && (goods & 1u) && c0 >= 1) T.bail = 1;
-                    if (q == Q - 1 && (goods & 8u) && c0 + 3 < columns) T.bail = 1;
+                    if (q == Q - 1 && (goods & (1u << (P - 1))) && c0 + P - 1 < columns) T.bail = 1;
                     T.gprev = gIn; T.gmask = (int)goods; T.mprev = (int)mbits; T.gpass = (gIn | (goods ? 1 : 0));
-                    dir[((long long)row * 2 + T.slot) * 64 + lane] = word | (goods << 16);
+                    dir[((long long)row * 2 + T.slot) * 64 + lane] = word | (goods << (4 * P));
                 }
             }
         }
@@ -241,9 +252,9 @@
         for (int s = 0; s < 2; s++) {
             const long long j = jobJ[s];
             const int set = (q & 1) ^ s;
-            int lastM[4], lastD[4], lastI[4];
-#pragma unroll
-            for (int i = 0; i < 4; i++) { lastM[i] = set ? S[1].M[i] : S[0].M[i]; lastD[i] = set ? S[1].D[i] : S[0].D[i]; lastI[i] = set ? S[1].I[i] : S[0].I[i]; }
+            int lastM[P], lastD[P], lastI[P];
+#pragma unroll
+            for (int i = 0; i < P; i++) { lastM[i] = set ? S[1].M[i] : S[0].M[i]; lastD[i] = set ? S[1].D[i] : S[0].D[i]; lastI[i] = set ? S[1].I[i] : S[0].I[i]; }
             int bail = set ? S[1].bail : S[0].bail;
             for (int d = 1; d < Q; d <<= 1) bail |= __shfl_xor(bail, d, 64);
             const bool live = jobOk[s];
@@ -266,7 +277,7 @@
             const int per = (rows + Q - 1) / Q;
             const int rFirst = q * per + 1, rLast = min(rows, (q + 1) * per);
             int iters = 0, lastColStart = 1, lastHasGood = 0, lastEntered = 0;
-            {
+            if constexpr (B <= 64) {
                 unsigned long long pg = 0;
                 if (rFirst > 1 && rFirst <= rLast) for (int l = 0; l < Q; l++) pg |= (unsigned long long)((ld_coherent(jdir + (long long)(rFirst - 1) * 128 + l) >> 16) & 15u) << (4 * l);
                 for (int r = rFirst; r <= rLast; r++) {
@@ -281,6 +292,28 @@
                     if (r == rows) { lastColStart = colStart; lastHasGood = g != 0; lastEntered = entered; }
                     pg = g;
                 }
+            } else {
+                auto row_span = [&](int r, int &lo, int &hi) {
+                    lo = -1; hi = -1;
+                    for (int l = 0; l < Q; l++) {
+                        const unsigned g = (ld_coherent(jdir + (long long)r * 128 + l) >> (4 * P)) & ((1u << P) - 1u);
+                        if (g) { if (lo < 0) lo = P * l + __builtin_ctz(g); hi = P * l + (31 - __builtin_clz(g)); }
+                    }
+                };
+                int plo = -1, phi = -1;
+                if (rFirst > 1 && rFirst <= rLast) row_span(rFirst - 1, plo, phi);
+                for (int r = rFirst; r <= rLast; r++) {
+                    int lo, hi;
+                    row_span(r, lo, hi);
+                    const bool entered = r == 1 || plo >= 0;
+                    const int colStart = r == 1 ? 1 : (r - 1) + D0 + (plo >= 0 ? plo : B - 1);
+                    const int colStop = r == 1 ? columns : (r - 1) + D0 + (phi >= 0 ? phi : 0);
+                    const int maxG = hi >= 0 ? r + D0 + hi : -2;
+                    const int endc = min(columns, max(colStop, maxG) + 1);
+                    if (entered) iters += endc - colStart + 1;
+                    if (r == rows) { lastColStart = colStart; lastHasGood = hi >= 0; lastEntered = entered; }
+                    plo = lo; phi = hi;
+                }
             }
             for (int d = 1; d < Q; d <<= 1) iters += __shfl_xor(iters, d, 64);
             {
@@ -289,8 +322,8 @@
             }
             int bScore = INT_MIN, bKey = INT_MAX, bPacked = 0;
 #pragma unroll
-            for (int i = 0; i < 4; i++) {
-                const int c = rows + D0 + 4 * q + i;
+            for (int i = 0; i < P; i++) {
+                const int c = rows + D0 + P * q + i;
                 if (c >= 1 && c <= columns) {
                     const int v[3] = {lastM[i], lastD[i], lastI[i]};
 #pragma unroll
@@ -322,7 +355,7 @@
                 auto nib_at = [&](int r, int c) -> unsigned {
                     const int pos = c - r - D0;
                     if (pos < 0 || pos >= B) return 0u;
-                    return (ld_coherent(jdir + (long long)r * 128 + (pos >> 2)) >> (4 * (pos & 3))) & 15u;
+                    return (ld_coherent(jdir + (long long)r * 128 + (unsigned)pos / P) >> (4 * ((unsigned)pos % P))) & 15u;
                 };
                 int row = rows, col = res1, state = res2, n = 0, stateTime = 0;
                 while (row > 0 && col > 0) {
@@ -406,11 +439,12 @@
     }
 }
 
-template __global__ void msa_fill_band_kernel<8>(const NarrowParams);
-
-const void *band_kernel() { return (const void *)msa_fill_band_kernel<8>; }
-int band_lds_bytes(int tableLen, int bandRows) {
-    constexpr int Q = 8, B = 4 * Q, JOBS = 2 * (64 / Q);
+template __global__ void msa_fill_band_kernel<8, 4>(const NarrowParams);
+template __global__ void msa_fill_band_kernel<32, 5>(const NarrowParams);
+
+const void *band_kernel(bool wide) { return wide ? (const void *)msa_fill_band_kernel<32, 5> : (const void *)msa_fill_band_kernel<8, 4>; }
+int band_lds_bytes(int tableLen, int bandRows, bool wide) {
+    const int Q = wide ? 32 : 8, B = (wide ? 5 : 4) * Q, JOBS = 2 * (64 / Q);
     const int RB = (bandRows + 4 + 3) & ~3, FB = (bandRows + B + 4 + 3) & ~3;
     return lds_table_ints(tableLen) * 4 + 4 * JOBS * (RB + FB);
 }
diff --git a/bbmap_amd/csrc/msa_host.hip b/bbmap_amd/csrc/msa_host.hip
--- a/bbmap_amd/csrc/msa_host.hip
+++ b/bbmap_amd/csrc/msa_host.hip
@@ -24,8 +24,8 @@
 const void *fast_kernel_unl_for(int R);
 const void *fast_kernel_both_for(int R);
 template <class S> __global__ void msa_fill_generic_kernel(const GenericParams p);
-const void *band_kernel();
-int band_lds_bytes(int tableLen, int bandRows);
+const void *band_kernel(bool wide);
+int band_lds_bytes(int tableLen, int bandRows, bool wide);
 }
 
 static int clamp_occupancy(int per, int most) { return per < 1 ? 1 : (per > most ? most : per); }
@@ -168,16 +168,25 @@
     if (!c->sw.banded && env_int("BBMSA_NARROW", 1) != 0) {
         int perCU = 0;
         c->bandRows = cfg->maxRows < 256 ? cfg->maxRows : 256;
-        c->bandLds = bbmsa::band_lds_bytes(c->tableLen, c->bandRows);
-        if (c->bandLds > 64 * 1024) BBHIP(hipFuncSetAttribute(bbmsa::band_kernel(), hipFuncAttributeMaxDynamicSharedMemorySize, c->bandLds));
-        BBHIP(hipOccupancyMaxActiveBlocksPerMultiprocessor(&perCU, bbmsa::band_kernel(), 256, c->bandLds));
+        c->bandLds = bbmsa::band_lds_bytes(c->tableLen, c->bandRows, false);
+        if (c->bandLds > 64 * 1024) BBHIP(hipFuncSetAttribute(bbmsa::band_kernel(false), hipFuncAttributeMaxDynamicSharedMemorySize, c->bandLds));
+        BBHIP(hipOccupancyMaxActiveBlocksPerMultiprocessor(&perCU, bbmsa::band_kernel(false), 256, c->bandLds));
         c->narrowBlocks = c->numCUs * clamp_occupancy(perCU, 4);
         c->sw.bandPresent = true;
-        BBHIP(hipMalloc(&c->d_bandDir, (size_t)c->narrowBlocks * 4 * (size_t)(c->bandRows + 1) * 128 * 4));
+        int widePerCU = 0;
+        c->wideBandLds = bbmsa::band_lds_bytes(c->tableLen, c->bandRows, true);
+        if (c->wideBandLds > 64 * 1024) BBHIP(hipFuncSetAttribute(bbmsa::band_kernel(true), hipFuncAttributeMaxDynamicSharedMemorySize, c->wideBandLds));
+        BBHIP(hipOccupancyMaxActiveBlocksPerMultiprocessor(&widePerCU, bbmsa::band_kernel(true), 256, c->wideBandLds));
+        c->wideBandBlocks = c->numCUs * clamp_occupancy(widePerCU, 4);
+        c->wideBandSlack = env_int("BBMSA_WIDE_BAND_SLACK", 9000);
+        c->sw.wideBandPresent = true;
+        const int dirBlocks = c->narrowBlocks > c->wideBandBlocks ? c->narrowBlocks : c->wideBandBlocks;
+        BBHIP(hipMalloc(&c->d_bandDir, (size_t)dirBlocks * 4 * (size_t)(c->bandRows + 1) * 128 * 4));
     }
     c->sw.sortByWidth = env_int("BBMSA_SORT_BY_WIDTH", 0) != 0;
     c->sw.sortWithBand = env_int("BBMSA_SORT_WITH_BAND", 0) != 0;
     c->sw.wideUnlimited = env_int("BBMSA_WIDE_UNLIMITED", 0) != 0;
+    c->sw.wideBand = env_int("BBMSA_WIDE_BAND", 0) != 0;
     c->sw.unlimitedLoop = env_int("BBMSA_UNLIMITED_LOOP", 1) != 0;
     c->unlimitedStats = env_int("BBMSA_UNLIMITED_STATS", 0) != 0 || getenv("BBMAP_DP_COUNTS") != nullptr;
     { const int lat = env_int("BBMSA_LATENCY_JOBS", 0); if (lat > 0) BBTRY(bbmsa_set_latency_jobs(c, lat)); }
@@ -283,18 +292,21 @@
     return BBMAP_OK;
 }
 
-int launch_band(bbmsa_ctx *c, const JobBatch &B, const Route &r, hipStream_t stream) {
+int launch_band(bbmsa_ctx *c, const JobBatch &B, const Route &r, hipStream_t stream, bool wide) {
     int *const fastList = c->fastList.as<int>();
     bbmsa::NarrowParams np;
     set_batch(np, c, B);
-    np.queue = c->d_counters + CNT_BAND_QUEUE; np.fast_list = fastList; np.fast_count = c->d_counters + CNT_LIST_COUNT;
-    np.stats = c->d_counters + CNT_BAND_STATS; np.maxSlack = c->narrowSlack;
+    np.queue = c->d_counters + (wide ? CNT_WBAND_QUEUE : CNT_BAND_QUEUE); np.fast_list = fastList; np.fast_count = c->d_counters + CNT_LIST_COUNT;
+    np.stats = c->d_counters + (wide ? CNT_WBAND_STATS : CNT_BAND_STATS); np.maxSlack = c->narrowSlack; np.wideSlack = c->wideBandSlack;
     np.dirbuf32 = c->d_bandDir; np.tableLen = c->tableLen; np.bandRows = c->bandRows;
-    np.list = r.sorted ? fastList + 2 * r.jobs : nullptr; np.list_count = r.sorted ? c->d_counters + CNT_CAND_COUNT : nullptr;
-    long long nb = (r.jobs + 63) / 64;
-    if (nb > c->narrowBlocks) nb = c->narrowBlocks;
+    np.list = r.sorted ? fastList + (wide ? 3 : 2) * r.jobs : nullptr;
+    np.list_count = r.sorted ? c->d_counters + (wide ? CNT_WCAND_COUNT : CNT_CAND_COUNT) : nullptr;
+    const int jobsPerBlock = wide ? 16 : 64;
+    long long nb = (r.jobs + jobsPerBlock - 1) / jobsPerBlock;
+    const long long most = wide ? c->wideBandBlocks : c->narrowBlocks;
+    if (nb > most) nb = most;
     void *nargs[] = {&np};
-    BBHIP(hipLaunchKernel(bbmsa::band_kernel(), dim3((unsigned)nb), dim3(256), nargs, (size_t)c->bandLds, stream));
+    BBHIP(hipLaunchKernel(bbmsa::band_kernel(wide), dim3((unsigned)nb), dim3(256), nargs, (size_t)(wide ? c->wideBandLds : c->bandLds), stream));
     return BBMAP_OK;
 }
 
@@ -349,7 +361,7 @@
     const size_t listBytes = (size_t)n_jobs * 4;
     BBHIP(c->slowList.grow(listBytes, 0, &stream));
     if (r.wide) BBHIP(c->slowList2.grow(listBytes, 0, &stream));
-    if (c->sw.bandPresent || r.sorted) BBHIP(c->fastList.grow(r.sorted ? 3 * listBytes : listBytes, 0, &stream));
+    if (c->sw.bandPresent || r.sorted) BBHIP(c->fastList.grow(r.sorted ? (r.wideBand ? 4 : 3) * listBytes : listBytes, 0, &stream));
     BBHIP(hipMemsetAsync(c->d_counters, 0, bbmsa::kCounterBytes, stream));
     c->last = r;
     BBHIP(hipEventRecord(c->ev[0], stream));
@@ -359,8 +371,9 @@
         BBHIP(hipEventRecord(c->ev[1], stream));
         return launch_generic<bbmsa::Scheme9PacBio>(c, B, stream, c->slowList.as<int>(), c->d_counters + CNT_SLOW_COUNT);
     }
-    if (r.sorted) BBTRY(bbmsa_width_sort(c, stream, jobs, n_jobs, r.band));
-    if (r.band) BBTRY(launch_band(c, B, r, stream));
+    if (r.sorted) BBTRY(bbmsa_width_sort(c, stream, jobs, n_jobs, r.band, r.wideBand));
+    if (r.band) BBTRY(launch_band(c, B, r, stream, false));
+    if (r.wideBand) BBTRY(launch_band(c, B, r, stream, true));
     BBHIP(hipEventRecord(c->ev[3], stream));
     bbmsa::FillParams fp = first_pass_params(c, B, r);
     const int jobsPerBlock = 4 * (64 / c->G);
@@ -380,6 +393,7 @@
 void bbmsa_sort_by_width(bbmsa_ctx *c, bool on) { if (c) c->sw.sortByWidth = on; }
 void bbmsa_sort_with_band(bbmsa_ctx *c, bool on) { if (c) c->sw.sortWithBand = on; }
 void bbmsa_set_wide_unlimited(bbmsa_ctx *c, bool on) { if (c) c->sw.wideUnlimited = on; }
+void bbmsa_set_wide_band(bbmsa_ctx *c, bool on) { if (c) c->sw.wideBand = on; }
 int bbmsa_set_latency_jobs(bbmsa_ctx *c, int64_t n) {
     if (!c || c->sw.scheme != BBMSA_SCHEME_11TS || c->legacyOnly) return BBMAP_OK;
     BBHIP(hipSetDevice(c->device));
@@ -434,6 +448,7 @@
     if (getenv("BBMAP_DP_COUNTS")) {
         if (r.wide) fprintf(stderr, "   (first pass handed %u jobs to the wide pass)\n", h[CNT_SLOW_COUNT]);
         if (r.sorted) fprintf(stderr, "   (sorted: %u general, %u unlimited, %u band candidates)\n", h[CNT_SORTED_COUNT], h[CNT_UNL_LIST_COUNT], h[CNT_CAND_COUNT]);
+        if (r.wideBand) fprintf(stderr, "   (160-diagonal band stage: %u candidates, %u finished, %u handed on)\n", h[CNT_WCAND_COUNT], h[CNT_WBAND_DONE], h[CNT_WBAND_HANDED]);
         fprintf(stderr, "   (the wavefronts ran %u steps)\n", h[CNT_WAVE_STEPS]);
     }
     return BBMAP_OK;
@@ -453,6 +468,15 @@
     return BBMAP_OK;
 }
 
+extern "C" int bbmsa_last_wide_band(bbmsa_ctx *c, int64_t *counts4) {
+    if (!c || !c->timed || !counts4) return bbfail(BBMAP_E_ARG, "bbmsa_last_wide_band: nothing launched yet");
+    unsigned h[bbmsa::kCounterWords];
+    BBTRY(read_counters(c, h));
+    const bool ran = c->last.wideBand;
+    counts4[0] = ran; counts4[1] = ran ? h[CNT_WCAND_COUNT] : 0; counts4[2] = ran ? h[CNT_WBAND_DONE] : 0; counts4[3] = ran ? h[CNT_WBAND_HANDED] : 0;
+    return BBMAP_OK;
+}
+
 extern "C" int bbmsa_last_unlimited(bbmsa_ctx *c, int64_t *counts4) {
     if (!c || !c->timed || !counts4) return bbfail(BBMAP_E_ARG, "bbmsa_last_unlimited: nothing launched yet");
     const bool wave = c->sw.scheme == BBMSA_SCHEME_11TS && !c->legacyOnly;
@@ -466,7 +490,8 @@
 
 int bbmsa_last_route_flags(const bbmsa_ctx *c) {
     if (!c || !c->timed) return 0;
-    return (c->last.band ? BBMSA_ROUTE_NARROW : 0) | (c->last.sorted ? BBMSA_ROUTE_SORTED : 0) | (c->last.latency ? BBMSA_ROUTE_LATENCY : 0);
+    return (c->last.band ? BBMSA_ROUTE_NARROW : 0) | (c->last.sorted ? BBMSA_ROUTE_SORTED : 0) | (c->last.latency ? BBMSA_ROUTE_LATENCY : 0) |
+           (c->last.wideBand ? BBMSA_ROUTE_WIDE_BAND : 0);
 }
 
 extern "C" int bbmsa_last_route(bbmsa_ctx *c, int64_t *route8) {
diff --git a/bbmap_amd/csrc/msa_route.h b/bbmap_amd/csrc/msa_route.h
--- a/bbmap_amd/csrc/msa_route.h
+++ b/bbmap_amd/csrc/msa_route.h
@@ -8,6 +8,8 @@
     bool bandOff = false;
     bool sortByWidth = false;
     bool sortWithBand = false;
+    bool wideBand = false;
+    bool wideBandPresent = false;
     bool unlimitedLoop = true;
     bool wideUnlimited = false;
     bool widePresent = false;
@@ -21,6 +23,7 @@
     bool latency = false;
     bool indirect = false;
     bool wide = false;
+    bool wideBand = false;
     bool unlList = false;
     bool wideBoth = false;
     bool pipelined = false;
@@ -38,6 +41,7 @@
     r.wide = s.widePresent;
     r.sorted = s.sortByWidth && !indirect && n_jobs >= 256 && n_jobs > s.latencyJobs && (!r.band || s.sortWithBand);
     r.latency = r.wide && !indirect && !r.band && n_jobs <= s.latencyJobs;
+    r.wideBand = s.wideBand && s.wideBandPresent && r.band && r.sorted;
     r.unlList = r.sorted && s.unlimitedLoop;
     r.wideBoth = s.wideUnlimited && !s.banded;
     return r;
diff --git a/bbmap_amd/csrc/msa_sort.hip b/bbmap_amd/csrc/msa_sort.hip
--- a/bbmap_amd/csrc/msa_sort.hip
+++ b/bbmap_amd/csrc/msa_sort.hip
@@ -6,17 +6,18 @@
 
 namespace bbmsa {
 constexpr int WIDTH_PER_CLASS = 512;
-constexpr int WIDTH_CLASSES = 3;
+constexpr int WIDTH_CLASSES = 4;
 constexpr int WIDTH_BUCKETS = WIDTH_CLASSES * WIDTH_PER_CLASS;
-enum { CLASS_UNLIMITED = 0, CLASS_CANDIDATE = 1, CLASS_GENERAL = 2 };
+enum { CLASS_UNLIMITED = 0, CLASS_CANDIDATE = 1, CLASS_GENERAL = 2, CLASS_WIDE_CANDIDATE = 3 };
 constexpr int SORT_THREADS = 256, SORT_JOBS_PER_THREAD = 4;
-struct SortKey { int maxRows, maxColumns, bandwidth; float bandwidthRatio; int byKind, band, bandRows, maxSlack; };
+struct SortKey { int maxRows, maxColumns, bandwidth; float bandwidthRatio; int byKind, band, bandRows, maxSlack, wideBand, wideSlack; };
 __device__ inline int job_width_bucket(const bbmsa_job &t, const SortKey k) {
     int a = t.refStartLoc, b = t.refEndLoc;
     if (t.flags & BBMSA_CLAMP_WINDOW) { a = max(0, a); b = min(t.ref_len - 1, b); if (b - a >= k.maxColumns) b = min(t.ref_len - 1, a + k.maxColumns - 1); }
     const int cols = max(0, b - a + 1);
     int cls = CLASS_GENERAL;
     if (k.band && band_is_candidate(t.flags, t.minScore, t.read_len, b - a + 1, k.maxRows, k.maxColumns, k.bandRows, k.maxSlack)) cls = CLASS_CANDIDATE;
+    else if (k.wideBand && wide_band_is_candidate(t.flags, t.minScore, t.read_len, b - a + 1, k.maxRows, k.maxColumns, k.bandRows, k.maxSlack, k.wideSlack)) cls = CLASS_WIDE_CANDIDATE;
     else if (k.byKind && !fill_is_limited(t.flags, t.minScore, t.read_len, b - a + 1, fill_halfband(t.read_len, b - a + 1, k.bandwidth, k.bandwidthRatio))) cls = CLASS_UNLIMITED;
     constexpr int W = WIDTH_PER_CLASS;
     return cls * W + W - 1 - min(W - 1, cols >> 3);
@@ -34,7 +35,7 @@
     __syncthreads();
     for (int i = threadIdx.x; i < WIDTH_BUCKETS; i += SORT_THREADS) { const unsigned v = s[i]; if (v) atomicAdd(&hist[i], v); }
 }
-__global__ void width_scan_kernel(unsigned *hist, unsigned *listCount, unsigned *sortedCount, unsigned *unlCount, unsigned *candCount) {
+__global__ void width_scan_kernel(unsigned *hist, unsigned *listCount, unsigned *sortedCount, unsigned *unlCount, unsigned *candCount, unsigned *wideCandCount) {
     __shared__ unsigned s[WIDTH_PER_CLASS];
     const int t = threadIdx.x;
     for (int cls = 0; cls < WIDTH_CLASSES; cls++) {
@@ -46,12 +47,13 @@
         if (t == WIDTH_PER_CLASS - 1) {
             if (cls == CLASS_UNLIMITED) *unlCount = s[t];
             else if (cls == CLASS_CANDIDATE) *candCount = s[t];
+            else if (cls == CLASS_WIDE_CANDIDATE) *wideCandCount = s[t];
             else { *listCount = s[t]; *sortedCount = s[t]; }
         }
         __syncthreads();
     }
 }
-__global__ __launch_bounds__(SORT_THREADS) void width_scatter_kernel(const bbmsa_job *jobs, long long n, SortKey key, unsigned *cursor, int *list, int *unlList, int *candList) {
+__global__ __launch_bounds__(SORT_THREADS) void width_scatter_kernel(const bbmsa_job *jobs, long long n, SortKey key, unsigned *cursor, int *list, int *unlList, int *candList, int *wideCandList) {
     __shared__ unsigned s[WIDTH_BUCKETS];
     for (int i = threadIdx.x; i < WIDTH_BUCKETS; i += SORT_THREADS) s[i] = 0;
     __syncthreads();
@@ -73,26 +75,26 @@
         const unsigned pos = s[bucket[k]] + rank[k];
         if ((long long)pos >= n) continue;
         const int cls = bucket[k] / WIDTH_PER_CLASS;
-        (cls == CLASS_UNLIMITED ? unlList : (cls == CLASS_CANDIDATE ? candList : list))[pos] = (int)i;
+        (cls == CLASS_UNLIMITED ? unlList : (cls == CLASS_CANDIDATE ? candList : (cls == CLASS_WIDE_CANDIDATE ? wideCandList : list)))[pos] = (int)i;
     }
 }
 }
 
-int bbmsa_width_sort(bbmsa_ctx *c, hipStream_t stream, const bbmsa_job *jobs, int64_t n_jobs, bool band) {
+int bbmsa_width_sort(bbmsa_ctx *c, hipStream_t stream, const bbmsa_job *jobs, int64_t n_jobs, bool band, bool wideBand) {
     using namespace bbmsa;
     if (!c->d_widthHist) BBHIP(hipMalloc(&c->d_widthHist, WIDTH_BUCKETS * 4));
     BBHIP(hipMemsetAsync(c->d_widthHist, 0, WIDTH_BUCKETS * 4, stream));
     const int perBlock = SORT_THREADS * SORT_JOBS_PER_THREAD;
     const unsigned sb = (unsigned)((n_jobs + perBlock - 1) / perBlock);
     const SortKey key = {c->cfg.maxRows, c->cfg.maxColumns, c->cfg.bandwidth, c->cfg.bandwidthRatio, c->sw.unlimitedLoop ? 1 : 0,
-                         band ? 1 : 0, c->bandRows, c->narrowSlack};
+                         band ? 1 : 0, c->bandRows, c->narrowSlack, wideBand ? 1 : 0, c->wideBandSlack};
     int *const list = c->fastList.as<int>();
     unsigned *const cnt = c->d_counters;
     hipLaunchKernelGGL(width_hist_kernel, dim3(sb), dim3(SORT_THREADS), 0, stream, jobs, (long long)n_jobs, key, c->d_widthHist);
     hipLaunchKernelGGL(width_scan_kernel, dim3(1), dim3(WIDTH_PER_CLASS), 0, stream, c->d_widthHist, cnt + CNT_LIST_COUNT, cnt + CNT_SORTED_COUNT,
-                       cnt + CNT_UNL_LIST_COUNT, cnt + CNT_CAND_COUNT);
+                       cnt + CNT_UNL_LIST_COUNT, cnt + CNT_CAND_COUNT, cnt + CNT_WCAND_COUNT);
     hipLaunchKernelGGL(width_scatter_kernel, dim3(sb), dim3(SORT_THREADS), 0, stream, jobs, (long long)n_jobs, key, c->d_widthHist,
-                       list, list + n_jobs, list + 2 * n_jobs);
+                       list, list + n_jobs, list + 2 * n_jobs, list + 3 * n_jobs);
     BBHIP(hipGetLastError());
     return BBMAP_OK;
 }
diff --git a/bbmap_amd/mapper.py b/bbmap_amd/mapper.py
--- a/bbmap_amd/mapper.py
+++ b/bbmap_amd/mapper.py
@@ -70,7 +70,8 @@
                [("probe_stats", C.c_int64 * 5), ("reads_reprobed", C.c_int64), ("ms_overflow", C.c_float), ("log_growths", C.c_float),
                 ("ms_dp_wave_max", C.c_float), ("ms_final", C.c_float), ("final_fills", C.c_int64), ("final_rounds", C.c_int64),
                 ("final_local", C.c_int64), ("dp_narrow_launches", C.c_int64), ("dp_sorted_launches", C.c_int64),
-                ("sites_cross_scaffold", C.c_int64)]
+                ("sites_cross_scaffold", C.c_int64), ("dp_wide_band_launches", C.c_int64), ("dp_wide_band_finished", C.c_int64),
+                ("dp_wide_band_handed", C.c_int64)]
 
 
 class bbmap_overflow_output(C.Structure):
diff --git a/bbmap_amd/msa.py b/bbmap_amd/msa.py
--- a/bbmap_amd/msa.py
+++ b/bbmap_amd/msa.py
@@ -156,6 +156,11 @@
         c = (C.c_int64 * 4)()
         _lib.check(self.L.bbmsa_last_counts(self.h, c), "bbmsa_last_counts")
         return {"narrow": c[0], "narrow_left": c[1], "wave": c[2], "generic": c[3]}
+
+    def last_wide_band(self):
+        c = (C.c_int64 * 4)()
+        _lib.check(self.L.bbmsa_last_wide_band(self.h, c), "bbmsa_last_wide_band")
+        return {"ran": bool(c[0]), "candidates": c[1], "finished": c[2], "handed_on": c[3]}
 
     def debug_sorted_lists(self, n_jobs):
         lists = np.full((3, n_jobs), -1, np.int32)
diff --git a/include/bbmap_amd.h b/include/bbmap_amd.h
--- a/include/bbmap_amd.h
+++ b/include/bbmap_amd.h
@@ -124,6 +124,7 @@
 int bbmsa_last_kernel_ms(bbmsa_ctx *ctx, float *ms_fast, float *ms_slow);
 int bbmsa_last_kernel_ms3(bbmsa_ctx *ctx, float *ms3);
 int bbmsa_last_counts(bbmsa_ctx *ctx, int64_t *counts4);
+int bbmsa_last_wide_band(bbmsa_ctx *ctx, int64_t *counts4);
 int bbmsa_debug_sorted_lists(bbmsa_ctx *ctx, int64_t n_jobs, int32_t *lists3, int64_t *lens3);
 int bbmsa_last_route(bbmsa_ctx *ctx, int64_t *route8);
 int bbmsa_last_unlimited(bbmsa_ctx *ctx, int64_t *counts4);
@@ -475,6 +476,8 @@
     int64_t dp_narrow_launches;
     int64_t dp_sorted_launches;
     int64_t sites_cross_scaffold;
+    int64_t dp_wide_band_launches;
+    int64_t dp_wide_band_finished, dp_wide_band_handed;
 } bbmap_stats;
 
 typedef struct bbmap_ctx bbmap_ctx;
```

Result: slower. 9.978 million (-4.5%).
